# peterhpark/neuroclear

Hardware: AMD Instinct MI355X
Metric: voxels/sec (higher is better)
Workload: dtype f32

## Files before the change

include/nc_hip.h:

```cpp
#ifndef NC_HIP_H
#define NC_HIP_H

#include <stddef.h>
#include <stdint.h>

#ifdef __cplusplus
extern "C" {
#endif

#define NC_OK 0
#define NC_ERR_SHAPE (-1)
#define NC_ERR_WS (-2)
#define NC_ERR_HIP (-3)
#define NC_ERR_ARG (-4)

const char* nc_last_error(void);
int nc_version(void);
int nc_conv_fwd_path(int C, int K, int kd, int kh, int kw, int stride, int pad);
int nc_conv_wgrad_path(int C, int K, int kd, int kh, int kw, int stride, int pad);
void nc_prof_begin(double min_flop);
int nc_prof_end(int max, int* cls, double* flop, float* ms);
int nc_prof_end2(int max, int* cls, double* flop, float* ms, double* abytes);
void nc_set_force_direct(int on);
void nc_sconv_set_cfg(int cfg);
// ... 2 lines not shown
size_t nc_conv_ws_bytes(int N, int C, int D, int H, int W, int K, int kd, int kh, int kw, int stride, int pad);
int nc_conv_fwd(const float* x, const float* w, const float* bias, float* y, int N, int C, int D, int H, int W,
                int K, int kd, int kh, int kw, int stride, int pad, void* ws, size_t ws_bytes, void* stream);
int nc_conv_dgrad(const float* dy, const float* w, float* dx, int N, int C, int D, int H, int W, int K, int kd,
                  int kh, int kw, int stride, int pad, void* ws, size_t ws_bytes, void* stream);
int nc_conv_wgrad(const float* x, const float* dy, float* dw, float* dbias , int N, int C, int D, int H,
                  int W, int K, int kd, int kh, int kw, int stride, int pad, void* ws, size_t ws_bytes, void* stream);
int nc_conv_bwd(const float* x, const float* dy, const float* w, float* dx, float* dw, float* dbias, int N, int C, int D, int H, int W,
                int K, int kd, int kh, int kw, int stride, int pad, void* ws, size_t ws_bytes, void* stream);

#define NC_DT_F32 0
#define NC_DT_F16 1
#define NC_DT_BF16 2
int nc_conv_lp_supported(int what, int N, int C, int D, int H, int W, int K, int kd, int kh, int kw, int stride, int pad);
size_t nc_conv_lp_ws_bytes(int N, int C, int D, int H, int W, int K, int kd, int kh, int kw, int stride, int pad);
size_t nc_c8_bytes(int N, int C, long S);
int nc_to_c8(const float* x, void* xh, int N, int C, long S, int dtype, void* stream);
int nc_conv_fwd_lp(const float* x, const void* xh, const float* w, const float* bias, float* y, int N, int C, int D, int H,
                   int W, int K, int kd, int kh, int kw, int stride, int pad, int dtype, void* ws, size_t ws_bytes,
                   void* stream);
int nc_conv_dgrad_lp(const float* dy, const void* dyh, const float* w, float* dx, int N, int C, int D, int H, int W, int K,
                     int kd, int kh, int kw, int stride, int pad, int dtype, void* ws, size_t ws_bytes, void* stream);
int nc_conv_wgrad_lp(const float* x, const void* xh, const float* dy, const void* dyh, float* dw,
                     float* dbias , int N, int C, int D, int H, int W, int K, int kd, int kh, int kw,
                     int stride, int pad, int dtype, void* ws, size_t ws_bytes, void* stream);

size_t nc_convT_ws_bytes(int N, int C, int D, int H, int W, int K);
int nc_convT_k2s2_fwd(const float* x, const float* w, const float* bias, float* y, int N, int C, int D, int H, int W,
                      int K, void* stream);
int nc_convT_k2s2_dgrad(const float* dy, const float* w, float* dx, int N, int C, int D, int H, int W, int K,
                        void* ws, size_t ws_bytes, void* stream);
int nc_convT_k2s2_wgrad(const float* x, const float* dy, float* dw, float* dbias, int N, int C, int D, int H, int W,
                        int K, void* ws, size_t ws_bytes, void* stream);

size_t nc_instnorm_ws_bytes(int NC, long S);
int nc_instnorm_stats(const float* x, int NC, long S, float eps, float* mean, float* rstd, void* ws, size_t ws_bytes,
                      void* stream);
int nc_instnorm_fwd(const float* x, float eps, float slope, float* mean, float* rstd, float* y, int NC, long S, void* ws,
                    size_t ws_bytes, void* stream);
int nc_instnorm_act_fwd(const float* x, const float* mean, const float* rstd, float slope, float* y, int NC, long S,
                        void* stream);
int nc_instnorm_act_bwd(const float* dy, const float* x, const float* mean, const float* rstd, float slope, float* dx,
                        int NC, long S, void* ws, size_t ws_bytes, void* stream);
int nc_batchnorm_stats(const float* x, int N, int C, long S, float eps, float momentum, int training, float* mean, float* rstd,
                       float* running_mean, float* running_var, void* ws, size_t ws_bytes, void* stream);
int nc_batchnorm_act_fwd(const float* x, const float* mean, const float* rstd, const float* gamma, const float* beta, float slope, float* y,
                         int N, int C, long S, void* stream);
int nc_batchnorm_act_bwd(const float* dy, const float* x, const float* mean, const float* rstd, const float* gamma, const float* beta,
                         float slope, int training, float* dx, float* dgamma, float* dbeta, float* coef , int N, int C,
                         long S, void* ws, size_t ws_bytes, void* stream);
size_t nc_instnorm_bwd_dbias_ws_bytes(int NC, long S);
int nc_instnorm_act_bwd_dbias(const float* dy, const float* x, const float* mean, const float* rstd, float slope, float* dx,
                              float* dbias, int N, int C, long S, void* ws, size_t ws_bytes, void* stream);
int nc_instnorm_act_bwd_dbias_s3(const float* dy, const float* x, const float* mean, const float* rstd, float slope, void* dxs, float* dbias,
                                 int N, int C, long S, void* ws, size_t ws_bytes, void* stream);
int nc_instnorm_act_fwd_c8(const float* x, const float* mean, const float* rstd, float slope, float* y , void* yh,
                           int N, int C, long S, int dtype, void* stream);
int nc_instnorm_act_bwd_c8(const float* dy, const float* x, const float* mean, const float* rstd, float slope, float* dx,
                           void* dxh, float* dbias , int N, int C, long S, int dtype, void* ws, size_t ws_bytes,
                           void* stream);
int nc_leaky_relu_fwd(const float* x, float slope, float* y, long n, void* stream);
int nc_leaky_relu_bwd(const float* dy, const float* x, float slope, float* dx, long n, void* stream);

int nc_maxpool2_fwd(const float* x, float* y, int NC, int D, int H, int W, void* stream);
int nc_maxpool2_bwd(const float* dy, const float* x, float* dx, int NC, int D, int H, int W, void* stream);
int nc_maxpool2_bwd_add(const float* dy, const float* x, const float* skip, float* dx, int NC, int D, int H, int W,
                        void* stream);

int nc_sigmoid_fwd(const float* x, float* y, long n, void* stream);
int nc_sigmoid_bwd(const float* dy, const float* y, float* dx, long n, void* stream);

int nc_slice_fwd(const float* vol, float* out, int NC, int D, int H, int W, int axis, int index, void* stream);
int nc_slice_bwd(const float* dout, float* dvol, int NC, int D, int H, int W, int axis, int index, void* stream);
int nc_mip_fwd(const float* vol, float* out, int32_t* arg, int NC, int D, int H, int W, int axis, int start, int depth,
               void* stream);
int nc_mip_bwd(const float* dout, const int32_t* arg, float* dvol, int NC, int D, int H, int W, int axis,
               void* stream);

int nc_volume_slices(const float* src, float* dst, int N, int C, int D, int H, int W, int axis, int to_volume,
                     void* stream);

size_t nc_loss_ws_bytes(long n);
int nc_mse_const_fwd(const float* pred, long n, float target, float* out, void* ws, size_t ws_bytes, void* stream);
int nc_mse_const_bwd(const float* pred, long n, float target, const float* gscale, float* dpred, void* stream);
int nc_bce_logits_const_fwd(const float* pred, long n, float target, float* out, void* ws, size_t ws_bytes, void* stream);
int nc_bce_logits_const_bwd(const float* pred, long n, float target, const float* gscale, float* dpred, void* stream);
int nc_mean_fwd(const float* pred, long n, float* out, void* ws, size_t ws_bytes, void* stream);
int nc_mean_bwd(long n, const float* gscale, float* dpred, void* stream);
int nc_l1_fwd(const float* a, const float* b, long n, float* out, void* ws, size_t ws_bytes, void* stream);
int nc_l1_bwd(const float* a, const float* b, long n, const float* gscale, float* da, void* stream);

int nc_adam_step(float* p, const float* g, float* m, float* v, long n, float lr, float beta1, float beta2, float eps,
                 int step, void* stream);

int nc_dice_cut_cube(const void* vol, int is_u16, int L0, int L1, int L2, int roi, int overlap, int border, int index,
                     float* cube, void* stream);
int nc_rotate_crop(const void* vol, int is_u16, int D, int H, int W, int z0, int y0, int x0, int cz, int cy, int cx,
                   const double* inv_affine, float* out, void* stream);
int nc_assemble_scatter_add(const float* cube, float* acc, int P0, int P1, int P2, int roi, int overlap, int border,
                            int index, void* stream);
int nc_assemble_finalize(const float* acc, void* out, int out_is_u16, int P0, int P1, int P2, int L0, int L1, int L2,
                         int roi, int overlap, void* stream);
int nc_assemble_finalize_slab(const float* acc_slab, void* out, int out_is_u16, int P0, int P1, int P2, int L0, int L1, int L2, int roi,
                              int overlap, int z0, int nz, int za, void* stream);

int nc_assemble_merge(const float* acc, float* merged, int L0, int L1, int L2, int roi, int overlap, void* stream);
int nc_radix_hist(const float* x, long n, int pass, unsigned prefix, unsigned* hist4096, void* stream);
int nc_assemble_rescale_finalize(const float* merged, void* out, int out_is_u16, int L0, int L1, int L2, int roi,
                                 int overlap, float lo, float hi, float range, void* stream);

size_t nc_match_histograms_ws_bytes(long n);
int nc_match_histograms(const float* source, const float* tmpl, float* out, long n, void* ws, size_t ws_bytes,
                        void* stream);

int nc_spectral_norm_fwd(const float* w_orig, float* u, float* v, float* w_out, float* sigma, float* scratch_k, int K, int M,
                         int power_iteration, float eps, void* stream);
int nc_spectral_norm_bwd(const float* g, const float* w_sn, const float* u, const float* v, const float* sigma, float* dw_orig, int K,
                         int M, void* stream);

size_t nc_patchgan_param_floats(int n_layers, int ndf, int nd);
size_t nc_patchgan_saved_floats(int B, int D, int H, int W, int n_layers, int ndf, int nd);
size_t nc_patchgan_ws_bytes(int B, int D, int H, int W, int n_layers, int ndf, int nd);
int nc_patchgan_out_shape(int B, int D, int H, int W, int n_layers, int ndf, int nd, int* oD, int* oH, int* oW);
int nc_patchgan_fwd(const float* params, const float* x, float* y, float* saved, int B, int D, int H, int W,
                    int n_layers, int ndf, int nd, void* ws, size_t ws_bytes, void* stream);
int nc_patchgan_bwd(const float* params, const float* x, const float* saved, const float* dy, float* dx, float* dparams,
                    int B, int D, int H, int W, int n_layers, int ndf, int nd, void* ws, size_t ws_bytes, void* stream);
int nc_patchgan_fwd_part(const float* params, const float* x, float* y, float* saved, int Btot, int b0, int B, int D, int H,
                         int W, int n_layers, int ndf, int nd, void* ws, size_t ws_bytes, void* stream);
int nc_patchgan_bwd_part(const float* params, const float* x, const float* saved, const float* dy, float* dx, int Btot, int b0,
                         int B, int D, int H, int W, int n_layers, int ndf, int nd, void* ws, size_t ws_bytes, void* stream);
size_t nc_patchgan_gp_saved_floats(int B, int D, int H, int W, int n_layers, int ndf, int nd);
size_t nc_patchgan_gp_ws_bytes(int B, int D, int H, int W, int n_layers, int ndf, int nd);
int nc_patchgan_gp_fwd(const float* params, const float* x, float* g, float* pen, float* saved, int B, int D, int H, int W, int n_layers,
                       int ndf, int nd, float constant, float lambda_gp, void* ws, size_t ws_bytes, void* stream);
int nc_patchgan_gp_bwd(const float* params, const float* x, const float* saved, const float* g, const float* dpen, float* dparams, float* dx,
                       int B, int D, int H, int W, int n_layers, int ndf, int nd, float constant, float lambda_gp, void* ws, size_t ws_bytes,
                       void* stream);

size_t nc_unet_deconv_fwd_ws_bytes(int N, int S0, int S1, int S2);
int nc_unet_deconv_fwd(const float* params, const float* x, float* y, int N, int S0, int S1, int S2, void* ws,
                       size_t ws_bytes, void* stream);


size_t nc_unet_deconv_param_floats(void);
size_t nc_unet_deconv_saved_floats(int N, int S0, int S1, int S2);
size_t nc_unet_deconv_train_ws_bytes(int N, int S0, int S1, int S2);
int nc_unet_deconv_train_fwd(const float* params, const float* x, float* y, float* saved, int N, int S0, int S1, int S2,
                             void* ws, size_t ws_bytes, void* stream, unsigned* kept);
int nc_unet_deconv_bwd(const float* params, const float* x, const float* y, const float* saved, const float* dy, float* dx,
                       float* dparams, int N, int S0, int S1, int S2, void* ws, size_t ws_bytes, void* stream, unsigned kept);
void nc_set_unet_lean(int on);
int nc_get_unet_lean(void);
void nc_set_unet_wprep(int on);
int nc_get_unet_wprep(void);
int nc_unet_wprep_layout(int N, int S0, int S1, int S2, int block, int form, size_t* pack_off, size_t* pack_bytes, size_t* cell_off,
                         size_t* bound_off);
int nc_s3x_pack_h2_debug(const float* w, int C, int K, int form, const unsigned* cell_a, const unsigned* cell_b, void* wp, unsigned* wcell,
                         void* stream);
int nc_convT_h2_bound_debug(const float* w, const float* bias, int C, int K, float in_bound, unsigned* cell, void* stream);
size_t nc_deep_linear_param_floats(void);
size_t nc_deep_linear_saved_floats(int N, int S0, int S1, int S2);
size_t nc_deep_linear_ws_bytes(int N, int S0, int S1, int S2);
int nc_deep_linear_fwd(const float* params, const float* x, float* y, float* saved , int N, int S0, int S1,
                       int S2, void* ws, size_t ws_bytes, void* stream, unsigned* kept );
void nc_set_dl_collapse(int on);
int nc_get_dl_collapse(void);
int nc_deep_linear_bwd(const float* params, const float* x, const float* saved, const float* dy, float* dx, float* dparams,
                       int N, int S0, int S1, int S2, void* ws, size_t ws_bytes, void* stream, unsigned kept);

int nc_conv_fwd_c8(const void* xh, const float* w, const float* bias, void* yh, int out_ctot, int out_c0, int N, int C, int D, int H,
                   int W, int K, int kd, int kh, int kw, int stride, int pad, int dtype, void* ws, size_t ws_bytes, void* stream);
int nc_conv_dgrad_c8(const void* dyh, const float* w, void* dxh, int N, int C, int D, int H, int W, int K, int kd, int kh, int kw,
                     int stride, int pad, int dtype, void* ws, size_t ws_bytes, void* stream);
size_t nc_conv_c1_c8_ws_bytes(int N, int D, int H, int W, int ks);
int nc_conv_c1_fwd_c8(const float* x, const float* w, const float* bias, void* yh, int out_ctot, int out_c0, int N, int D, int H, int W,
                      int ks, int dtype, void* ws, size_t ws_bytes, void* stream);
int nc_conv_c1_dgrad_c8(const void* dyh, const float* w, float* dx, int N, int D, int H, int W, int ks, void* ws, size_t ws_bytes,
                        void* stream);
size_t nc_conv_c1_wgrad_c8_ws_bytes(int N, int D, int H, int W, int ks);
int nc_conv_c1_wgrad_c8(const float* x, const void* dyh, float* dw, int N, int D, int H, int W, int ks, void* ws, size_t ws_bytes,
                        void* stream);
size_t nc_c8_instnorm_ws_bytes(int N, int C, long S);
int nc_c8_instnorm_stats(const void* xh, int N, int C, long S, float eps, float* mean, float* rstd, int dtype, void* ws,
                         size_t ws_bytes, void* stream);
int nc_c8_instnorm_act_fwd(const void* xh, const float* mean, const float* rstd, float slope, void* yh, int out_ctot, int out_c0,
                           int N, int C, long S, int dtype, void* stream);
int nc_c8_instnorm_act_bwd(const void* gh, int g_ctot, int g_c0, const void* xh, const float* mean, const float* rstd, float slope,
                           void* dxh, float* dbias , int N, int C, long S, int dtype, void* ws, size_t ws_bytes,
                           void* stream);
int nc_c8_maxpool2_fwd(const void* xh, int x_ctot, int x_c0, void* yh, int N, int C, int D, int H, int W, int dtype, void* stream);
int nc_c8_maxpool2_bwd_add(const void* dph, const void* xh, int x_ctot, int x_c0, const void* skiph, int s_ctot, int s_c0, void* dxh,
                           int N, int C, int D, int H, int W, int dtype, void* stream);
int nc_from_c8(const void* xh, int x_ctot, int x_c0, float* y, int N, int C, long S, int dtype, void* stream);
size_t nc_convT_c8_ws_bytes(int N, int C, int D, int H, int W, int K);
int nc_convT_k2s2_fwd_c8(const void* xh, const float* w, const float* bias, void* yh, int out_ctot, int out_c0, int N, int C, int D,
                         int H, int W, int K, int dtype, void* ws, size_t ws_bytes, void* stream);
int nc_convT_k2s2_dgrad_c8(const void* dyh, int dy_ctot, int dy_c0, const float* w, void* dxh, int N, int C, int D, int H, int W, int K,
                           void* ws, size_t ws_bytes, void* stream);
int nc_convT_k2s2_wgrad_c8(const void* xh, const void* dyh, int dy_ctot, int dy_c0, float* dw, float* dbias , int N,
                           int C, int D, int H, int W, int K, void* ws, size_t ws_bytes, void* stream);

int nc_unet_deconv_lp_supported(int N, int S0, int S1, int S2, int dtype);
size_t nc_unet_deconv_lp_saved_bytes(int N, int S0, int S1, int S2);
size_t nc_unet_deconv_lp_ws_bytes(int N, int S0, int S1, int S2);
int nc_unet_deconv_lp_fwd(const float* params, const float* x, float* y, void* saved, int N, int S0, int S1, int S2, int dtype,
                          void* ws, size_t ws_bytes, void* stream);
int nc_unet_deconv_lp_bwd(const float* params, const float* x, const float* y, const void* saved, const float* dy, float* dx,
                          float* dparams, int N, int S0, int S1, int S2, int dtype, void* ws, size_t ws_bytes, void* stream);
int nc_deep_linear_lp_supported(int N, int S0, int S1, int S2, int dtype);
size_t nc_deep_linear_lp_saved_bytes(int N, int S0, int S1, int S2);
size_t nc_deep_linear_lp_ws_bytes(int N, int S0, int S1, int S2);
int nc_deep_linear_lp_fwd(const float* params, const float* x, float* y, void* saved, int N, int S0, int S1, int S2, int dtype,
                          void* ws, size_t ws_bytes, void* stream, unsigned* kept);
int nc_deep_linear_lp_bwd(const float* params, const float* x, const void* saved, const float* dy, float* dx, float* dparams,
                          int N, int S0, int S1, int S2, int dtype, void* ws, size_t ws_bytes, void* stream, unsigned kept);

void nc_set_conv_split(int on);
int nc_get_conv_split(void);
void nc_set_split_terms(int terms);
int nc_get_split_terms(void);
void nc_set_p2d_terms(int mode);
int nc_get_p2d_terms(void);
void nc_set_h2_guard(int on);
int nc_get_h2_guard(void);
int nc_h2_guard_stats(unsigned long long* out4, int reset);
void nc_set_epi_stats(int on);
int nc_get_epi_stats(void);
void nc_set_s3x_w64(int on);
int nc_get_s3x_w64(void);
int nc_unet_deconv_fwd_terms(int S0, int S1, int S2);
void nc_set_c8x_mode(int mode);
int nc_get_c8x_mode(void);
int nc_conv_lp_uses_c8x(int what , int fp32_out, int N, int C, int D, int H, int W, int K, int ks);
void nc_set_s3_fusion(int on);
int nc_conv_split_supported(int what, int N, int C, int D, int H, int W, int K, int kd, int kh, int kw, int stride, int pad);
size_t nc_conv_split_ws_bytes(int N, int C, int D, int H, int W, int K, int ks);
size_t nc_s3_bytes(int N, int C, long S);
int nc_to_s3(const float* x, void* xs, int N, int C, long S, void* stream);
int nc_conv_fwd_split(const float* x, const void* xs, const float* w, const float* bias, float* y, int N, int C, int D, int H, int W,
                      int K, int ks , void* ws, size_t ws_bytes, void* stream);
int nc_conv_dgrad_split(const float* dy, const void* dys, const float* w, float* dx, int N, int C, int D, int H, int W, int K, int ks,
                        void* ws, size_t ws_bytes, void* stream);
int nc_conv_wgrad_split(const float* x, const void* xs, const float* dy, const void* dys, float* dw, int N, int C, int D, int H, int W,
                        int K, int ks, void* ws, size_t ws_bytes, void* stream);

int nc_conv2d_split_active(int what, int N, int C, int H, int W, int K, int k, int stride, int pad);

int nc_convT_k2s2_split_supported(int N, int C, int D, int H, int W, int K);
int nc_convT_k2s2_split_active(int N, int C, int D, int H, int W, int K);
size_t nc_convT_k2s2_split_ws_bytes(int N, int C, int D, int H, int W, int K);
int nc_convT_k2s2_fwd_split(const float* x, const void* xs, const float* w, const float* bias, float* y, void* ys, int ys_ctot, int ys_c0,
                            int N, int C, int D, int H, int W, int K, void* ws, size_t ws_bytes, void* stream);

size_t nc_h2_bytes(int N, int C, long S);
size_t nc_h2_cells_offset(size_t elems);
int nc_to_h2_debug(const float* x, long xstride, void* xs, int N, int C, long S, int ctot, int c0, unsigned* cell, float bound, unsigned* guard,
                   void* stream);
int nc_act_split2h_debug(const float* x, const float* mean, const float* rstd, float slope, float* y, long ystride, void* ys, int N, int C, long S,
                         int ctot, int c0, float bound, unsigned* cell, unsigned* cell2, void* stream);
int nc_act_split2h_pool_debug(const float* x, const float* mean, const float* rstd, float slope, void* ys, void* pooled, int N, int C, int D, int H,
                              int W, int ctot, int c0, float bound, unsigned* cell, void* stream);
int nc_maxpool2_h2_debug(const void* in, void* out, int N, int C, int ctot, int D, int H, int W, void* stream);
int nc_h2_to_s3_if_debug(const void* xh, void* xs, int N, int C, long S, const unsigned* cells, const unsigned* guard, void* stream);
int nc_instnorm_act_bwd_dbias_h2_debug(const float* dy, const float* w1, const float* x, const float* mean, const float* rstd, float slope, void* dxs,
                                       float* dbias, int N, int C, long S, void* ws, size_t ws_bytes, unsigned* guard, void* stream);
size_t nc_convT_k2s2_split_h2_ws_bytes(int N, int C, int D, int H, int W, int K);
int nc_convT_k2s2_fwd_split_h2_debug(const float* x, const float* w, const float* bias, float* y, void* ys, int ys_ctot, int ys_c0, int N, int C,
                                     int D, int H, int W, int K, unsigned* out_cell, void* ws, size_t ws_bytes, void* stream);

size_t nc_lk_ws_bytes(int N, int D, int H, int W, int k);
int nc_lk_fwd(const float* x, const float* w, float* y, int N, int D, int H, int W, int k, void* ws, size_t ws_bytes, void* stream);
int nc_lk_dgrad(const float* dy, const float* w, float* dx, int N, int D, int H, int W, int k, void* ws, size_t ws_bytes, void* stream);
int nc_lk_wgrad(const float* x, const float* dy, float* dw, int N, int D, int H, int W, int k, void* ws, size_t ws_bytes, void* stream);

size_t nc_kgan_param_floats(int ndf, int nd);
size_t nc_kgan_saved_floats(int B, int D, int H, int W, int ndf, int nd);
size_t nc_kgan_ws_bytes(int B, int D, int H, int W, int ndf, int nd);
int nc_kgan_out_shape(int B, int D, int H, int W, int ndf, int nd, int* oD, int* oH, int* oW);
int nc_kgan_fwd(const float* params, const float* x, float* y, float* saved, int B, int D, int H, int W, int ndf, int nd, void* ws,
                size_t ws_bytes, void* stream);
int nc_kgan_bwd(const float* params, const float* x, const float* saved, const float* dy, float* dx, float* dparams, int B, int D, int H,
                int W, int ndf, int nd, void* ws, size_t ws_bytes, void* stream);

#ifdef __cplusplus
}
#endif
#endif
```

neuroclear_amd/_lib.py:

```python
import ctypes
import os
import re

_HERE = os.path.dirname(os.path.abspath(__file__))
LIB_PATH = os.environ.get('NC_HIP_LIB') or os.path.join(_HERE, 'csrc', 'libnc_hip.so')
HEADER_PATH = os.path.join(os.path.dirname(_HERE), 'include', 'nc_hip.h')

_lib = None


class NcError(RuntimeError):
    pass


def header_symbols():
    src = open(HEADER_PATH).read()
    src = re.sub(r'/\*.*?\*/', '', src, flags=re.S)
    return sorted(set(re.findall(r'\b(nc_[a-zA-Z0-9_]+)\s*\(', src)))


def lib():
    global _lib
    if _lib is None:
        if not os.path.exists(LIB_PATH):
            raise NcError('libnc_hip.so is not built (%s): run `python -c "import __graft_entry__ as g; g.build()"` '
                          'or `make -C neuroclear_amd/csrc`; there is no CPU fallback' % LIB_PATH)
        L = ctypes.CDLL(LIB_PATH)
        for name in header_symbols():
            fn = getattr(L, name)
            if name.endswith('_bytes') or name.endswith('_floats') or name == 'nc_h2_cells_offset':
                fn.restype = ctypes.c_size_t
            elif name == 'nc_last_error':
                fn.restype = ctypes.c_char_p
            elif name in ('nc_set_force_direct', 'nc_prof_begin', 'nc_sconv_set_cfg', 'nc_sconv_set_tune', 'nc_set_conv_split', 'nc_set_s3_fusion', 'nc_set_c8x_mode', 'nc_set_split_terms', 'nc_set_h2_guard', 'nc_set_epi_stats', 'nc_set_dl_collapse', 'nc_set_p2d_terms', 'nc_set_s3x_w64', 'nc_set_unet_lean', 'nc_set_unet_wprep'):
                fn.restype = None
            else:
                fn.restype = ctypes.c_int
        _lib = L
    return _lib


def check(code, what=''):
    if code != 0:
        raise NcError('%s failed (%d): %s' % (what, code, lib().nc_last_error().decode()))


P = ctypes.c_void_p
I = ctypes.c_int
L_ = ctypes.c_long
F = ctypes.c_float
Z = ctypes.c_size_t
```

neuroclear_amd/csrc/common.hpp:

```cpp
#pragma once
#include <hip/hip_runtime.h>

#include <cstdarg>
#include <cstdio>

#include "../../include/nc_hip.h"

namespace nc {

void set_error(const char* fmt, ...);

inline int check_launch(const char* what) {
  hipError_t e = hipGetLastError();
  if (e != hipSuccess) {
    set_error("%s: %s", what, hipGetErrorString(e));
    return NC_ERR_HIP;
  }
  return NC_OK;
}

inline long cdiv(long a, long b) { return (a + b - 1) / b; }

int raise_dyn_lds(const void* kernel, int bytes, const char* who);
template <typename K>
// ... 56 lines not shown
bool c1k3_fwd_supported(const ConvDims& d);
int conv_fwd_c1k3(const float* x, const float* w, const float* bias, float* y, const ConvDims& d, hipStream_t s, float* stats_part = nullptr);
size_t c1k3_stats_bytes(const ConvDims& d);
int c1k3_stats_finalize(const float* stats_part, const float* bias, const ConvDims& d, float eps, float* mean, float* rstd, hipStream_t s);
bool mfma_dgrad_supported(const ConvDims& d);
bool mfma_wgrad_supported(const ConvDims& d);
size_t mfma_ws_bytes(const ConvDims& d);
size_t mfma_fwd_ws_bytes(const ConvDims& d);
int conv_fwd_mfma(const float* x, const float* w, const float* b, float* y, const ConvDims& d, void* ws, size_t wsb,
                  hipStream_t s);
int conv_dgrad_mfma(const float* dy, const float* w, float* dx, const ConvDims& d, void* ws, size_t wsb,
                    hipStream_t s);
int conv_wgrad_mfma(const float* x, const float* dy, float* dw, const ConvDims& d, void* ws, size_t wsb,
                    hipStream_t s);

bool gemm_fwd_supported(const ConvDims& d);
bool gemm_dgrad_supported(const ConvDims& d);
bool gemm_wgrad_supported(const ConvDims& d);
size_t gemm_ws_bytes(const ConvDims& d);
int conv_fwd_gemm(const float* x, const float* w, const float* b, float* y, const ConvDims& d, void* ws, size_t wsb,
                  hipStream_t s);
int conv_dgrad_gemm(const float* dy, const float* w, float* dx, const ConvDims& d, void* ws, size_t wsb,
                    hipStream_t s);
int conv_wgrad_gemm(const float* x, const float* dy, float* dw, const ConvDims& d, void* ws, size_t wsb,
                    hipStream_t s);

bool sconv_fwd_supported(const ConvDims& d);
bool sconv_dgrad_supported(const ConvDims& d);
size_t sconv_ws_bytes(const ConvDims& d);
void p2d_set_terms(int m);
int p2d_get_terms();
bool p2d_fwd_supported(const ConvDims& d);
bool p2d_dgrad_supported(const ConvDims& d);
size_t p2d_ws_bytes(const ConvDims& d);
int conv_fwd_p2d(const float* x, const float* w, const float* bias, float* y, const ConvDims& d, void* ws, size_t wsb, hipStream_t s);
int conv_dgrad_p2d(const float* dy, const float* w, float* dx, const ConvDims& d, void* ws, size_t wsb, hipStream_t s);
bool p2d_wgrad_supported(const ConvDims& d);
size_t p2d_wgrad_ws_bytes(const ConvDims& d);
int conv_wgrad_p2d(const float* x, const float* dy, float* dw, const ConvDims& d, void* ws, size_t wsb, hipStream_t s);
int conv_fwd_sconv(const float* x, const float* w, const float* bias, float* y, const ConvDims& d, void* ws, size_t wsb, hipStream_t s);
int conv_dgrad_sconv(const float* dy, const float* w, float* dx, const ConvDims& d, void* ws, size_t wsb, hipStream_t s);
void sconv_set_cfg(int cfg);
void sconv_set_tune(int on);
bool sconv_wgrad_supported(const ConvDims& d);
size_t sconv_wgrad_ws_bytes(const ConvDims& d);
int conv_wgrad_sconv(const float* x, const float* dy, float* dw, const ConvDims& d, void* ws, size_t wsb, hipStream_t s);

bool pg1_supported(const ConvDims& d);
size_t pg1_ws_bytes(const ConvDims& d);
int conv_fwd_pg1(const float* x, const float* w, const float* bias, float* y, const ConvDims& d, float slope, hipStream_t s);
int conv_wgrad_pg1(const float* x, const float* g, const float* act, float slope, float* dw, float* db, const ConvDims& d,
                   void* ws, size_t wsb, hipStream_t s);
int conv_dgrad_pg1(const float* g, const float* act, float slope, const float* w, float* dx, const ConvDims& d, hipStream_t s);

bool wgrad_1x1_supported(const ConvDims& d);
size_t wgrad_1x1_ws_bytes(const ConvDims& d);
int conv_wgrad_1x1(const float* x, const float* dy, float* dw, const ConvDims& d, void* ws, size_t wsb, hipStream_t s);
bool flat_1x1_supported(const ConvDims& d);
int conv_fwd_1x1(const float* x, const float* w, const float* b, float* y, const ConvDims& d, void* ws, size_t wsb,
                 hipStream_t s);
int conv_dgrad_1x1(const float* dy, const float* w, float* dx, const ConvDims& d, void* ws, size_t wsb,
                   hipStream_t s);

size_t conv_fwd_to1_k3_ws_bytes(int N, int D, int H, int W);
int conv_fwd_to1_k3(const float* x, const float* w, float* y, int N, int C, int D, int H, int W, void* ws, size_t wsb, hipStream_t s);
bool to1_dgrad_supported(const ConvDims& d);
int conv_dgrad_to1(const float* dy, const float* w, float* dx, const ConvDims& d, hipStream_t s);
bool to1_mfma_supported(const ConvDims& d);
size_t to1_mfma_ws_bytes(const ConvDims& d);
int conv_dgrad_to1_mfma(const float* dy, const float* w, float* dx, const ConvDims& d, void* ws, size_t wsb,
                        hipStream_t s);
bool k1_fwd_supported(const ConvDims& d);
bool k1_wgrad_supported(const ConvDims& d);
int conv_fwd_k1(const float* x, const float* w, const float* b, float* y, const ConvDims& d, hipStream_t s);
int conv_wgrad_k1(const float* x, const float* dy, float* dw, const ConvDims& d, hipStream_t s);
bool c1_wgrad_supported(const ConvDims& d);
size_t c1_wgrad_ws_bytes(const ConvDims& d);
int conv_wgrad_c1(const float* x, const float* dy, float* dw, const ConvDims& d, void* ws, size_t wsb, hipStream_t s);

bool s3_fwd_supported(const ConvDims& d);
bool s3_dgrad_supported(const ConvDims& d);
size_t s3_ws_bytes(const ConvDims& d);
size_t s3_tensor_bytes(int N, int C, long S);
int split3_to(const float* x, void* xs, int N, int C, long S, hipStream_t s);
int split3_into(const float* x, long xstride, void* xs, int N, int C, long S, int ctot, int c0, hipStream_t s, const unsigned* guard = nullptr);
bool conv_layer_h2(const ConvDims& d);
struct ForceThreeTerm { ForceThreeTerm(); ~ForceThreeTerm(); };
struct NetworkScope { NetworkScope(); ~NetworkScope(); };
struct SwitchScope { SwitchScope(); ~SwitchScope(); };
struct ForceTwoTerm { ForceTwoTerm(); ~ForceTwoTerm(); int prev_terms, prev_depth; };
int frozen_terms();
int frozen_guard();
bool h2_guard_can_flip();
int operand_into(const ConvDims& d, const float* x, long xstride, void* xs, int N, int C, long S, int ctot, int c0, hipStream_t s);
int act_operand(const ConvDims& d, const float* x, const float* mean, const float* rstd, float slope, float* y, long ystride, void* ys, int N, int C,
                long S, int ctot, int c0, hipStream_t s);
int act_split3(const float* x, const float* mean, const float* rstd, float slope, float* y, long ystride, void* ys, int N, int C, long S,
               int ctot, int c0, hipStream_t s);
struct S3xPrepared { const void* wp; const unsigned* wcell; };
int conv_fwd_s3(const float* x, const void* xs, const float* w, const float* b, float* y, const ConvDims& d, void* ws, size_t wsb,
                hipStream_t s, void* xs_keep = nullptr, float* stats_part = nullptr, const S3xPrepared* prep = nullptr);
bool epi_stats_on();
void epi_stats_set(int on);
int epi_stats_mode();
void s3x_w64_set(int on);
int s3x_w64_get();
int conv_dgrad_s3(const float* dy, const void* dys, const float* w, float* dx, const ConvDims& d, void* ws, size_t wsb, hipStream_t s);
size_t s3_bwd_ws_bytes(const ConvDims& d);
int conv_bwd_s3(const float* x, const float* dy, const float* w, float* dx, float* dw, const ConvDims& d, void* ws, size_t wsb,
                hipStream_t s, int phase, const void* xs = nullptr, bool dy_guarded = false, const S3xPrepared* prep = nullptr);
int conv_fwd_keep(const float* x, const float* w, const float* bias, float* y, int N, int C, int D, int H, int W, int K, int ks,
                  void* ws, size_t ws_bytes, void* stream, void* xs_keep, bool* kept, const S3xPrepared* prep = nullptr);
int conv_bwd_keep(const float* x, const void* xs, const float* dy, const float* w, float* dx, float* dw, int N, int C, int D, int H,
                  int W, int K, int ks, void* ws, size_t ws_bytes, void* stream);
bool s3x_supported(int N, int Cin, int D, int H, int W, int Kout, int KS);
size_t s3x_packed_bytes(int Cin, int Kout, int KS, int NT = 3);
int s3x_ksteps(int Cin, int KS);
constexpr int kWPrepMaxSegs = 18, kWPrepMaxBounds = 2, kWPrepBoundCell0 = kWPrepMaxSegs, kWPrepCellBytes = 256;
struct WPrepSeg { const float* w; int Cin, Kout, flip; unsigned a_bits; int b_cell; unsigned* ext_cell; };
struct WPrepBound { const float* w; const float* bias; int C, K; float in_bound; int cell; };
size_t wprep_bytes(const WPrepSeg* segs, int n);
int wprep_run(const WPrepSeg* segs, int n, const WPrepBound* bounds, int nb, void* region, S3xPrepared* out, hipStream_t s);
int s3x_pack_h2(const float* w, int Cin, int Kout, int KS, long so, long si, int flip, int split_c, const unsigned* cell_a, const unsigned* cell_b,
                unsigned* wcell, void* wp_ws, hipStream_t s);
void s3x_set_terms(int t);
int s3x_get_terms();
int conv_s3x_h2(const void* xs, const unsigned* cell_a, const unsigned* cell_b, int split_c, const float* w, const float* bias, float* y, int N,
                int Cin, int D, int H, int W, int Kout, int KS, long so, long si, int flip, unsigned* wcell, void* wp_ws, hipStream_t s,
                const unsigned* guard = nullptr, float* stats_part = nullptr, const S3xPrepared* prep = nullptr);
size_t s3x_stats_bytes(int N, int D, int H, int W, int Kout, int KS);
int s3x_stats_finalize(const float* stats_part, const float* bias, int N, int D, int H, int W, int Kout, int KS, float eps, float* mean, float* rstd,
                       hipStream_t s);
bool c1k7_h2_supported(const ConvDims& d);
size_t c1k7_h2_ws_bytes(const ConvDims& d);
int conv_c1k7_h2(const float* x, const float* w, const float* bias, float* y, const ConvDims& d, void* ws, size_t wsb, hipStream_t s);
size_t c1k7_h2_dgrad_ws_bytes(const ConvDims& d);
bool dl_typed_supported(int N, int D, int H, int W);
size_t dl_typed_bytes(int N, int D, int H, int W);
const float* dl_typed_wp(const char* scratch, int N, int D, int H, int W);
float* dl_typed_dwsw(char* scratch, int N, int D, int H, int W);
int dl_typed_compose(const float* F, char* scratch, int N, int D, int H, int W, hipStream_t s);
int dl_typed_fwd_boundary(const float* act0, float* y, char* scratch, int N, int D, int H, int W, hipStream_t s);
int dl_typed_dgrad_boundary(const float* act0, const float* dy, float* g, char* scratch, int N, int D, int H, int W, hipStream_t s);
int dl_typed_p(const float* act0, const float* dy, float* Pq, char* scratch, int N, int D, int H, int W, hipStream_t s);
int conv_c1k7_h2_dgrad(const float* dy, const float* w, float* dx, const ConvDims& d, void* ws, size_t wsb, hipStream_t s);
inline size_t h2_cells_offset(size_t elems) { return (elems * 4 + 255) & ~(size_t)255; }
inline unsigned* h2_cells_of(const void* t, size_t elems) { return (unsigned*)((char*)const_cast<void*>(t) + h2_cells_offset(elems)); }
int instnorm_relu_tail_sigmoid(const float* x, const float* mean, const float* rstd, const float* w1, const float* b1, const float* w2,
                               const float* b2, float* y, int C, long S, hipStream_t s);
int instnorm_act_bwd_dbias_h2(const float* dy, const float* x, const float* mean, const float* rstd, float slope, void* dxs,
                              float* dbias, int N, int C, long S, void* ws, size_t ws_bytes, void* stream, unsigned* guard = nullptr);
int instnorm_act_bwd_dbias_h2_rank1(const float* dy1, const float* w1, const float* x, const float* mean, const float* rstd, float slope, void* dxs,
                                    float* dbias, int C, long S, void* ws, size_t ws_bytes, void* stream, unsigned* guard);
unsigned* conv_bwd_guard_words(void* ws, int N, int K, long S);
int maxpool2_h2(const void* in, void* out, int N, int C, int ctot, int D, int H, int W, hipStream_t s);
int h2_zero_cells(unsigned* cells, int n, hipStream_t s);
int h2_set_cell(unsigned* cell, float bound, hipStream_t s);
int h2_absmax(const float* x, long n, unsigned* cell, hipStream_t s, unsigned* cell2 = nullptr);
int split2h_into(const float* x, long xstride, void* xs, int N, int C, long S, int ctot, int c0, const unsigned* cell, hipStream_t s,
                 unsigned* guard = nullptr);
constexpr int kGuardLow = 0, kGuardAll = 1, kGuardFlag = 2;
constexpr unsigned kGuardDrop = 17u << 23;
constexpr unsigned long long kGuardShare = 64;
#if defined(__HIP_DEVICE_COMPILE__)
__device__ __forceinline__ bool guard_skip(const unsigned* guard, int want) {
  return guard && (int)(__builtin_nontemporal_load(guard + kGuardFlag) != 0) != want;
}
#else
__device__ bool guard_skip(const unsigned* guard, int want);
#endif
bool h2_guard_on();
int h2_guard_mode();
void h2_guard_set(int on);
int h2_guard_read(unsigned long long* out4, int reset);
int h2_guard_zero(unsigned* g, hipStream_t s, int nwords = 8);
int h2_guard_decide(unsigned* ga, unsigned* gb, unsigned* prior, unsigned* flag, bool can_flip, hipStream_t s, unsigned long long total_a = 0);
int h2_to_s3_if(const void* xh, void* xs, int N, int C, long S, const unsigned* cells, const unsigned* guard, hipStream_t s);
int act_split2h(const float* x, const float* mean, const float* rstd, float slope, float* y, long ystride, void* ys, int N, int C, long S, int ctot,
                int c0, float bound, unsigned* cell, unsigned* cell2, hipStream_t s);
int act_split2h_pool(const float* x, const float* mean, const float* rstd, float slope, void* ys, void* pooled, int N, int C, int D, int H, int W,
                     int ctot, int c0, float bound, unsigned* cell, hipStream_t s);
int conv_s3x(const void* xs, const float* w, const float* bias, float* y, int N, int Cin, int D, int H, int W, int Kout, int KS, long so,
             long si, int flip, void* wp_ws, hipStream_t s, const unsigned* guard = nullptr);
bool conv_keep_supported(int N, int C, int D, int H, int W, int K, int ks);
int conv_fwd_pre(const void* xs, const float* w, const float* bias, float* y, int N, int C, int D, int H, int W, int K, int ks, void* ws,
                 size_t ws_bytes, void* stream, float* stats_part = nullptr, const S3xPrepared* prep = nullptr);
bool conv_bwd_pre_supported(int N, int C, int D, int H, int W, int K, int ks, bool want_dx, size_t ws_bytes);
int conv_bwd_pre(const float* x, const void* xs, const float* w, float* dx, float* dw, int N, int C, int D, int H, int W, int K, int ks,
                 void* ws, size_t ws_bytes, void* stream, bool dy_guarded = false, const S3xPrepared* prep = nullptr);
bool instnorm_bwd_s3_supported(int N, int C, long S);
int instnorm_act_bwd_dbias_s3(const float* dy, const float* x, const float* mean, const float* rstd, float slope, void* dxs,
                              float* dbias, int N, int C, long S, void* ws, size_t ws_bytes, void* stream);
bool convT_fwd_s3_supported(int N, int C, int D, int H, int W, int K);
size_t c8x_packed_bytes(int Cin, int Kout, int KS);
void c8x_set_mode(int m);
int c8x_get_mode();
bool c8x_supported(int N, int Cin, int D, int H, int W, int Kout, int KS, bool fp32_out);
int conv_c8x(const void* xh, const float* w, const float* bias, float* y, void* yh, int ctot, int c0, int N, int Cin, int D, int H, int W,
             int Kout, int KS, long so, long si, int flip, int diffuse, int dt, void* wp_ws, hipStream_t s);
bool convT_s3x_supported(int N, int C, int D, int H, int W, int K);
size_t convT_s3x_ws_bytes(int C, int K);
int convT_fwd_s3x(const void* xs, const float* w, const float* bias, float* y, void* ys, int ctot, int c0, int N, int C, int D, int H, int W,
                  int K, void* ws, size_t wsb, hipStream_t s, const unsigned* h2cell = nullptr, const unsigned* xcell = nullptr);
int convT_h2_bound(const float* w, const float* bias, int C, int K, float in_bound, unsigned* cell, hipStream_t s);
int convT_fwd_split_h2(const float* x, const float* w, const float* bias, float* y, void* ys, int ys_ctot, int ys_c0, int N, int C, int D, int H,
                       int W, int K, const unsigned* out_cell, void* ws, size_t ws_bytes, hipStream_t s);
int convT_fwd_s3(const float* x, const float* w, const float* bias, float* y, void* ys, int ctot, int c0, int N, int C, int D, int H,
                 int W, int K, void* stream);
bool s3_wgrad_supported(const ConvDims& d);
bool c8x_wgrad_supported(const ConvDims& d);
size_t c8x_wgrad_part_bytes(const ConvDims& d);
int conv_wgrad_c8x(const void* xh, const void* dyh, float* dw, const ConvDims& d, int dtype, void* ws, size_t wsb, hipStream_t s);
size_t s3_wgrad_ws_bytes(const ConvDims& d);
int conv_wgrad_s3(const float* x, const void* xs, const float* dy, const void* dys, float* dw, const ConvDims& d, void* ws, size_t wsb,
                  hipStream_t s);
bool s3x_k32_supported(int N, int D, int H, int W);
bool conv_fwd_h2_k32_supported(const ConvDims& d);
int conv_fwd_h2_k32_keep(const float* x, const float* w, float* y, const ConvDims& d, void* ws, size_t wsb, hipStream_t s, void* xs_keep);
bool conv_fwd_h2_c32_supported(const ConvDims& d);
size_t conv_fwd_h2_c32_ws_bytes(const ConvDims& d);
int conv_fwd_h2_c32(const float* x, const float* w, float* y, const ConvDims& d, void* ws, size_t wsb, hipStream_t s);
bool wgrad_h2_supported(const ConvDims& d);
int conv_wgrad_h2(const float* x, const void* xs, const float* dy, const void* dys, float* dw, const ConvDims& d, void* ws, size_t wsb, hipStream_t s);
bool h_fwd_supported(const ConvDims& d);
bool h_dgrad_supported(const ConvDims& d);
bool h_wgrad_supported(const ConvDims& d);
size_t h_ws_bytes(const ConvDims& d);
int to_c8(const float* x, void* xh, int N, int C, long S, int dt, hipStream_t s);
int conv_fwd_h(const float* x, const void* xh, const float* w, const float* b, float* y, const ConvDims& d, int dt,
               void* ws, size_t wsb, hipStream_t s);
int conv_dgrad_h(const float* dy, const void* dyh, const float* w, float* dx, const ConvDims& d, int dt, void* ws,
                 size_t wsb, hipStream_t s);
int conv_wgrad_h(const float* x, const void* xh, const float* dy, const void* dyh, float* dw, const ConvDims& d, int dt,
                 void* ws, size_t wsb, hipStream_t s);
int conv_fwd_h_c8(const void* xh, const float* w, const float* b, void* yh, int ctot, int c0, const ConvDims& d, int dt,
                  void* ws, size_t wsb, hipStream_t s);
int conv_fwd_h_na1(const void* xh, const float* w, float* y, const ConvDims& d, int dt, void* ws, size_t wsb, hipStream_t s);
int conv_dgrad_h_c8(const void* dyh, const float* w, void* dxh, int ctot, int c0, const ConvDims& d, int dt, void* ws,
                    size_t wsb, hipStream_t s);
bool dl_collapse_on();
size_t dl_tail_bytes();
const float* dl_tail_E(const char* tail);
const float* dl_tail_Ef(const char* tail);
float* dl_tail_q(char* tail);
int dl_tail_compose(const float* w2, const float* w3, const float* w4, const float* w5, char* tail, hipStream_t s);
int dl_tail_grads(const float* w2, const float* w3, const float* w4, const float* w5, char* tail, float* dw2, float* dw3, float* dw4, float* dw5,
                  hipStream_t s);
float* dl_tail_P(char* tail);
const float* dl_w1_fold(char* tail, const float* w1, hipStream_t s);
int dl_w1_contract(const char* tail, float* dw1, hipStream_t s);
int dl_q_from_p(char* tail, const float* w1, hipStream_t s);
const float* dl_fold_fwd64(char* tail, const float* w1, hipStream_t s);
int dl_combine27(const float* Z, float* y, int N, int D, int H, int W, int zch, hipStream_t s);
bool c1_h_supported(int D, int H, int W, int KS);
size_t c1_h_ws_bytes(int N, int D, int H, int W, int KS);
int conv_c1_fwd_h(const float* x, const float* w, const float* bias, void* yh, int ctot, int c0, int N, int D, int H, int W, int KS,
                  int dt, void* ws, size_t wsb, hipStream_t s);
int conv_c1_dgrad_h(const void* dyh, const float* w, float* dx, int N, int D, int H, int W, int KS, void* ws, size_t wsb,
                    hipStream_t s);

void h_set_weight_diffusion(int on);

bool c1_wgrad_h_supported(int N, int D, int H, int W, int KS);
size_t c1_wgrad_h_ws_bytes(int N, int D, int H, int W, int KS);
int conv_c1_wgrad_h(const float* x, const void* dyh, float* dw, int N, int D, int H, int W, int KS, void* ws, size_t wsb,
                    hipStream_t s);

static constexpr size_t kPackSlackBytes = 128 * 1024;

extern int g_force_direct;

struct ProfScope {
  int idx;
  hipStream_t s;
  ProfScope(int op, int path, const ConvDims& d, int lp, hipStream_t stream);
  ~ProfScope();
};

}
```

neuroclear_amd/csrc/gen_nets.hip:

```cpp

#include <atomic>
#include <cstdlib>

#include "common.hpp"

using namespace nc;

#define NC_TRY(expr) do { int e_ = (expr); if (e_) return e_; } while (0)

namespace {

size_t up64(size_t n) { return (n + 63) & ~(size_t)63; }

size_t s3_floats(size_t elems) { return up64((elems * 6 + 3) / 4); }
size_t align256(size_t b) { return (b + 255) & ~(size_t)255; }

std::atomic<int> g_unet_lean{getenv("NC_UNET_LEAN") ? (atoi(getenv("NC_UNET_LEAN")) != 0) : 1};
constexpr int kLeanBit0 = 10;
constexpr int kLeanBlocks[5] = {1, 3, 5, 6, 8};
int lean_index(int consumer) {
  for (int j = 0; j < 5; ++j) if (kLeanBlocks[j] == consumer) return j;
  return -1;
}

struct UBlock { int C, K, lvl; };
const UBlock kUB[10] = {{1, 64, 0},    {64, 64, 0},    {64, 128, 1},  {128, 128, 1}, {128, 256, 2},
                        {256, 256, 2}, {256, 256, 2}, {256, 128, 1}, {128, 128, 1}, {128, 64, 0}};

std::atomic<int> g_unet_wprep{getenv("NC_UNET_WPREP") ? (atoi(getenv("NC_UNET_WPREP")) != 0) : 1};
constexpr unsigned kKeptWPrep = 1u << 15;
void wprep_segs(WPrepSeg (&sg)[18]) {
  for (int i = 1; i < 10; ++i) {
    sg[2 * (i - 1)] = WPrepSeg{nullptr, kUB[i].C, kUB[i].K, 0, 0u, -1, nullptr};
    sg[2 * (i - 1) + 1] = WPrepSeg{nullptr, kUB[i].K, kUB[i].C, 1, 0u, -1, nullptr};
  }
}
unsigned f32_bits(float f) { unsigned b; __builtin_memcpy(&b, &f, 4); return b; }


struct UPlan {
  int N, d[3][3];
  long S[3];
  size_t a1, cat1, p1, a2, cat2, p2, b1, b2, b3, e2a, e2b, e1, t1, raw[10], mean[10], rstd[10], saved;
  size_t xs3[10];
  size_t wprep;
  size_t G1, G2, G3, H1, H2, H3, Q1, Q2, s1, s2, T, grads;
  size_t conv_ws, in_ws, convT_ws;
};

bool u_plan(UPlan& p, int N, int S0, int S1, int S2) {
  if (N < 1 || S0 < 4 || S1 < 4 || S2 < 4 || (S0 & 3) || (S1 & 3) || (S2 & 3)) return false;
  p = UPlan{};
  p.N = N;
  for (int l = 0; l < 3; ++l) {
    p.d[l][0] = S0 >> l; p.d[l][1] = S1 >> l; p.d[l][2] = S2 >> l;
    p.S[l] = (long)p.d[l][0] * p.d[l][1] * p.d[l][2];
  }
  const size_t n = (size_t)N, S = (size_t)p.S[0], Sh = (size_t)p.S[1], Sq = (size_t)p.S[2];
  size_t off = 0;
  auto take = [&](size_t k) { size_t r = off; off += up64(k); return r; };
  p.a1 = take(n * 64 * S); p.cat1 = take(n * 128 * S); p.p1 = take(n * 64 * Sh); p.a2 = take(n * 128 * Sh);
  p.cat2 = take(n * 256 * Sh); p.p2 = take(n * 128 * Sq); p.b1 = take(n * 256 * Sq); p.b2 = take(n * 256 * Sq);
  p.b3 = take(n * 256 * Sq); p.e2a = take(n * 128 * Sh); p.e2b = take(n * 128 * Sh); p.e1 = take(n * 64 * S);
  p.t1 = take(n * S);
  for (int i = 0; i < 10; ++i) {
    p.raw[i] = take(n * kUB[i].K * (size_t)p.S[kUB[i].lvl]);
    p.mean[i] = take(n * kUB[i].K);
    p.rstd[i] = take(n * kUB[i].K);
  }
  for (int i = 1; i < 10; ++i) { p.xs3[i] = off; off += s3_floats(n * kUB[i].C * (size_t)p.S[kUB[i].lvl]); }
  {
    WPrepSeg sg[18];
    wprep_segs(sg);
    p.wprep = off;
    off += up64((wprep_bytes(sg, 18) + 3) / 4);
  }
  p.saved = off;
  off = 0;
  p.G1 = take(n * 64 * S); p.G2 = take(n * 64 * S); p.G3 = take(n * 128 * S);
  p.H1 = take(n * 128 * Sh); p.H2 = take(n * 128 * Sh); p.H3 = take(n * 256 * Sh);
  p.Q1 = take(n * 256 * Sq); p.Q2 = take(n * 256 * Sq); p.s1 = take(n * S); p.s2 = take(n * S);
  p.T = take(n * 64 * S);
  p.grads = off;
  auto upd = [&](int C, int K, int l, int k) {
    const size_t b = nc_conv_ws_bytes(N, C, p.d[l][0], p.d[l][1], p.d[l][2], K, k, k, k, 1, k / 2);
    if (b > p.conv_ws) p.conv_ws = b;
  };
  for (int i = 0; i < 10; ++i) upd(kUB[i].C, kUB[i].K, kUB[i].lvl, 3);
  upd(64, 1, 0, 1); upd(1, 1, 0, 1);
  p.in_ws = nc_instnorm_bwd_dbias_ws_bytes(N * 256, (long)S);
  for (int i = 1; i < 10; ++i) {
    const size_t b = s3x_stats_bytes(N, p.d[kUB[i].lvl][0], p.d[kUB[i].lvl][1], p.d[kUB[i].lvl][2], kUB[i].K, 3);
    if (b > p.in_ws) p.in_ws = b;
  }
  p.convT_ws = nc_convT_ws_bytes(N, 256, p.d[2][0], p.d[2][1], p.d[2][2], 128);
  const size_t c2 = nc_convT_ws_bytes(N, 128, p.d[1][0], p.d[1][1], p.d[1][2], 64);
  if (c2 > p.convT_ws) p.convT_ws = c2;
  return true;
}

struct UOff { size_t w[14], b[14], total; };
UOff u_offsets() {
  struct L { int id; size_t wn, bn; };
  const L order[14] = {{0, 64 * 1 * 27, 64},     {1, 64 * 64 * 27, 64},    {2, 128 * 64 * 27, 128},  {3, 128 * 128 * 27, 128},
                       {4, 256 * 128 * 27, 256}, {5, 256 * 256 * 27, 256}, {6, 256 * 256 * 27, 256}, {10, 256 * 128 * 8, 128},
                       {7, 128 * 256 * 27, 128}, {8, 128 * 128 * 27, 128}, {11, 128 * 64 * 8, 64},   {9, 64 * 128 * 27, 64},
                       {12, 64, 1},              {13, 1, 1}};
  UOff o{};
  size_t off = 0;
  for (const L& l : order) {
    o.w[l.id] = off; off += l.wn;
    o.b[l.id] = off; off += l.bn;
  }
  o.total = off;
  return o;
}

int gather_half(const float* src, float* dst, int N, int Ctot, int c0, int C, long S, hipStream_t s) {
  if (hipMemcpy2DAsync(dst, (size_t)C * S * 4, src + (size_t)c0 * S, (size_t)Ctot * S * 4, (size_t)C * S * 4, N,
                       hipMemcpyDeviceToDevice, s) != hipSuccess) {
    set_error("gather_half: hipMemcpy2DAsync failed");
    return NC_ERR_HIP;
  }
  return NC_OK;
}

size_t u_ws_bytes(const UPlan& p, bool bwd) {
  return align256(p.conv_ws) + align256(p.in_ws) + align256(p.convT_ws) + (bwd ? p.grads * sizeof(float) : 0) + 256;
}

}

extern "C" {

void nc_set_unet_wprep(int on) { g_unet_wprep.store(on != 0, std::memory_order_relaxed); }
int nc_get_unet_wprep(void) { return g_unet_wprep.load(std::memory_order_relaxed); }
void nc_set_unet_lean(int on) { g_unet_lean.store(on != 0, std::memory_order_relaxed); }
int nc_get_unet_lean(void) { return g_unet_lean.load(std::memory_order_relaxed); }

size_t nc_unet_deconv_param_floats(void) { return u_offsets().total; }

int nc_unet_wprep_layout(int N, int S0, int S1, int S2, int block, int form, size_t* pack_off, size_t* pack_bytes, size_t* cell_off,
                         size_t* bound_off) {
  UPlan p;
  if (!u_plan(p, N, S0, S1, S2) || block < 1 || block > 9 || form < 0 || form > 1) { set_error("unet_wprep_layout: bad argument"); return NC_ERR_ARG; }
  WPrepSeg sg[18];
  wprep_segs(sg);
  const int k = 2 * (block - 1) + form;
  size_t off = kWPrepCellBytes;
  for (int j = 0; j < k; ++j) off += s3x_packed_bytes(sg[j].Cin, sg[j].Kout, 3, 2);
  if (pack_off) *pack_off = p.wprep * 4 + off;
  if (pack_bytes) *pack_bytes = s3x_packed_bytes(sg[k].Cin, sg[k].Kout, 3, 2);
  if (cell_off) *cell_off = p.wprep * 4 + (size_t)k * 4;
  if (bound_off) *bound_off = block == 7 ? p.wprep * 4 + (size_t)kWPrepBoundCell0 * 4 : block == 9 ? p.wprep * 4 + (size_t)(kWPrepBoundCell0 + 1) * 4 : 0;
  return NC_OK;
}
int nc_s3x_pack_h2_debug(const float* w, int C, int K, int form, const unsigned* cell_a, const unsigned* cell_b, void* wp, unsigned* wcell,
                         void* stream) {
  if (!w || !cell_a || !cell_b || !wp || !wcell || C % 64 || K % 64) { set_error("s3x_pack_h2_debug: bad argument"); return NC_ERR_ARG; }
  if (form) return s3x_pack_h2(w, K, C, 3, 27, (long)C * 27, 1, K, cell_a, cell_a, wcell, wp, (hipStream_t)stream);
  return s3x_pack_h2(w, C, K, 3, (long)C * 27, 27, 0, C / 2, cell_a, cell_b, wcell, wp, (hipStream_t)stream);
}
int nc_convT_h2_bound_debug(const float* w, const float* bias, int C, int K, float in_bound, unsigned* cell, void* stream) {
  if (!w || !cell) { set_error("convT_h2_bound_debug: null pointer"); return NC_ERR_ARG; }
  NC_TRY(h2_zero_cells(cell, 1, (hipStream_t)stream));
  return convT_h2_bound(w, bias, C, K, in_bound, cell, (hipStream_t)stream);
}

size_t nc_unet_deconv_saved_floats(int N, int S0, int S1, int S2) {
  UPlan p;
  return u_plan(p, N, S0, S1, S2) ? p.saved : 0;
}

size_t nc_unet_deconv_train_ws_bytes(int N, int S0, int S1, int S2) {
  UPlan p;
  return u_plan(p, N, S0, S1, S2) ? u_ws_bytes(p, true) : 0;
}

int nc_unet_deconv_train_fwd(const float* params, const float* x, float* y, float* saved, int N, int S0, int S1, int S2,
                             void* ws, size_t ws_bytes, void* stream, unsigned* kept) {
  NetworkScope net_scope;
  if (!params || !x || !y || !saved) { set_error("unet_deconv_train_fwd: null pointer"); return NC_ERR_ARG; }
  UPlan p;
  if (!u_plan(p, N, S0, S1, S2)) {
    set_error("unet_deconv_train_fwd: every edge must be a positive multiple of 4 (got %d,%d,%d)", S0, S1, S2);
    return NC_ERR_SHAPE;
  }
  if (!ws || ws_bytes < u_ws_bytes(p, false)) { set_error("unet_deconv_train_fwd: workspace too small"); return NC_ERR_WS; }
  const UOff o = u_offsets();
  void* cws = ws;
  void* iws = (char*)ws + align256(p.conv_ws);
  float* V = saved;
  const float* P = params;
  if (kept) *kept = 0;
  hipStream_t hs = (hipStream_t)stream;
  static const bool fuse_on = !(getenv("NC_S3_TRAIN_FUSE") && atoi(getenv("NC_S3_TRAIN_FUSE")) == 0);
  const bool lean = g_unet_lean.load(std::memory_order_relaxed) != 0;
  bool use[10], pre[10], h2l[10];
  ConvDims cd[10];
  for (int i = 0; i < 10; ++i) {
    const UBlock& b = kUB[i];
    const int* d = p.d[b.lvl];
    use[i] = fuse_on && i >= 1 && conv_keep_supported(N, b.C, d[0], d[1], d[2], b.K, 3);
    pre[i] = false;
    h2l[i] = make_dims(cd[i], N, b.C, d[0], d[1], d[2], b.K, 3, 3, 3, 1, 1) && use[i] && conv_layer_h2(cd[i]);
  }
  const long S = p.S[0], Sh = p.S[1], Sq = p.S[2];
  const int *d0 = p.d[0], *d1 = p.d[1], *d2 = p.d[2];
  const bool ct2 = nc_convT_k2s2_split_active(1, 256, d2[0], d2[1], d2[2], 128) &&
                   p.conv_ws >= nc_convT_k2s2_split_ws_bytes(1, 256, d2[0], d2[1], d2[2], 128);
  static const bool ct_h2 = !(getenv("NC_CONVT_H2") && atoi(getenv("NC_CONVT_H2")) == 0);
  const bool ct2h = ct2 && h2l[7] && ct_h2;
  const bool ct1 = nc_convT_k2s2_split_active(1, 128, d1[0], d1[1], d1[2], 64) &&
                   p.conv_ws >= nc_convT_k2s2_split_ws_bytes(1, 128, d1[0], d1[1], d1[2], 64);
  const bool ct1h = ct1 && h2l[9] && ct_h2;
  unsigned* cell7 = h2_cells_of(V + p.xs3[7], (size_t)N * 256 * Sh) + 1;
  unsigned* cell9 = h2_cells_of(V + p.xs3[9], (size_t)N * 128 * S) + 1;
  unsigned kept_mask = 0;
  S3xPrepared prep[18] = {};
  bool bound7 = false, bound9 = false;
  if (g_unet_wprep.load(std::memory_order_relaxed) != 0) {
    WPrepSeg sg[18];
    wprep_segs(sg);
    WPrepBound wb[2];
    int nb = 0, any = 0;
    for (int i = 1; i < 10; ++i) {
      if (!h2l[i]) continue;
      WPrepSeg& f = sg[2 * (i - 1)];
      f.a_bits = f32_bits(sqrtf((float)p.S[kUB[i].lvl]));
      f.w = P + o.w[i];
      if (i == 7 || i == 9) {
        if (i == 7 ? ct2h : ct1h) {
          f.b_cell = kWPrepBoundCell0 + nb;
          f.ext_cell = i == 7 ? cell7 : cell9;
          wb[nb++] = i == 7 ? WPrepBound{P + o.w[10], P + o.b[10], 256, 128, sqrtf((float)Sq), 0}
                            : WPrepBound{P + o.w[11], P + o.b[11], 128, 64, sqrtf((float)Sh), 0};
          (i == 7 ? bound7 : bound9) = true;
        } else {
          f.w = nullptr;
        }
      }
      sg[2 * (i - 1) + 1].w = P + o.w[i];
      any = 1;
    }
    if (any) {
      NC_TRY(wprep_run(sg, 18, wb, nb, V + p.wprep, prep, hs));
      kept_mask |= kKeptWPrep;
    }
  }
  auto prep_of = [&](int seg) -> const S3xPrepared* { return prep[seg].wp ? &prep[seg] : nullptr; };
  auto block = [&](int i, const float* in, float* out, size_t out_stride, int to, int to_ctot) -> int {
    const UBlock& b = kUB[i];
    const int* d = p.d[b.lvl];
    const long S = p.S[b.lvl];
    const bool epi = pre[i] && h2l[i] && epi_stats_mode() == 2 && s3x_stats_bytes(N, d[0], d[1], d[2], b.K, 3) && s3x_stats_bytes(N, d[0], d[1], d[2], b.K, 3) <= p.in_ws;
    if (pre[i]) {
      NC_TRY(conv_fwd_pre(V + p.xs3[i], P + o.w[i], P + o.b[i], V + p.raw[i], N, b.C, d[0], d[1], d[2], b.K, 3, cws, p.conv_ws, stream,
                          epi ? (float*)iws : nullptr, i >= 1 ? prep_of(2 * (i - 1)) : nullptr));
      kept_mask |= 1u << i;
      if (h2l[i]) kept_mask |= 1u << (16 + i);
    } else {
      bool kept1 = false;
      NC_TRY(conv_fwd_keep(in, P + o.w[i], P + o.b[i], V + p.raw[i], N, b.C, d[0], d[1], d[2], b.K, 3, cws, p.conv_ws, stream,
                           i >= 1 ? (void*)(V + p.xs3[i]) : nullptr, &kept1, i >= 1 ? prep_of(2 * (i - 1)) : nullptr));
      if (kept1) kept_mask |= 1u << i;
      if (kept1 && i >= 1 && conv_layer_h2(cd[i])) kept_mask |= 1u << (16 + i);
    }
    if (epi) NC_TRY(s3x_stats_finalize((const float*)iws, P + o.b[i], N, d[0], d[1], d[2], b.K, 3, 1e-5f, V + p.mean[i], V + p.rstd[i], hs));
    else NC_TRY(nc_instnorm_stats(V + p.raw[i], N * b.K, S, 1e-5f, V + p.mean[i], V + p.rstd[i], iws, p.in_ws, stream));
    if (to >= 0 && use[to]) {
      const int lj = lean && h2l[to] && to_ctot == b.K ? lean_index(to) : -1;
      if (lj >= 0) { out = nullptr; kept_mask |= 1u << (kLeanBit0 + lj); }
      NC_TRY(act_operand(cd[to], V + p.raw[i], V + p.mean[i], V + p.rstd[i], 0.f, out, (long)out_stride, V + p.xs3[to], N, b.K, S, to_ctot, 0, hs));
      if (to_ctot == b.K) pre[to] = true;
      return NC_OK;
    }
    if (out_stride == (size_t)b.K * S || N == 1)
      return nc_instnorm_act_fwd(V + p.raw[i], V + p.mean[i], V + p.rstd[i], 0.f, out, N * b.K, S, stream);
    for (int n = 0; n < N; ++n)
      NC_TRY(nc_instnorm_act_fwd(V + p.raw[i] + (size_t)n * b.K * S, V + p.mean[i] + n * b.K, V + p.rstd[i] + n * b.K, 0.f,
                                 out + n * out_stride, b.K, S, stream));
    return NC_OK;
  };
  NC_TRY(block(0, x, V + p.a1, (size_t)64 * S, 1, 64));
  NC_TRY(block(1, V + p.a1, V + p.cat1, (size_t)128 * S, 9, 128));
  for (int n = 0; n < N; ++n)
    NC_TRY(nc_maxpool2_fwd(V + p.cat1 + (size_t)n * 128 * S, V + p.p1 + (size_t)n * 64 * Sh, 64, d0[0], d0[1], d0[2], stream));
  NC_TRY(block(2, V + p.p1, V + p.a2, (size_t)128 * Sh, 3, 128));
  NC_TRY(block(3, V + p.a2, V + p.cat2, (size_t)256 * Sh, 7, 256));
  for (int n = 0; n < N; ++n)
    NC_TRY(nc_maxpool2_fwd(V + p.cat2 + (size_t)n * 256 * Sh, V + p.p2 + (size_t)n * 128 * Sq, 128, d1[0], d1[1], d1[2], stream));
  NC_TRY(block(4, V + p.p2, V + p.b1, (size_t)256 * Sq, 5, 256));
  NC_TRY(block(5, V + p.b1, V + p.b2, (size_t)256 * Sq, 6, 256));
  NC_TRY(block(6, V + p.b2, V + p.b3, (size_t)256 * Sq, -1, 0));
  if (ct2h && !bound7) {
    NC_TRY(h2_zero_cells(cell7, 1, hs));
    NC_TRY(convT_h2_bound(P + o.w[10], P + o.b[10], 256, 128, sqrtf((float)Sq), cell7, hs));
  }
  for (int n = 0; n < N; ++n) {
    if (ct2h)
      NC_TRY(convT_fwd_split_h2(V + p.b3 + (size_t)n * 256 * Sq, P + o.w[10], P + o.b[10], V + p.cat2 + ((size_t)n * 256 + 128) * Sh,
                                (char*)(V + p.xs3[7]) + (size_t)n * 256 * Sh * 4, 256, 128, 1, 256, d2[0], d2[1], d2[2], 128, cell7, cws, p.conv_ws, hs));
    else if (ct2)
      NC_TRY(nc_convT_k2s2_fwd_split(V + p.b3 + (size_t)n * 256 * Sq, nullptr, P + o.w[10], P + o.b[10], V + p.cat2 + ((size_t)n * 256 + 128) * Sh,
                                     use[7] && !h2l[7] ? (char*)(V + p.xs3[7]) + (size_t)n * 256 * Sh * 6 : nullptr, 256, 128, 1, 256, d2[0], d2[1], d2[2], 128, cws,
                                     p.conv_ws, stream));
    else
      NC_TRY(nc_convT_k2s2_fwd(V + p.b3 + (size_t)n * 256 * Sq, P + o.w[10], P + o.b[10], V + p.cat2 + ((size_t)n * 256 + 128) * Sh,
                               1, 256, d2[0], d2[1], d2[2], 128, stream));
  }
  if (use[7]) {
    if (!ct2 || (h2l[7] && !ct2h)) NC_TRY(operand_into(cd[7], V + p.cat2 + (size_t)128 * Sh, (long)256 * Sh, V + p.xs3[7], N, 128, Sh, 256, 128, hs));
    pre[7] = true;
  }
  NC_TRY(block(7, V + p.cat2, V + p.e2a, (size_t)128 * Sh, 8, 128));
  NC_TRY(block(8, V + p.e2a, V + p.e2b, (size_t)128 * Sh, -1, 0));
  const bool ct_s3 = use[9] && !h2l[9] && (ct1 || convT_fwd_s3_supported(1, 128, d1[0], d1[1], d1[2], 64));
  if (ct1h && !bound9) {
    NC_TRY(h2_zero_cells(cell9, 1, hs));
    NC_TRY(convT_h2_bound(P + o.w[11], P + o.b[11], 128, 64, sqrtf((float)Sh), cell9, hs));
  }
  for (int n = 0; n < N; ++n) {
    if (ct1h)
      NC_TRY(convT_fwd_split_h2(V + p.e2b + (size_t)n * 128 * Sh, P + o.w[11], P + o.b[11], V + p.cat1 + ((size_t)n * 128 + 64) * S,
                                (char*)(V + p.xs3[9]) + (size_t)n * 128 * S * 4, 128, 64, 1, 128, d1[0], d1[1], d1[2], 64, cell9, cws, p.conv_ws, hs));
    else if (ct1)
      NC_TRY(nc_convT_k2s2_fwd_split(V + p.e2b + (size_t)n * 128 * Sh, nullptr, P + o.w[11], P + o.b[11], V + p.cat1 + ((size_t)n * 128 + 64) * S,
                                     use[9] && !h2l[9] ? (char*)(V + p.xs3[9]) + (size_t)n * 128 * S * 6 : nullptr, 128, 64, 1, 128, d1[0], d1[1], d1[2], 64, cws,
                                     p.conv_ws, stream));
    else if (ct_s3)
      NC_TRY(convT_fwd_s3(V + p.e2b + (size_t)n * 128 * Sh, P + o.w[11], P + o.b[11], V + p.cat1 + ((size_t)n * 128 + 64) * S,
                          (char*)(V + p.xs3[9]) + (size_t)n * 128 * S * 6, 128, 64, 1, 128, d1[0], d1[1], d1[2], 64, stream));
    else
      NC_TRY(nc_convT_k2s2_fwd(V + p.e2b + (size_t)n * 128 * Sh, P + o.w[11], P + o.b[11], V + p.cat1 + ((size_t)n * 128 + 64) * S,
                               1, 128, d1[0], d1[1], d1[2], 64, stream));
  }
  if (use[9]) {
    if (!ct_s3 && !ct1h) NC_TRY(operand_into(cd[9], V + p.cat1 + (size_t)64 * S, (long)128 * S, V + p.xs3[9], N, 64, S, 128, 64, hs));
    pre[9] = true;
  }
  NC_TRY(block(9, V + p.cat1, V + p.e1, (size_t)64 * S, -1, 0));
  NC_TRY(nc_conv_fwd(V + p.e1, P + o.w[12], P + o.b[12], V + p.t1, N, 64, d0[0], d0[1], d0[2], 1, 1, 1, 1, 1, 0, cws, p.conv_ws, stream));
  NC_TRY(nc_conv_fwd(V + p.t1, P + o.w[13], P + o.b[13], y, N, 1, d0[0], d0[1], d0[2], 1, 1, 1, 1, 1, 0, cws, p.conv_ws, stream));
  if (kept) *kept = kept_mask;
  return nc_sigmoid_fwd(y, y, (long)N * S, stream);
}

int nc_unet_deconv_bwd(const float* params, const float* x, const float* y, const float* saved, const float* dy, float* dx,
                       float* dparams, int N, int S0, int S1, int S2, void* ws, size_t ws_bytes, void* stream, unsigned kept) {
  NetworkScope net_scope;
  if (!params || !x || !y || !saved || !dy || !dparams) { set_error("unet_deconv_bwd: null pointer"); return NC_ERR_ARG; }
  UPlan p;
  if (!u_plan(p, N, S0, S1, S2)) { set_error("unet_deconv_bwd: bad shape"); return NC_ERR_SHAPE; }
  if (!ws || ws_bytes < u_ws_bytes(p, true)) { set_error("unet_deconv_bwd: workspace too small"); return NC_ERR_WS; }
  const UOff o = u_offsets();
  hipStream_t hs = (hipStream_t)stream;
  void* cws = ws;
  void* iws = (char*)ws + align256(p.conv_ws);
  void* tws = (char*)iws + align256(p.in_ws);
  float* G = (float*)((char*)tws + align256(p.convT_ws));
  const float* V = saved;
  const float* P = params;
  float* DP = dparams;
  const long S = p.S[0], Sh = p.S[1], Sq = p.S[2];
  const int *d0 = p.d[0], *d1 = p.d[1], *d2 = p.d[2];
  const unsigned kept_mask = kept;
  static const bool fuse_bwd = !(getenv("NC_S3_TRAIN_FUSE") && atoi(getenv("NC_S3_TRAIN_FUSE")) == 0) &&
                               true;
  const bool wprep_now = g_unet_wprep.load(std::memory_order_relaxed) != 0;
  S3xPrepared prepd[10] = {};
  {
    WPrepSeg sg[18];
    wprep_segs(sg);
    const char* region = (const char*)(V + p.wprep);
    size_t off = kWPrepCellBytes;
    for (int k = 0; k < 18; ++k) {
      if (k & 1) prepd[k / 2 + 1] = S3xPrepared{region + off, (const unsigned*)region + k};
      off += s3x_packed_bytes(sg[k].Cin, sg[k].Kout, 3, 2);
    }
  }
  auto block_bwd = [&](int i, const float* g, const float* in, float* draw, float* gin, bool r1 = false) -> int {
    const UBlock& b = kUB[i];
    const int* d = p.d[b.lvl];
    const long Sl = p.S[b.lvl];
    ConvDims cdk;
    const bool now_h2 = make_dims(cdk, N, b.C, d[0], d[1], d[2], b.K, 3, 3, 3, 1, 1) && conv_layer_h2(cdk);
    const void* xs = ((kept_mask >> i) & 1) && (((kept_mask >> (16 + i)) & 1) != 0) == now_h2 ? (const void*)(V + p.xs3[i]) : nullptr;
    const S3xPrepared* pd = i >= 1 && gin && now_h2 && (kept_mask & kKeptWPrep) && ((kept_mask >> (16 + i)) & 1) && wprep_now ? &prepd[i] : nullptr;
    const int lj = lean_index(i);
    if (lj >= 0 && ((kept_mask >> (kLeanBit0 + lj)) & 1) &&
        !(xs && !h2_guard_can_flip() && conv_bwd_pre_supported(N, b.C, d[0], d[1], d[2], b.K, 3, gin != nullptr, p.conv_ws))) {
      NC_TRY(nc_instnorm_act_fwd(V + p.raw[i - 1], V + p.mean[i - 1], V + p.rstd[i - 1], 0.f, G + p.T, N * b.C, Sl, stream));
      in = G + p.T;
    }
    if (r1) {
      NC_TRY(instnorm_act_bwd_dbias_h2_rank1(g, P + o.w[12], V + p.raw[i], V + p.mean[i], V + p.rstd[i], 0.f, cws, DP + o.b[i], b.K, Sl, iws, p.in_ws,
                                             stream, conv_bwd_guard_words(cws, N, b.K, Sl)));
      return conv_bwd_pre(in, xs, P + o.w[i], gin, DP + o.w[i], N, b.C, d[0], d[1], d[2], b.K, 3, cws, p.conv_ws, stream, h2_guard_can_flip(), pd);
    }
    if (fuse_bwd && i >= 1 && conv_bwd_pre_supported(N, b.C, d[0], d[1], d[2], b.K, 3, gin != nullptr, p.conv_ws) &&
        instnorm_bwd_s3_supported(N, b.K, Sl)) {
      if (now_h2)
        NC_TRY(instnorm_act_bwd_dbias_h2(g, V + p.raw[i], V + p.mean[i], V + p.rstd[i], 0.f, cws, DP + o.b[i], N, b.K, Sl, iws, p.in_ws, stream,
                                         conv_bwd_guard_words(cws, N, b.K, Sl)));
      else
        NC_TRY(instnorm_act_bwd_dbias_s3(g, V + p.raw[i], V + p.mean[i], V + p.rstd[i], 0.f, cws, DP + o.b[i], N, b.K, Sl, iws, p.in_ws, stream));
      return conv_bwd_pre(in, xs, P + o.w[i], gin, DP + o.w[i], N, b.C, d[0], d[1], d[2], b.K, 3, cws, p.conv_ws, stream, now_h2 && h2_guard_can_flip(), pd);
    }
    NC_TRY(nc_instnorm_act_bwd_dbias(g, V + p.raw[i], V + p.mean[i], V + p.rstd[i], 0.f, draw, DP + o.b[i], N, b.K, Sl, iws,
                                     p.in_ws, stream));
    return conv_bwd_keep(in, xs, draw, P + o.w[i], gin, DP + o.w[i], N, b.C, d[0], d[1], d[2], b.K, 3, cws, p.conv_ws, stream);
  };
  auto upper_half = [&](const float* dcat, int Ctot, long Sl, const float** out) -> int {
    const int C = Ctot / 2;
    if (N == 1) { *out = dcat + (size_t)C * Sl; return NC_OK; }
    NC_TRY(gather_half(dcat, G + p.T, N, Ctot, C, C, Sl, hs));
    *out = G + p.T;
    return NC_OK;
  };
  NC_TRY(nc_sigmoid_bwd(dy, y, G + p.s1, (long)N * S, stream));
  NC_TRY(nc_conv_wgrad(V + p.t1, G + p.s1, DP + o.w[13], DP + o.b[13], N, 1, d0[0], d0[1], d0[2], 1, 1, 1, 1, 1, 0, cws, p.conv_ws, stream));
  NC_TRY(nc_conv_dgrad(G + p.s1, P + o.w[13], G + p.s2, N, 1, d0[0], d0[1], d0[2], 1, 1, 1, 1, 1, 0, cws, p.conv_ws, stream));
  ConvDims cd9;
  const bool r1 = g_unet_lean.load(std::memory_order_relaxed) != 0 && N == 1 && fuse_bwd &&
                  make_dims(cd9, N, 128, d0[0], d0[1], d0[2], 64, 3, 3, 3, 1, 1) && conv_layer_h2(cd9) &&
                  conv_bwd_pre_supported(N, 128, d0[0], d0[1], d0[2], 64, 3, true, p.conv_ws) && instnorm_bwd_s3_supported(N, 64, S);
  NC_TRY(nc_conv_wgrad(V + p.e1, G + p.s2, DP + o.w[12], DP + o.b[12], N, 64, d0[0], d0[1], d0[2], 1, 1, 1, 1, 1, 0, cws, p.conv_ws, stream));
  if (!r1) {
    NC_TRY(nc_conv_dgrad(G + p.s2, P + o.w[12], G + p.G1, N, 64, d0[0], d0[1], d0[2], 1, 1, 1, 1, 1, 0, cws, p.conv_ws, stream));
  }
  NC_TRY(block_bwd(9, r1 ? G + p.s2 : G + p.G1, V + p.cat1, G + p.G2, G + p.G3, r1));
  const float* g;
  NC_TRY(upper_half(G + p.G3, 128, S, &g));
  NC_TRY(nc_convT_k2s2_dgrad(g, P + o.w[11], G + p.H1, N, 128, d1[0], d1[1], d1[2], 64, tws, p.convT_ws, stream));
  NC_TRY(nc_convT_k2s2_wgrad(V + p.e2b, g, DP + o.w[11], DP + o.b[11], N, 128, d1[0], d1[1], d1[2], 64, tws, p.convT_ws, stream));
  NC_TRY(block_bwd(8, G + p.H1, V + p.e2a, G + p.H2, G + p.H1));
  NC_TRY(block_bwd(7, G + p.H1, V + p.cat2, G + p.H2, G + p.H3));
  NC_TRY(upper_half(G + p.H3, 256, Sh, &g));
  NC_TRY(nc_convT_k2s2_dgrad(g, P + o.w[10], G + p.Q1, N, 256, d2[0], d2[1], d2[2], 128, tws, p.convT_ws, stream));
  NC_TRY(nc_convT_k2s2_wgrad(V + p.b3, g, DP + o.w[10], DP + o.b[10], N, 256, d2[0], d2[1], d2[2], 128, tws, p.convT_ws, stream));
  NC_TRY(block_bwd(6, G + p.Q1, V + p.b2, G + p.Q2, G + p.Q1));
  NC_TRY(block_bwd(5, G + p.Q1, V + p.b1, G + p.Q2, G + p.Q1));
  NC_TRY(block_bwd(4, G + p.Q1, V + p.p2, G + p.Q2, G + p.Q1));
  for (int n = 0; n < N; ++n)
    NC_TRY(nc_maxpool2_bwd_add(G + p.Q1 + (size_t)n * 128 * Sq, V + p.cat2 + (size_t)n * 256 * Sh, G + p.H3 + (size_t)n * 256 * Sh,
                               G + p.H1 + (size_t)n * 128 * Sh, 128, d1[0], d1[1], d1[2], stream));
  NC_TRY(block_bwd(3, G + p.H1, V + p.a2, G + p.H2, G + p.H1));
  NC_TRY(block_bwd(2, G + p.H1, V + p.p1, G + p.H2, G + p.H1));
  for (int n = 0; n < N; ++n)
    NC_TRY(nc_maxpool2_bwd_add(G + p.H1 + (size_t)n * 64 * Sh, V + p.cat1 + (size_t)n * 128 * S, G + p.G3 + (size_t)n * 128 * S,
                               G + p.G1 + (size_t)n * 64 * S, 64, d0[0], d0[1], d0[2], stream));
  NC_TRY(block_bwd(1, G + p.G1, V + p.a1, G + p.G2, G + p.G1));
  return block_bwd(0, G + p.G1, x, G + p.G2, dx);
}

}

namespace {

struct LLayer { int C, K, k; };
const LLayer kLL[6] = {{1, 64, 7}, {64, 64, 5}, {64, 64, 3}, {64, 32, 1}, {32, 16, 1}, {16, 1, 1}};

struct LPlan {
  int N, d[3];
  long S;
  size_t w[6], params;
  size_t act[5], saved;
  size_t xs3[6];
  size_t g[2], grads;
  size_t conv_ws;
};

struct LTail {
  static constexpr size_t a = 0, e = 32 * 8, r = e + 64 * 8, E = r + 64 * 8, Ef = E + 1728 * 4, q = Ef + 1728 * 4, P = q + 1728 * 4 + 256,
                          Wf = P + (size_t)64 * 32 * 125 * 4 + 256, bytes = Wf + (size_t)64 * 32 * 125 * 4 + 256;
};

__global__ void __launch_bounds__(256) k_dl_shift27(const float* __restrict__ dy, float* __restrict__ dsh, int D, int H, int W) {
  const long S = (long)D * H * W;
  const int a = blockIdx.y, n = blockIdx.z;
  float* out = dsh + ((long)n * 32 + a) * S;
  const float* in = dy + (long)n * S;
  const int az = a / 9 - 1, ay = (a / 3) % 3 - 1, ax = a % 3 - 1;
  for (long v = (long)blockIdx.x * 256 + threadIdx.x; v < S; v += (long)gridDim.x * 256) {
    float r = 0.f;
    if (a < 27) {
      const int x = (int)(v % W), y = (int)((v / W) % H), z = (int)(v / ((long)W * H));
      const int sx = x - ax, sy = y - ay, sz = z - az;
      if ((unsigned)sx < (unsigned)W && (unsigned)sy < (unsigned)H && (unsigned)sz < (unsigned)D) r = in[((long)sz * H + sy) * W + sx];
    }
    out[v] = r;
  }
}
__global__ void __launch_bounds__(128) k_dl_w1_fold(const float* __restrict__ E, const float* __restrict__ w1, float* __restrict__ wf) {
  const int c = blockIdx.x, a = blockIdx.y, sidx = threadIdx.x;
  if (sidx >= 125) return;
  double v = 0.0;
  if (a < 27)
    for (int k = 0; k < 64; ++k) v += (double)w1[((long)k * 64 + c) * 125 + 124 - sidx] * (double)E[k * 27 + a];
  wf[((long)c * 32 + a) * 125 + sidx] = (float)v;
}
__global__ void __launch_bounds__(128) k_dl_fold_fwd(const float* __restrict__ E, const float* __restrict__ w1, float* __restrict__ F) {
  const int t = blockIdx.x, c = blockIdx.y, sidx = threadIdx.x;
  if (sidx >= 125) return;
  double v = 0.0;
  if (t < 27)
    for (int cp = 0; cp < 64; ++cp) v += (double)E[cp * 27 + t] * (double)w1[((long)cp * 64 + c) * 125 + sidx];
  F[((long)t * 64 + c) * 125 + sidx] = (float)v;
}
__global__ void __launch_bounds__(256) k_dl_combine27(const float* __restrict__ Z, float* __restrict__ y, int D, int H, int W, int zch) {
  const long S = (long)D * H * W;
  const int n = blockIdx.y;
  const float* z = Z + (long)n * zch * S;
  for (long v = (long)blockIdx.x * 256 + threadIdx.x; v < S; v += (long)gridDim.x * 256) {
    const int x = (int)(v % W), yy = (int)((v / W) % H), zz = (int)(v / ((long)W * H));
    float acc = 0.f;
#pragma unroll
    for (int t = 0; t < 27; ++t) {
      const int dz = t / 9 - 1, dy = (t / 3) % 3 - 1, dx = t % 3 - 1;
      if ((unsigned)(x + dx) < (unsigned)W && (unsigned)(yy + dy) < (unsigned)H && (unsigned)(zz + dz) < (unsigned)D)
        acc += z[(long)t * S + v + ((long)dz * H + dy) * W + dx];
    }
    y[(long)n * S + v] = acc;
  }
}

__global__ void __launch_bounds__(256) k_dl_q_from_p(const float* __restrict__ w1, const float* __restrict__ Pq, float* __restrict__ qf) {
  __shared__ double red[256];
  const int cp = blockIdx.x, t = blockIdx.y, th = threadIdx.x;
  double v = 0.0;
  for (int i = th; i < 64 * 125; i += 256) {
    const int c = i / 125, sidx = i - c * 125;
    v += (double)w1[((long)cp * 64 + c) * 125 + sidx] * (double)Pq[((long)c * 32 + t) * 125 + 124 - sidx];
  }
  red[th] = v;
  __syncthreads();
  for (int o = 128; o > 0; o >>= 1) {
    if (th < o) red[th] += red[th + o];
    __syncthreads();
  }
  if (th == 0) qf[cp * 27 + 26 - t] = (float)red[0];
}
__global__ void __launch_bounds__(128) k_dl_w1_contract(const float* __restrict__ E, const float* __restrict__ Pq, float* __restrict__ dw1) {
  const int k = blockIdx.x, c = blockIdx.y, t = threadIdx.x;
  if (t >= 125) return;
  double v = 0.0;
#pragma unroll
  for (int a = 0; a < 27; ++a) v += (double)E[k * 27 + a] * (double)Pq[((long)c * 32 + a) * 125 + 124 - t];
  dw1[((long)k * 64 + c) * 125 + t] = (float)v;
}
constexpr unsigned kKeptCollapsed = 1u << 31;
constexpr unsigned kKeptNoAct1 = 1u << 30;
constexpr unsigned kKeptTyped = 1u << 29;

__global__ void __launch_bounds__(256) k_dl_compose(const float* __restrict__ w2, const float* __restrict__ w3, const float* __restrict__ w4,
                                                    const float* __restrict__ w5, char* __restrict__ tail) {
  __shared__ double sa[32], se[64];
  const int t = threadIdx.x;
  if (t < 32) {
    double v = 0.0;
#pragma unroll
    for (int i = 0; i < 16; ++i) v += (double)w5[i] * (double)w4[i * 32 + t];
    sa[t] = v;
    if (blockIdx.x == 0) ((double*)(tail + LTail::a))[t] = v;
  }
  __syncthreads();
  if (t < 64) {
    double v = 0.0;
#pragma unroll
    for (int b = 0; b < 32; ++b) v += sa[b] * (double)w3[b * 64 + t];
    se[t] = v;
    if (blockIdx.x == 0) ((double*)(tail + LTail::e))[t] = v;
  }
  __syncthreads();
  if (t < 216) {
    const int i = blockIdx.x * 216 + t;
    double v = 0.0;
#pragma unroll 16
    for (int k = 0; k < 64; ++k) v += se[k] * (double)w2[(long)k * 1728 + i];
    const int c = i / 27, tap = i - c * 27;
    ((float*)(tail + LTail::E))[i] = (float)v;
    ((float*)(tail + LTail::Ef))[c * 27 + 26 - tap] = (float)v;
  }
}

__global__ void __launch_bounds__(256) k_dl_tail_w2(const float* __restrict__ w2, char* __restrict__ tail, float* __restrict__ dw2) {
  __shared__ double red[256];
  const int k = blockIdx.x, t = threadIdx.x;
  const float* qf = (const float*)(tail + LTail::q);
  const double ek = ((const double*)(tail + LTail::e))[k];
  double part = 0.0;
  for (int i = t; i < 1728; i += 256) {
    const int c = i / 27, tap = i - c * 27;
    const double q = (double)qf[c * 27 + 26 - tap];
    dw2[(long)k * 1728 + i] = (float)(ek * q);
    part += (double)w2[(long)k * 1728 + i] * q;
  }
  red[t] = part;
  __syncthreads();
  for (int o = 128; o > 0; o >>= 1) {
    if (t < o) red[t] += red[t + o];
    __syncthreads();
  }
  if (t == 0) ((double*)(tail + LTail::r))[k] = red[0];
}
// ... 304 lines not shown
```

neuroclear_amd/csrc/h2.hip:

```cpp
#include <atomic>
#include <cstdlib>
#include <mutex>

#include "common.hpp"
#include "s3_common.hpp"

namespace nc {
namespace {

__global__ void __launch_bounds__(256) k_absmax(const float* __restrict__ x, long n, unsigned* __restrict__ cell, unsigned* __restrict__ cell2) {
  unsigned m = 0;
  const int head = (int)((4 - (((unsigned long long)x >> 2) & 3)) & 3) < n ? (int)((4 - (((unsigned long long)x >> 2) & 3)) & 3) : (int)n;
  if (blockIdx.x == 0 && (int)threadIdx.x < head) {
    const unsigned b = __float_as_uint(x[threadIdx.x]) & 0x7fffffffu;
    if (b < 0x7f800000u && b > m) m = b;
  }
  x += head;
  n -= head;
  const long n4 = n >> 2;
  const float4* x4 = reinterpret_cast<const float4*>(x);
  auto take = [&](const float4& v) __attribute__((always_inline)) {
    const unsigned b[4] = {__float_as_uint(v.x) & 0x7fffffffu, __float_as_uint(v.y) & 0x7fffffffu, __float_as_uint(v.z) & 0x7fffffffu,
                           __float_as_uint(v.w) & 0x7fffffffu};
#pragma unroll
// ... 2 lines not shown
  };
  const long stride = (long)gridDim.x * 256;
  long i = (long)blockIdx.x * 256 + threadIdx.x;
  for (; i + 3 * stride < n4; i += 4 * stride) {
    const float4 v0 = x4[i], v1 = x4[i + stride], v2 = x4[i + 2 * stride], v3 = x4[i + 3 * stride];
    take(v0); take(v1); take(v2); take(v3);
  }
  for (; i < n4; i += stride) take(x4[i]);
  if (blockIdx.x == 0 && threadIdx.x < (n & 3)) {
    const unsigned b = __float_as_uint(x[(n4 << 2) + threadIdx.x]) & 0x7fffffffu;
    if (b < 0x7f800000u && b > m) m = b;
  }
#pragma unroll
  for (int o = 32; o > 0; o >>= 1) {
    const unsigned q = (unsigned)__shfl_xor((int)m, o);
    m = q > m ? q : m;
  }
  __shared__ unsigned wm[4];
  if ((threadIdx.x & 63) == 0) wm[threadIdx.x >> 6] = m;
  __syncthreads();
  if (threadIdx.x == 0) {
    unsigned b = wm[0];
    for (int k = 1; k < 4; ++k) b = wm[k] > b ? wm[k] : b;
    if (b) {
      atomicMax(cell, b);
      if (cell2) atomicMax(cell2, b);
    }
  }
}

__global__ void k_set_cells(unsigned* cells, int n, unsigned bits) {
  if ((int)threadIdx.x < n) cells[threadIdx.x] = bits;
}

__global__ void __launch_bounds__(256) k_split2h(const float* __restrict__ x, uint4* __restrict__ out, long S, int cblocks, int oblocks, int ob0,
                                                 long xstride, const unsigned* __restrict__ cell, unsigned* __restrict__ guard) {
  const unsigned cb_bits = *cell;
  const float sc = h2_scale(cb_bits);
  const int n = blockIdx.y / cblocks, cb = blockIdx.y % cblocks;
  const float* xb = x + (long)n * xstride + (long)cb * 8 * S;
  const long ob = (long)n * oblocks + ob0 + cb;
  unsigned n_all = 0, n_low = 0;
  for (long v0 = (long)blockIdx.x * 256; v0 < S; v0 += (long)gridDim.x * 256) {
    const long v = v0 + threadIdx.x;
    unsigned m = 0;
    if (v < S) {
      unsigned short e[8][3];
#pragma unroll
      for (int j = 0; j < 8; ++j) {
        const float f = xb[j * S + v];
        const unsigned b = __float_as_uint(f) & 0x7fffffffu;
        if (b < 0x7f800000u && b > m) m = b;
        h2_split(f * sc, e[j]);
      }
#pragma unroll
      for (int t = 0; t < 2; ++t) out[(ob * 2 + t) * S + v] = s3_unit(e, t);
    }
    if (guard) {
      const unsigned thr = cb_bits > kGuardDrop ? cb_bits - kGuardDrop : 0u;
      const bool any_hi = __builtin_amdgcn_ballot_w64(m >= thr && m != 0) != 0;
      const bool any_nz = __builtin_amdgcn_ballot_w64(m != 0) != 0;
      if (any_nz) {
        ++n_all;
        if (!any_hi) ++n_low;
      }
    }
  }
  if (!guard) return;
  __shared__ unsigned cnt[2];
  if (threadIdx.x < 2) cnt[threadIdx.x] = 0;
  __syncthreads();
  if ((threadIdx.x & 63) == 0) {
    if (n_all) atomicAdd(&cnt[kGuardAll], n_all);
    if (n_low) atomicAdd(&cnt[kGuardLow], n_low);
  }
  __syncthreads();
  if (threadIdx.x < 2 && cnt[threadIdx.x]) atomicAdd(guard + threadIdx.x, cnt[threadIdx.x]);
}

__global__ void k_h2_guard_decide(unsigned* ga, unsigned* gb, unsigned* prior, unsigned* flag, int can_flip, unsigned long long* stats,
                                  unsigned long long total_a) {
  if (threadIdx.x || blockIdx.x) return;
  unsigned f = 0;
  unsigned long long worst = 0;
  int n = 0;
  for (unsigned* g : {ga, gb}) {
    if (!g) continue;
    ++n;
    const unsigned long long lo = g[kGuardLow], all = (g == ga && total_a) ? total_a - g[kGuardAll] : g[kGuardAll];
    if (all && lo * kGuardShare > all) f = 1;
    const unsigned long long ppm = all ? lo * 1000000ull / all : 0;
    worst = ppm > worst ? ppm : worst;
  }
  unsigned F = f && can_flip ? 1u : 0u;
  if (prior && prior[kGuardFlag]) F = 1u;
  *flag = F;
  if (prior) prior[kGuardFlag] = F;
  if (stats && n) {
    __hip_atomic_fetch_add(stats + 0, (unsigned long long)n, __ATOMIC_RELAXED, __HIP_MEMORY_SCOPE_SYSTEM);
    if (f) __hip_atomic_fetch_add(stats + (can_flip ? 1 : 2), 1ull, __ATOMIC_RELAXED, __HIP_MEMORY_SCOPE_SYSTEM);
    __hip_atomic_fetch_max(stats + 3, worst, __ATOMIC_RELAXED, __HIP_MEMORY_SCOPE_SYSTEM);
  }
}

__global__ void __launch_bounds__(256) k_h2_to_s3_if(const uint4* __restrict__ in, uint4* __restrict__ out, long S, int cblocks,
                                                      const unsigned* __restrict__ cells, const unsigned* __restrict__ guard) {
  if (guard_skip(guard, 1)) return;
  const long v = (long)blockIdx.x * 256 + threadIdx.x;
  if (v >= S) return;
  const int cb = blockIdx.y % cblocks;
  const float inv = h2_inv_scale(cells[cb >= cblocks / 2 ? 1 : 0]);
  const long b = blockIdx.y;
  const uint4 a = in[(b * 2 + 0) * S + v], r = in[(b * 2 + 1) * S + v];
  const unsigned aw[4] = {a.x, a.y, a.z, a.w}, rw[4] = {r.x, r.y, r.z, r.w};
  unsigned short e[8][3];
#pragma unroll
  for (int j = 0; j < 8; ++j) {
    const unsigned short h0 = (unsigned short)(aw[j >> 1] >> ((j & 1) * 16)), h1 = (unsigned short)(rw[j >> 1] >> ((j & 1) * 16));
    const float val = ((float)__builtin_bit_cast(_Float16, h0) + (float)__builtin_bit_cast(_Float16, h1)) * inv;
    s3_split(val, e[j]);
  }
#pragma unroll
  for (int t = 0; t < 3; ++t) out[(b * 3 + t) * S + v] = s3_unit(e, t);
}

__global__ void __launch_bounds__(256) k_act_split2h(const float* __restrict__ x, const float* __restrict__ mean, const float* __restrict__ rstd,
                                                     float slope, float* __restrict__ y, long ystride, uint4* __restrict__ out, long S, int cblocks,
                                                     int oblocks, int ob0, unsigned bound_bits, unsigned* __restrict__ cell, unsigned* __restrict__ cell2) {
  if (blockIdx.x == 0 && blockIdx.y == 0 && threadIdx.x == 0) {
    if (cell) *cell = bound_bits;
    if (cell2) *cell2 = bound_bits;
  }
  const long v = (long)blockIdx.x * 256 + threadIdx.x;
  if (v >= S) return;
  const float sc = h2_scale(bound_bits);
  const int n = blockIdx.y / cblocks, cb = blockIdx.y % cblocks;
  const long c0 = (long)blockIdx.y * 8;
  const float* xs = x + c0 * S + v;
  float* ys = y ? y + (long)n * ystride + (long)cb * 8 * S + v : nullptr;
  unsigned short e[8][3];
#pragma unroll
  for (int j = 0; j < 8; ++j) {
    float t = (xs[j * S] - mean[c0 + j]) * rstd[c0 + j];
    t = t > 0.f ? t : t * slope;
    if (ys) ys[j * S] = t;
    asm("" : "+v"(t));
    h2_split(t * sc, e[j]);
  }
  const long ob = (long)n * oblocks + ob0 + cb;
#pragma unroll
  for (int t = 0; t < 2; ++t) out[(ob * 2 + t) * S + v] = s3_unit(e, t);
}

__global__ void __launch_bounds__(256) k_act_split2h_pool(const float* __restrict__ x, const float* __restrict__ mean, const float* __restrict__ rstd,
                                                          float slope, uint4* __restrict__ out, uint4* __restrict__ pooled, int D, int H, int W,
                                                          int cblocks, int oblocks, int ob0, unsigned bound_bits, unsigned* __restrict__ cell) {
  if (blockIdx.x == 0 && blockIdx.y == 0 && threadIdx.x == 0 && cell) *cell = bound_bits;
  const int Do = D / 2, Ho = H / 2, Wo = W / 2;
  const long So = (long)Do * Ho * Wo, S = (long)D * H * W;
  const long v = (long)blockIdx.x * 256 + threadIdx.x;
  if (v >= So) return;
  const int xo = (int)(v % Wo), yo = (int)((v / Wo) % Ho), zo = (int)(v / ((long)Wo * Ho));
  const float sc = h2_scale(bound_bits);
  const int n = blockIdx.y / cblocks, cb = blockIdx.y % cblocks;
  const long c0 = (long)blockIdx.y * 8;
  const long ob = (long)n * oblocks + ob0 + cb;
  float m[8], r[8];
#pragma unroll
  for (int j = 0; j < 8; ++j) { m[j] = mean[c0 + j]; r[j] = rstd[c0 + j]; }
  float best[8];
  unsigned short w0[8], w1[8];
#pragma unroll
  for (int kp = 0; kp < 4; ++kp) {
    const long u = ((long)(2 * zo + (kp >> 1)) * H + (2 * yo + (kp & 1))) * W + 2 * xo;
    unsigned short e[2][8][3];
#pragma unroll
    for (int j = 0; j < 8; ++j) {
      const float2 xv = *reinterpret_cast<const float2*>(x + (c0 + j) * S + u);
      float t0 = (xv.x - m[j]) * r[j], t1 = (xv.y - m[j]) * r[j];
      t0 = t0 > 0.f ? t0 : t0 * slope;
      t1 = t1 > 0.f ? t1 : t1 * slope;
      asm("" : "+v"(t0), "+v"(t1));
      h2_split(t0 * sc, e[0][j]);
      h2_split(t1 * sc, e[1][j]);
    }
#pragma unroll
    for (int h = 0; h < 2; ++h) {
#pragma unroll
      for (int t = 0; t < 2; ++t) out[(ob * 2 + t) * S + u + h] = s3_unit(e[h], t);
      const int k = (kp >> 1) * 4 + (kp & 1) * 2 + h;
#pragma unroll
      for (int j = 0; j < 8; ++j) {
        const float val = (float)__builtin_bit_cast(_Float16, e[h][j][0]) + (float)__builtin_bit_cast(_Float16, e[h][j][1]);
        if (val > best[j] || k == 0) { best[j] = val; w0[j] = e[h][j][0]; w1[j] = e[h][j][1]; }
      }
    }
  }
  uint4 o0, o1;
  o0.x = w0[0] | ((unsigned)w0[1] << 16); o0.y = w0[2] | ((unsigned)w0[3] << 16); o0.z = w0[4] | ((unsigned)w0[5] << 16); o0.w = w0[6] | ((unsigned)w0[7] << 16);
  o1.x = w1[0] | ((unsigned)w1[1] << 16); o1.y = w1[2] | ((unsigned)w1[3] << 16); o1.z = w1[4] | ((unsigned)w1[5] << 16); o1.w = w1[6] | ((unsigned)w1[7] << 16);
  uint4* o = pooled + ((long)n * cblocks + cb) * 2 * So;
  o[v] = o0;
  o[So + v] = o1;
}

__global__ void __launch_bounds__(256) k_maxpool2_h2(const uint4* __restrict__ in, uint4* __restrict__ out, int cblocks, int iblocks, int D, int H,
                                                     int W) {
  const int Do = D / 2, Ho = H / 2, Wo = W / 2;
  const long So = (long)Do * Ho * Wo, S = (long)D * H * W;
  const long v = (long)blockIdx.x * 256 + threadIdx.x;
  if (v >= So) return;
  const int n = blockIdx.y / cblocks, cb = blockIdx.y % cblocks;
  const int xo = (int)(v % Wo), yo = (int)((v / Wo) % Ho), zo = (int)(v / ((long)Wo * Ho));
  const uint4* i0 = in + ((long)n * iblocks + cb) * 2 * S;
  float best[8];
  unsigned short t0[8], t1[8];
#pragma unroll
  for (int j = 0; j < 8; ++j) { best[j] = -3.0e38f; t0[j] = 0; t1[j] = 0; }
#pragma unroll
  for (int k = 0; k < 8; ++k) {
    const long u = ((long)(2 * zo + (k >> 2)) * H + (2 * yo + ((k >> 1) & 1))) * W + 2 * xo + (k & 1);
    const uint4 a = i0[u], b = i0[S + u];
    const unsigned aw[4] = {a.x, a.y, a.z, a.w}, bw[4] = {b.x, b.y, b.z, b.w};
#pragma unroll
    for (int j = 0; j < 8; ++j) {
      const unsigned short h0 = (unsigned short)(aw[j >> 1] >> ((j & 1) * 16)), h1 = (unsigned short)(bw[j >> 1] >> ((j & 1) * 16));
      const float val = (float)__builtin_bit_cast(_Float16, h0) + (float)__builtin_bit_cast(_Float16, h1);
      if (val > best[j] || k == 0) { best[j] = val; t0[j] = h0; t1[j] = h1; }
    }
  }
  uint4 o0, o1;
  o0.x = t0[0] | ((unsigned)t0[1] << 16); o0.y = t0[2] | ((unsigned)t0[3] << 16); o0.z = t0[4] | ((unsigned)t0[5] << 16); o0.w = t0[6] | ((unsigned)t0[7] << 16);
  o1.x = t1[0] | ((unsigned)t1[1] << 16); o1.y = t1[2] | ((unsigned)t1[3] << 16); o1.z = t1[4] | ((unsigned)t1[5] << 16); o1.w = t1[6] | ((unsigned)t1[7] << 16);
  uint4* o = out + ((long)n * cblocks + cb) * 2 * So;
  o[v] = o0;
  o[So + v] = o1;
}

}

int maxpool2_h2(const void* in, void* out, int N, int C, int ctot, int D, int H, int W, hipStream_t s) {
  if (C % 8 || ctot % 8 || (D | H | W) & 1) { set_error("maxpool2_h2: channels % 8, even extents"); return NC_ERR_SHAPE; }
  const long So = (long)(D / 2) * (H / 2) * (W / 2);
  hipLaunchKernelGGL(k_maxpool2_h2, dim3((unsigned)cdiv(So, 256), (unsigned)(N * C / 8)), dim3(256), 0, s, (const uint4*)in, (uint4*)out, C / 8, ctot / 8, D, H,
                     W);
  return check_launch("maxpool2_h2");
}

int h2_zero_cells(unsigned* cells, int n, hipStream_t s) {
  hipLaunchKernelGGL(k_set_cells, dim3(1), dim3(64), 0, s, cells, n, 0u);
  return check_launch("h2_zero_cells");
}
int h2_set_cell(unsigned* cell, float bound, hipStream_t s) {
  unsigned bits;
  static_assert(sizeof(bits) == sizeof(bound), "");
  __builtin_memcpy(&bits, &bound, 4);
  hipLaunchKernelGGL(k_set_cells, dim3(1), dim3(64), 0, s, cell, 1, bits);
  return check_launch("h2_set_cell");
}
int h2_absmax(const float* x, long n, unsigned* cell, hipStream_t s, unsigned* cell2) {
  if ((unsigned long long)x & 3) { set_error("h2_absmax: the tensor must be 4-byte aligned"); return NC_ERR_ARG; }
  long blocks = cdiv(n, 256 * 4 * 8);
  if (blocks > 1024) blocks = 1024;
  if (blocks < 1) blocks = 1;
  hipLaunchKernelGGL(k_absmax, dim3((unsigned)blocks), dim3(256), 0, s, x, n, cell, cell2);
  return check_launch("h2_absmax");
}
int split2h_into(const float* x, long xstride, void* xs, int N, int C, long S, int ctot, int c0, const unsigned* cell, hipStream_t s, unsigned* guard) {
  if (C % 8 || ctot % 8 || c0 % 8) { set_error("split2h: channels must be multiples of 8"); return NC_ERR_SHAPE; }
  long bx = cdiv(S, 256);
  const long ny = (long)N * C / 8;
  if (guard && h2_guard_on() && bx * ny > 4096) bx = cdiv(4096, ny) < bx ? cdiv(4096, ny) : bx;
  hipLaunchKernelGGL(k_split2h, dim3((unsigned)bx, (unsigned)ny), dim3(256), 0, s, x, (uint4*)xs, S, C / 8, ctot / 8, c0 / 8, xstride,
                     cell, h2_guard_on() ? guard : nullptr);
  return check_launch("split2h");
}

static std::atomic<int> g_guard{getenv("NC_H2_GUARD") ? atoi(getenv("NC_H2_GUARD")) : 1};
int h2_guard_mode() { const int f = frozen_guard(); return f >= 0 ? f : g_guard.load(); }
bool h2_guard_on() { return h2_guard_mode() != 0; }
namespace { unsigned long long* guard_stats_dev(); }
void h2_guard_set(int on) { g_guard = on == 2 ? 2 : on ? 1 : 0; if (on) (void)guard_stats_dev(); }
namespace {
std::mutex g_stats_mu;
unsigned long long* g_stats_host = nullptr;
unsigned long long* g_stats_dev = nullptr;
unsigned long long* guard_stats_dev() {
  std::lock_guard<std::mutex> lk(g_stats_mu);
  if (!g_stats_host) {
    void* h = nullptr;
    if (hipHostMalloc(&h, 64, hipHostMallocMapped | hipHostMallocPortable) != hipSuccess) { (void)hipGetLastError(); return nullptr; }
    __builtin_memset(h, 0, 64);
    void* d = nullptr;
    if (hipHostGetDevicePointer(&d, h, 0) != hipSuccess) { (void)hipGetLastError(); (void)hipHostFree(h); return nullptr; }
    g_stats_host = (unsigned long long*)h;
    g_stats_dev = (unsigned long long*)d;
  }
  return g_stats_dev;
}
}
int h2_guard_read(unsigned long long* out4, int reset) {
  std::lock_guard<std::mutex> lk(g_stats_mu);
  for (int i = 0; i < 4; ++i) {
    if (!g_stats_host) out4[i] = 0;
    else out4[i] = reset ? __atomic_exchange_n(g_stats_host + i, 0ull, __ATOMIC_RELAXED) : __atomic_load_n(g_stats_host + i, __ATOMIC_RELAXED);
  }
  return NC_OK;
}
int h2_guard_zero(unsigned* g, hipStream_t s, int nwords) {
  hipLaunchKernelGGL(k_set_cells, dim3(1), dim3(64), 0, s, g, nwords, 0u);
  return check_launch("h2_guard_zero");
}
int h2_guard_decide(unsigned* ga, unsigned* gb, unsigned* prior, unsigned* flag, bool can_flip, hipStream_t s, unsigned long long total_a) {
  if (!h2_guard_on() && !prior) return NC_OK;
  hipLaunchKernelGGL(k_h2_guard_decide, dim3(1), dim3(64), 0, s, ga, gb, prior, flag, can_flip ? 1 : 0, guard_stats_dev(), total_a);
  return check_launch("h2_guard_decide");
}
int h2_to_s3_if(const void* xh, void* xs, int N, int C, long S, const unsigned* cells, const unsigned* guard, hipStream_t s) {
  if (C % 8) { set_error("h2_to_s3: channels must be a multiple of 8"); return NC_ERR_SHAPE; }
  hipLaunchKernelGGL(k_h2_to_s3_if, dim3((unsigned)cdiv(S, 256), (unsigned)(N * C / 8)), dim3(256), 0, s, (const uint4*)xh, (uint4*)xs, S, C / 8, cells, guard);
  return check_launch("h2_to_s3_if");
}
int act_split2h(const float* x, const float* mean, const float* rstd, float slope, float* y, long ystride, void* ys, int N, int C, long S, int ctot,
                int c0, float bound, unsigned* cell, unsigned* cell2, hipStream_t s) {
  if (C % 8 || ctot % 8 || c0 % 8) { set_error("act_split2h: channels must be multiples of 8"); return NC_ERR_SHAPE; }
  unsigned bits;
  __builtin_memcpy(&bits, &bound, 4);
  hipLaunchKernelGGL(k_act_split2h, dim3((unsigned)cdiv(S, 256), (unsigned)(N * C / 8)), dim3(256), 0, s, x, mean, rstd, slope, y, ystride,
                     (uint4*)ys, S, C / 8, ctot / 8, c0 / 8, bits, cell, cell2);
  return check_launch("act_split2h");
}

int act_split2h_pool(const float* x, const float* mean, const float* rstd, float slope, void* ys, void* pooled, int N, int C, int D, int H, int W,
                     int ctot, int c0, float bound, unsigned* cell, hipStream_t s) {
  if (C % 8 || ctot % 8 || c0 % 8 || ((D | H | W) & 1)) { set_error("act_split2h_pool: channels % 8, even extents"); return NC_ERR_SHAPE; }
  if ((((uintptr_t)x) & 7) != 0) { set_error("act_split2h_pool: input not 8-byte aligned"); return NC_ERR_ARG; }
  unsigned bits;
  __builtin_memcpy(&bits, &bound, 4);
  const long So = (long)(D / 2) * (H / 2) * (W / 2);
  hipLaunchKernelGGL(k_act_split2h_pool, dim3((unsigned)cdiv(So, 256), (unsigned)(N * C / 8)), dim3(256), 0, s, x, mean, rstd, slope, (uint4*)ys,
                     (uint4*)pooled, D, H, W, C / 8, ctot / 8, c0 / 8, bits, cell);
  return check_launch("act_split2h_pool");
}

}
```

neuroclear_amd/csrc/h2_debug.hip:

```cpp
#include <cmath>

#include "common.hpp"

using namespace nc;

extern "C" {

size_t nc_h2_bytes(int N, int C, long S) {
  if (N < 1 || C < 1 || S < 1) return 0;
  return h2_cells_offset((size_t)N * C * S) + 256;
}
size_t nc_h2_cells_offset(size_t elems) { return h2_cells_offset(elems); }

static bool h2_part_ok(int N, int C, long S, int ctot, int c0) {
  return N >= 1 && C >= 8 && S >= 1 && C % 8 == 0 && ctot % 8 == 0 && c0 % 8 == 0 && c0 >= 0 && c0 + C <= ctot && (long)N * C / 8 <= 65535;
}

int nc_to_h2_debug(const float* x, long xstride, void* xs, int N, int C, long S, int ctot, int c0, unsigned* cell, float bound, unsigned* guard,
                   void* stream) {
  if (!x || !xs || !cell) { set_error("to_h2_debug: null pointer"); return NC_ERR_ARG; }
  if (!h2_part_ok(N, C, S, ctot, c0) || xstride < (long)C * S) { set_error("to_h2_debug: bad shape"); return NC_ERR_SHAPE; }
  hipStream_t s = (hipStream_t)stream;
  if (bound > 0.f) {
    if (int e = h2_set_cell(cell, bound, s)) return e;
  } else {
    if (int e = h2_zero_cells(cell, 1, s)) return e;
    for (int n = 0; n < N; ++n)
      if (int e = h2_absmax(x + (long)n * xstride, (long)C * S, cell, s)) return e;
  }
  if (guard)
    if (int e = h2_guard_zero(guard, s)) return e;
  return split2h_into(x, xstride, xs, N, C, S, ctot, c0, cell, s, guard);
}

int nc_act_split2h_debug(const float* x, const float* mean, const float* rstd, float slope, float* y, long ystride, void* ys, int N, int C, long S,
                         int ctot, int c0, float bound, unsigned* cell, unsigned* cell2, void* stream) {
  if (!x || !mean || !rstd || !ys) { set_error("act_split2h_debug: null pointer"); return NC_ERR_ARG; }
  if (!h2_part_ok(N, C, S, ctot, c0) || (y && ystride < (long)C * S) || !(bound > 0.f)) { set_error("act_split2h_debug: bad shape"); return NC_ERR_SHAPE; }
  return act_split2h(x, mean, rstd, slope, y, ystride, ys, N, C, S, ctot, c0, bound, cell, cell2, (hipStream_t)stream);
}

int nc_act_split2h_pool_debug(const float* x, const float* mean, const float* rstd, float slope, void* ys, void* pooled, int N, int C, int D, int H,
                              int W, int ctot, int c0, float bound, unsigned* cell, void* stream) {
  if (!x || !mean || !rstd || !ys || !pooled) { set_error("act_split2h_pool_debug: null pointer"); return NC_ERR_ARG; }
  if (D < 2 || H < 2 || W < 2 || !h2_part_ok(N, C, (long)D * H * W, ctot, c0) || !(bound > 0.f)) { set_error("act_split2h_pool_debug: bad shape"); return NC_ERR_SHAPE; }
  return act_split2h_pool(x, mean, rstd, slope, ys, pooled, N, C, D, H, W, ctot, c0, bound, cell, (hipStream_t)stream);
}

int nc_maxpool2_h2_debug(const void* in, void* out, int N, int C, int ctot, int D, int H, int W, void* stream) {
  if (!in || !out) { set_error("maxpool2_h2_debug: null pointer"); return NC_ERR_ARG; }
  if (D < 2 || H < 2 || W < 2 || !h2_part_ok(N, C, (long)D * H * W, ctot, 0)) { set_error("maxpool2_h2_debug: bad shape"); return NC_ERR_SHAPE; }
  return maxpool2_h2(in, out, N, C, ctot, D, H, W, (hipStream_t)stream);
}

int nc_h2_to_s3_if_debug(const void* xh, void* xs, int N, int C, long S, const unsigned* cells, const unsigned* guard, void* stream) {
  if (!xh || !xs || !cells) { set_error("h2_to_s3_if_debug: null pointer"); return NC_ERR_ARG; }
  if (!h2_part_ok(N, C, S, C, 0)) { set_error("h2_to_s3_if_debug: bad shape"); return NC_ERR_SHAPE; }
  return h2_to_s3_if(xh, xs, N, C, S, cells, guard, (hipStream_t)stream);
}

int nc_instnorm_act_bwd_dbias_h2_debug(const float* dy, const float* w1, const float* x, const float* mean, const float* rstd, float slope, void* dxs,
                                       float* dbias, int N, int C, long S, void* ws, size_t ws_bytes, unsigned* guard, void* stream) {
  if (w1) {
    if (N != 1) { set_error("instnorm_act_bwd_dbias_h2_debug: the rank-one form takes one sample"); return NC_ERR_ARG; }
    return instnorm_act_bwd_dbias_h2_rank1(dy, w1, x, mean, rstd, slope, dxs, dbias, C, S, ws, ws_bytes, stream, guard);
  }
  return instnorm_act_bwd_dbias_h2(dy, x, mean, rstd, slope, dxs, dbias, N, C, S, ws, ws_bytes, stream, guard);
}

static size_t al256(size_t b) { return (b + 255) & ~(size_t)255; }
size_t nc_convT_k2s2_split_h2_ws_bytes(int N, int C, int D, int H, int W, int K) {
  if (!convT_s3x_supported(N, C, D, H, W, K)) return 0;
  return al256(convT_s3x_ws_bytes(C, K)) + h2_cells_offset((size_t)N * C * D * H * W) + 256;
}
int nc_convT_k2s2_fwd_split_h2_debug(const float* x, const float* w, const float* bias, float* y, void* ys, int ys_ctot, int ys_c0, int N, int C,
                                     int D, int H, int W, int K, unsigned* out_cell, void* ws, size_t ws_bytes, void* stream) {
  if (!x || !w || !ys || !out_cell || !ws) { set_error("convT_k2s2_fwd_split_h2_debug: null pointer"); return NC_ERR_ARG; }
  if (!convT_s3x_supported(N, C, D, H, W, K) || ys_ctot % 8 || ys_c0 % 8 || ys_c0 < 0 || ys_c0 + K > ys_ctot) {
    set_error("convT_k2s2_fwd_split_h2_debug: shape not covered");
    return NC_ERR_SHAPE;
  }
  hipStream_t s = (hipStream_t)stream;
  if (int e = h2_zero_cells(out_cell, 1, s)) return e;
  if (int e = convT_h2_bound(w, bias, C, K, sqrtf((float)((long)D * H * W)), out_cell, s)) return e;
  return convT_fwd_split_h2(x, w, bias, y, ys, ys_ctot, ys_c0, N, C, D, H, W, K, out_cell, ws, ws_bytes, s);
}

}
```

neuroclear_amd/csrc/norm_act.hip:

```cpp
#include <cstdlib>

#include "common.hpp"
#include "s3_common.hpp"

namespace nc {

static constexpr int kMaxSplits = 64;

static int pick_splits(int NC, long S) {
  long want = cdiv(2048, NC);
  long cap = cdiv(S, 8192);
  long s = want < cap ? want : cap;
  if (s < 1) s = 1;
  if (s > kMaxSplits) s = kMaxSplits;
  return (int)s;
}

__device__ __forceinline__ void block_reduce2(double& a, double& b, double* out2) {
  __shared__ double red[2][4];
  for (int o = 32; o > 0; o >>= 1) {
    a += __shfl_down(a, o);
    b += __shfl_down(b, o);
  }
  const int lane = threadIdx.x & 63, wv = threadIdx.x >> 6;
// ... 216 lines not shown
  const float* pg = dy + inst * S;
  float* o = dx + inst * S;
  double s1 = 0.0, s2 = 0.0;
#pragma unroll 4
  for (int i = sub; i < S; i += G) {
    const float xh = (px[i] - m) * r;
    const float g = xh > 0.f ? pg[i] : pg[i] * slope;
    s1 += (double)g;
    s2 = fma((double)g, (double)xh, s2);
  }
  s1 = group_sum<G>(s1);
  s2 = group_sum<G>(s2);
  const float m1 = (float)(s1 / (double)S), m2 = (float)(s2 / (double)S);
  double rs = 0.0;
#pragma unroll 4
  for (int i = sub; i < S; i += G) {
    const float v = in_bwd_value(px[i], pg[i], m, r, m1, m2, slope);
    o[i] = v;
    rs += (double)v;
  }
  if (rowsum) {
    rs = group_sum<G>(rs);
    if (sub == 0) rowsum[inst] = rs;
  }
}

static inline bool rows_path(long S) {
  static const bool on = true;
  return on && S <= kRowsMaxS;
}

template <int MODE>
static void launch_fwd_rows(const float* x, long NC, long S, float eps, float slope, float* mean, float* rstd, float* y,
                            hipStream_t s) {
  if (S <= 256)
    hipLaunchKernelGGL((k_in_fwd_rows<16, MODE>), dim3((unsigned)cdiv(NC, 16)), dim3(256), 0, s, x, NC, (int)S, eps, slope, mean,
                       rstd, y);
  else
    hipLaunchKernelGGL((k_in_fwd_rows<64, MODE>), dim3((unsigned)cdiv(NC, 4)), dim3(256), 0, s, x, NC, (int)S, eps, slope, mean,
                       rstd, y);
}

static void launch_bwd_rows(const float* dy, const float* x, const float* mean, const float* rstd, float slope, long NC, long S,
                            float* dx, double* rowsum, hipStream_t s) {
  if (S <= 256)
    hipLaunchKernelGGL((k_in_bwd_rows<16>), dim3((unsigned)cdiv(NC, 16)), dim3(256), 0, s, dy, x, mean, rstd, slope, NC, (int)S, dx,
                       rowsum);
  else
    hipLaunchKernelGGL((k_in_bwd_rows<64>), dim3((unsigned)cdiv(NC, 4)), dim3(256), 0, s, dy, x, mean, rstd, slope, NC, (int)S, dx,
                       rowsum);
}

template <int DT>
__device__ __forceinline__ unsigned short cvt16n(float f) {
  if constexpr (DT == NC_DT_F16) {
    const _Float16 v = (_Float16)f;
    return __builtin_bit_cast(unsigned short, v);
  } else {
    const __bf16 v = (__bf16)f;
    return __builtin_bit_cast(unsigned short, v);
  }
}
__device__ __forceinline__ uint4 pack8(const unsigned short (&e)[8]) {
  uint4 o;
  o.x = e[0] | ((unsigned)e[1] << 16); o.y = e[2] | ((unsigned)e[3] << 16);
  o.z = e[4] | ((unsigned)e[5] << 16); o.w = e[6] | ((unsigned)e[7] << 16);
  return o;
}

template <int DT>
__global__ __launch_bounds__(256) void k_in_act_fwd_c8(const float* __restrict__ x, const float* __restrict__ mean,
                                                       const float* __restrict__ rstd, float slope, float* __restrict__ y,
                                                       uint4* __restrict__ yh, long S) {
  const long ncb = blockIdx.y;
  float m[8], r[8];
#pragma unroll
  for (int j = 0; j < 8; ++j) { m[j] = mean[ncb * 8 + j]; r[j] = rstd[ncb * 8 + j]; }
  const float* px = x + ncb * 8 * S;
  float* py = y ? y + ncb * 8 * S : nullptr;
  for (long v = (long)blockIdx.x * 256 + threadIdx.x; v < S; v += (long)gridDim.x * 256) {
    unsigned short e[8];
#pragma unroll
    for (int j = 0; j < 8; ++j) {
      float t = (px[j * S + v] - m[j]) * r[j];
      t = t > 0.f ? t : t * slope;
      if (py) py[j * S + v] = t;
      e[j] = cvt16n<DT>(t);
    }
    yh[ncb * S + v] = pack8(e);
  }
}

template <int DT>
__global__ __launch_bounds__(256) void k_in_bwd_apply_c8(const float* __restrict__ dy, const float* __restrict__ x,
                                                         const float* __restrict__ mean, const float* __restrict__ rstd,
                                                         float slope, long S, int splits, const double* __restrict__ part,
                                                         float* __restrict__ dx, uint4* __restrict__ dxh,
                                                         double* __restrict__ rowpart) {
  __shared__ float sm[2][8];
  __shared__ double red[8][4];
  const long ncb = blockIdx.y;
  if (threadIdx.x < 8) {
    const long inst = ncb * 8 + threadIdx.x;
    double s1 = 0.0, s2 = 0.0;
    for (int k = 0; k < splits; ++k) {
      s1 += part[(inst * splits + k) * 2];
      s2 += part[(inst * splits + k) * 2 + 1];
    }
    sm[0][threadIdx.x] = (float)(s1 / (double)S);
    sm[1][threadIdx.x] = (float)(s2 / (double)S);
  }
  __syncthreads();
  float m[8], r[8], m1[8], m2[8];
#pragma unroll
  for (int j = 0; j < 8; ++j) { m[j] = mean[ncb * 8 + j]; r[j] = rstd[ncb * 8 + j]; m1[j] = sm[0][j]; m2[j] = sm[1][j]; }
  const float* px = x + ncb * 8 * S;
  const float* pg = dy + ncb * 8 * S;
  float* o = dx + ncb * 8 * S;
  double rs[8];
#pragma unroll
  for (int j = 0; j < 8; ++j) rs[j] = 0.0;
  for (long v = (long)blockIdx.x * 256 + threadIdx.x; v < S; v += (long)gridDim.x * 256) {
    unsigned short e[8];
#pragma unroll
    for (int j = 0; j < 8; ++j) {
      const float t = in_bwd_value(px[j * S + v], pg[j * S + v], m[j], r[j], m1[j], m2[j], slope);
      o[j * S + v] = t;
      rs[j] += (double)t;
      e[j] = cvt16n<DT>(t);
    }
    dxh[ncb * S + v] = pack8(e);
  }
  if (rowpart) {
    const int lane = threadIdx.x & 63, wv = threadIdx.x >> 6;
#pragma unroll
    for (int j = 0; j < 8; ++j) {
      double a = rs[j];
      for (int of = 32; of > 0; of >>= 1) a += __shfl_down(a, of);
      if (lane == 0) red[j][wv] = a;
    }
    __syncthreads();
    if (threadIdx.x < 8)
      rowpart[(ncb * 8 + threadIdx.x) * gridDim.x + blockIdx.x] =
          (red[threadIdx.x][0] + red[threadIdx.x][1]) + (red[threadIdx.x][2] + red[threadIdx.x][3]);
  }
}

__device__ __forceinline__ float r1_product(float w, float s) {
  float g = __builtin_fmaf(w, s, 0.f);
  asm("" : "+v"(g));
  return g;
}

template <bool R1 = false>
__global__ __launch_bounds__(256) void k_in_bwd_apply_s3(const float* __restrict__ dy, const float* __restrict__ x,
                                                         const float* __restrict__ mean, const float* __restrict__ rstd,
                                                         float slope, long S, int splits, const double* __restrict__ part,
                                                         uint4* __restrict__ dxs, int cblocks, double* __restrict__ rowpart,
                                                         const unsigned* __restrict__ guard = nullptr, const float* __restrict__ w1 = nullptr) {
  __shared__ float sm[2][8];
  __shared__ double red[8][4];
  if (guard_skip(guard, 1)) return;
  const long ncb = blockIdx.y;
  if (threadIdx.x < 8) {
    const long inst = ncb * 8 + threadIdx.x;
    double s1 = 0.0, s2 = 0.0;
    for (int k = 0; k < splits; ++k) {
      s1 += part[(inst * splits + k) * 2];
      s2 += part[(inst * splits + k) * 2 + 1];
    }
    sm[0][threadIdx.x] = (float)(s1 / (double)S);
    sm[1][threadIdx.x] = (float)(s2 / (double)S);
  }
  __syncthreads();
  float m[8], r[8], m1[8], m2[8];
#pragma unroll
  for (int j = 0; j < 8; ++j) { m[j] = mean[ncb * 8 + j]; r[j] = rstd[ncb * 8 + j]; m1[j] = sm[0][j]; m2[j] = sm[1][j]; }
  const float* px = x + ncb * 8 * S;
  const float* pg = R1 ? dy : dy + ncb * 8 * S;
  float wj[8];
#pragma unroll
  for (int j = 0; j < 8; ++j) wj[j] = R1 ? w1[ncb * 8 + j] : 0.f;
  double rs[8];
#pragma unroll
  for (int j = 0; j < 8; ++j) rs[j] = 0.0;
  for (long v = (long)blockIdx.x * 256 + threadIdx.x; v < S; v += (long)gridDim.x * 256) {
    unsigned short e[8][3];
    const float sv = R1 ? pg[v] : 0.f;
#pragma unroll
    for (int j = 0; j < 8; ++j) {
      const float t = in_bwd_value(px[j * S + v], R1 ? r1_product(wj[j], sv) : pg[j * S + v], m[j], r[j], m1[j], m2[j], slope);
      rs[j] += (double)t;
      s3_split(t, e[j]);
    }
#pragma unroll
    for (int t = 0; t < 3; ++t) dxs[(ncb * 3 + t) * S + v] = s3_unit(e, t);
  }
  if (rowpart) {
    const int lane = threadIdx.x & 63, wv = threadIdx.x >> 6;
#pragma unroll
    for (int j = 0; j < 8; ++j) {
      double a = rs[j];
      for (int of = 32; of > 0; of >>= 1) a += __shfl_down(a, of);
      if (lane == 0) red[j][wv] = a;
    }
    __syncthreads();
    if (threadIdx.x < 8)
      rowpart[(ncb * 8 + threadIdx.x) * gridDim.x + blockIdx.x] =
          (red[threadIdx.x][0] + red[threadIdx.x][1]) + (red[threadIdx.x][2] + red[threadIdx.x][3]);
  }
}

template <bool R1 = false>
__global__ __launch_bounds__(256) void k_in_bwd_sums_h2(const float* __restrict__ dy, const float* __restrict__ x, const float* __restrict__ mean,
                                                        const float* __restrict__ rstd, float slope, long S, int splits,
                                                        double* __restrict__ part, unsigned* __restrict__ gmax, unsigned* __restrict__ xmax,
                                                        const float* __restrict__ w1 = nullptr) {
  const int inst = blockIdx.y, sp = blockIdx.x;
  long b, e;
  chunk_range(S, splits, sp, b, e);
  const float m = mean[inst], r = rstd[inst];
  const float* px = x + (long)inst * S;
  const float* pg = R1 ? dy : dy + (long)inst * S;
  const float w = R1 ? w1[inst] : 0.f;
  double s1 = 0.0, s2 = 0.0;
  unsigned gm = 0, xm = 0;
  for (long i = b + threadIdx.x; i < e; i += 256) {
    const float xh = (px[i] - m) * r;
    const float gy = R1 ? r1_product(w, pg[i]) : pg[i];
    const float g = xh > 0.f ? gy : gy * slope;
    s1 += (double)g;
    s2 = fma((double)g, (double)xh, s2);
    const unsigned gb = __float_as_uint(g) & 0x7fffffffu, xb = __float_as_uint(xh) & 0x7fffffffu;
    if (gb < 0x7f800000u && gb > gm) gm = gb;
    if (xb < 0x7f800000u && xb > xm) xm = xb;
  }
#pragma unroll
  for (int o = 32; o > 0; o >>= 1) {
    const unsigned q1 = (unsigned)__shfl_xor((int)gm, o), q2 = (unsigned)__shfl_xor((int)xm, o);
    gm = q1 > gm ? q1 : gm; xm = q2 > xm ? q2 : xm;
  }
  if ((threadIdx.x & 63) == 0) {
    if (gm) atomicMax(gmax + inst, gm);
    if (xm) atomicMax(xmax + inst, xm);
  }
  block_reduce2(s1, s2, part + ((long)inst * splits + sp) * 2);
}

__global__ __launch_bounds__(256) void k_in_bwd_bound(const float* __restrict__ rstd, const unsigned* __restrict__ gmax,
                                                      const unsigned* __restrict__ xmax, int NC, unsigned* __restrict__ cell,
                                                      unsigned* __restrict__ cell2, unsigned* __restrict__ guard) {
  if (guard && threadIdx.x < 8) guard[threadIdx.x] = 0u;
  unsigned m = 0;
  for (int i = threadIdx.x; i < NC; i += 256) {
    const float bnd = rstd[i] * __uint_as_float(gmax[i]) * (2.f + __uint_as_float(xmax[i]));
    const unsigned b = __float_as_uint(bnd) & 0x7fffffffu;
    if (b < 0x7f800000u && b > m) m = b;
  }
#pragma unroll
  for (int o = 32; o > 0; o >>= 1) {
    const unsigned q = (unsigned)__shfl_xor((int)m, o);
    m = q > m ? q : m;
  }
  if ((threadIdx.x & 63) == 0 && m) {
    atomicMax(cell, m);
    atomicMax(cell2, m);
  }
}

__global__ void k_zero_u32(unsigned* p, int n) {
  for (int i = blockIdx.x * blockDim.x + threadIdx.x; i < n; i += gridDim.x * blockDim.x) p[i] = 0u;
}

template <bool R1 = false>
__global__ __launch_bounds__(256) void k_in_bwd_apply_h2(const float* __restrict__ dy, const float* __restrict__ x,
                                                         const float* __restrict__ mean, const float* __restrict__ rstd,
                                                         float slope, long S, int splits, const double* __restrict__ part,
                                                         uint4* __restrict__ dxs, int cblocks, double* __restrict__ rowpart,
                                                         const unsigned* __restrict__ cell, unsigned* __restrict__ guard,
                                                         const float* __restrict__ w1 = nullptr) {
  __shared__ float sm[2][8];
  __shared__ double red[8][4];
  const long ncb = blockIdx.y;
  if (threadIdx.x < 8) {
    const long inst = ncb * 8 + threadIdx.x;
    double s1 = 0.0, s2 = 0.0;
    for (int k = 0; k < splits; ++k) {
      s1 += part[(inst * splits + k) * 2];
      s2 += part[(inst * splits + k) * 2 + 1];
    }
    sm[0][threadIdx.x] = (float)(s1 / (double)S);
    sm[1][threadIdx.x] = (float)(s2 / (double)S);
  }
  __syncthreads();
  const unsigned cbits = *cell;
  const float sc = h2_scale(cbits);
  unsigned n_zero = 0, n_low = 0;
  float m[8], r[8], m1[8], m2[8];
#pragma unroll
  for (int j = 0; j < 8; ++j) { m[j] = mean[ncb * 8 + j]; r[j] = rstd[ncb * 8 + j]; m1[j] = sm[0][j]; m2[j] = sm[1][j]; }
  const float* px = x + ncb * 8 * S;
  const float* pg = R1 ? dy : dy + ncb * 8 * S;
  float wj[8];
#pragma unroll
  for (int j = 0; j < 8; ++j) wj[j] = R1 ? w1[ncb * 8 + j] : 0.f;
  double rs[8];
#pragma unroll
  for (int j = 0; j < 8; ++j) rs[j] = 0.0;
  for (long v = (long)blockIdx.x * 256 + threadIdx.x; v < S; v += (long)gridDim.x * 256) {
    unsigned short e[8][3];
    unsigned mx = 0;
    const float sv = R1 ? pg[v] : 0.f;
#pragma unroll
    for (int j = 0; j < 8; ++j) {
      float t = in_bwd_value(px[j * S + v], R1 ? r1_product(wj[j], sv) : pg[j * S + v], m[j], r[j], m1[j], m2[j], slope);
      rs[j] += (double)t;
      asm("" : "+v"(t));
      const unsigned b = __float_as_uint(t) & 0x7fffffffu;
      if (b < 0x7f800000u && b > mx) mx = b;
      h2_split(t * sc, e[j]);
    }
#pragma unroll
    for (int t = 0; t < 2; ++t) dxs[(ncb * 2 + t) * S + v] = s3_unit(e, t);
    if (guard) {
      const unsigned thr = cbits > kGuardDrop ? cbits - kGuardDrop : 0u;
      const bool any_hi = __builtin_amdgcn_ballot_w64(mx >= thr && mx != 0) != 0;
      const bool any_nz = __builtin_amdgcn_ballot_w64(mx != 0) != 0;
      if (!any_nz) ++n_zero;
      else if (!any_hi) ++n_low;
    }
  }
  if (guard && (threadIdx.x & 63) == 0) {
    if (n_low) atomicAdd(guard + kGuardLow, n_low);
    if (n_zero) atomicAdd(guard + kGuardAll, n_zero);
  }
  if (rowpart) {
    const int lane = threadIdx.x & 63, wv = threadIdx.x >> 6;
#pragma unroll
    for (int j = 0; j < 8; ++j) {
      double a = rs[j];
      for (int of = 32; of > 0; of >>= 1) a += __shfl_down(a, of);
      if (lane == 0) red[j][wv] = a;
    }
    __syncthreads();
    if (threadIdx.x < 8)
      rowpart[(ncb * 8 + threadIdx.x) * gridDim.x + blockIdx.x] =
          (red[threadIdx.x][0] + red[threadIdx.x][1]) + (red[threadIdx.x][2] + red[threadIdx.x][3]);
  }
}


__global__ void k_lrelu_fwd(const float* __restrict__ x, float slope, float* __restrict__ y, long n) {
  for (long i = (long)blockIdx.x * blockDim.x + threadIdx.x; i < n; i += (long)gridDim.x * blockDim.x) {
    const float v = x[i];
    y[i] = v > 0.f ? v : v * slope;
  }
}
__global__ void k_lrelu_bwd(const float* __restrict__ dy, const float* __restrict__ x, float slope,
                            float* __restrict__ dx, long n) {
  for (long i = (long)blockIdx.x * blockDim.x + threadIdx.x; i < n; i += (long)gridDim.x * blockDim.x)
    dx[i] = x[i] > 0.f ? dy[i] : dy[i] * slope;
}
__global__ void __launch_bounds__(256) k_in_act_tail(const float* __restrict__ x, const float* __restrict__ mean, const float* __restrict__ rstd,
                                                     const float* __restrict__ w1, const float* __restrict__ b1, const float* __restrict__ w2,
                                                     const float* __restrict__ b2, float* __restrict__ y, long S, int C) {
  __shared__ float sm[3][256];
  for (int c = threadIdx.x; c < C; c += 256) { sm[0][c] = mean[c]; sm[1][c] = rstd[c]; sm[2][c] = w1[c]; }
  __syncthreads();
  const long v = (long)blockIdx.x * 256 + threadIdx.x;
  if (v >= S) return;
  float acc = 0.f;
  for (int c = 0; c < C; ++c) {
    float t = (x[(long)c * S + v] - sm[0][c]) * sm[1][c];
    t = t > 0.f ? t : 0.f;
    acc = fmaf(sm[2][c], t, acc);
  }
  const float t1 = acc + b1[0];
  const float t2 = fmaf(w2[0], t1, b2[0]);
  y[v] = 1.f / (1.f + expf(-t2));
}

__global__ void k_sigmoid_fwd(const float* __restrict__ x, float* __restrict__ y, long n) {
  for (long i = (long)blockIdx.x * blockDim.x + threadIdx.x; i < n; i += (long)gridDim.x * blockDim.x)
    y[i] = 1.f / (1.f + expf(-x[i]));
}
__global__ void k_sigmoid_bwd(const float* __restrict__ dy, const float* __restrict__ y, float* __restrict__ dx,
                              long n) {
  for (long i = (long)blockIdx.x * blockDim.x + threadIdx.x; i < n; i += (long)gridDim.x * blockDim.x) {
    const float s = y[i];
    dx[i] = dy[i] * s * (1.f - s);
  }
}

__global__ void k_maxpool2_fwd(const float* __restrict__ x, float* __restrict__ y, int NC, int D, int H, int W, int Do,
                               int Ho, int Wo, int wd) {
  const long total = (long)NC * Do * Ho * Wo;
  for (long i = (long)blockIdx.x * blockDim.x + threadIdx.x; i < total; i += (long)gridDim.x * blockDim.x) {
    const int ow = (int)(i % Wo), oh = (int)((i / Wo) % Ho), od = (int)((i / ((long)Wo * Ho)) % Do);
    const long nc = i / ((long)Wo * Ho * Do);
    const float* p = x + nc * D * H * W;
    float best = -INFINITY;
    for (int a = 0; a < wd; ++a)
      for (int b = 0; b < 2; ++b)
        for (int c = 0; c < 2; ++c) {
          const float v = p[((long)(od * wd + a) * H + (oh * 2 + b)) * W + ow * 2 + c];
          if (v > best || v != v) best = v;
        }
    y[i] = best;
  }
}

template <bool SKIP>
__global__ void k_maxpool2_bwd(const float* __restrict__ dy, const float* __restrict__ x, const float* __restrict__ skip,
                               float* __restrict__ dx, int NC, int D, int H, int W, int Do, int Ho, int Wo, int wd) {
  const long total = (long)NC * Do * Ho * Wo;
  for (long i = (long)blockIdx.x * blockDim.x + threadIdx.x; i < total; i += (long)gridDim.x * blockDim.x) {
    const int ow = (int)(i % Wo), oh = (int)((i / Wo) % Ho), od = (int)((i / ((long)Wo * Ho)) % Do);
    const long nc = i / ((long)Wo * Ho * Do);
    const float* p = x + nc * D * H * W;
    float* q = dx + nc * D * H * W;
    float best = -INFINITY;
    int arg = 0;
    for (int a = 0; a < wd; ++a)
      for (int b = 0; b < 2; ++b)
        for (int c = 0; c < 2; ++c) {
          const float v = p[((long)(od * wd + a) * H + (oh * 2 + b)) * W + ow * 2 + c];
          if (v > best || v != v) {
            best = v;
            arg = (a * 2 + b) * 2 + c;
          }
        }
    const float g = dy[i];
    for (int a = 0; a < wd; ++a)
      for (int b = 0; b < 2; ++b)
        for (int c = 0; c < 2; ++c) {
          const long o = ((long)(od * wd + a) * H + (oh * 2 + b)) * W + ow * 2 + c;
          const float v = ((a * 2 + b) * 2 + c) == arg ? g : 0.f;
          q[o] = SKIP ? skip[nc * D * H * W + o] + v : v;
        }
  }
}

static unsigned flat_grid(long n, int per_block = 256) {
  long b = cdiv(n, per_block);
  if (b > 16384) b = 16384;
  if (b < 1) b = 1;
  return (unsigned)b;
}

}

using namespace nc;

__global__ void k_bn_finalize(const double* __restrict__ part, int N, int C, int splits, long S, float eps, float momentum,
                              float* __restrict__ mean, float* __restrict__ rstd, float* __restrict__ running_mean,
                              float* __restrict__ running_var) {
  const int c = blockIdx.x * blockDim.x + threadIdx.x;
  if (c >= C) return;
  double s = 0.0, q = 0.0;
  for (int n = 0; n < N; ++n)
    for (int k = 0; k < splits; ++k) {
      s += part[(((long)n * C + c) * splits + k) * 2];
      q += part[(((long)n * C + c) * splits + k) * 2 + 1];
    }
  const double M = (double)N * (double)S;
  const double m = s / M;
  double var = q / M - m * m;
  if (var < 0.0) var = 0.0;
// ... 113 lines not shown
  hipLaunchKernelGGL(k_in_stats, dim3(splits, NC), dim3(256), 0, s, x, S, splits, (double*)ws);
  hipLaunchKernelGGL(k_in_finalize, dim3((unsigned)cdiv(NC, 128)), dim3(128), 0, s, (const double*)ws, NC, splits, S, eps,
                     mean, rstd);
  return check_launch("instnorm_stats");
}

int nc_instnorm_act_fwd(const float* x, const float* mean, const float* rstd, float slope, float* y, int NC, long S,
                        void* stream) {
  if (!x || !mean || !rstd || !y) { set_error("instnorm_act_fwd: null pointer"); return NC_ERR_ARG; }
  if (NC >= 1 && S >= 1 && rows_path(S)) {
    launch_fwd_rows<1>(x, NC, S, 0.f, slope, const_cast<float*>(mean), const_cast<float*>(rstd), y, (hipStream_t)stream);
    return check_launch("instnorm_act_fwd");
  }
  if (NC > 65535) {
    for (int c0 = 0; c0 < NC; c0 += 65535) {
      const int n = NC - c0 < 65535 ? NC - c0 : 65535;
      if (int e = nc_instnorm_act_fwd(x + (long)c0 * S, mean + c0, rstd + c0, slope, y + (long)c0 * S, n, S, stream)) return e;
    }
    return NC_OK;
  }
  if (NC < 1 || S < 1) { set_error("instnorm_act_fwd: bad shape"); return NC_ERR_SHAPE; }
  long bx = cdiv(S, 1024 * 4);
  if (bx > 1024) bx = 1024;
  hipLaunchKernelGGL(k_in_act_fwd, dim3((unsigned)bx, NC), dim3(256), 0, (hipStream_t)stream, x, mean, rstd, slope, y, S);
  return check_launch("instnorm_act_fwd");
}

int nc_instnorm_fwd(const float* x, float eps, float slope, float* mean, float* rstd, float* y, int NC, long S, void* ws,
                    size_t ws_bytes, void* stream) {
  if (!x || !mean || !rstd || !y) { set_error("instnorm_fwd: null pointer"); return NC_ERR_ARG; }
  if (NC < 1 || S < 1) { set_error("instnorm_fwd: bad shape NC=%d S=%ld", NC, S); return NC_ERR_SHAPE; }
  if (rows_path(S)) {
    launch_fwd_rows<2>(x, NC, S, eps, slope, mean, rstd, y, (hipStream_t)stream);
    return check_launch("instnorm_fwd");
  }
  if (int e = nc_instnorm_stats(x, NC, S, eps, mean, rstd, ws, ws_bytes, stream)) return e;
  return nc_instnorm_act_fwd(x, mean, rstd, slope, y, NC, S, stream);
}

int nc_instnorm_act_bwd(const float* dy, const float* x, const float* mean, const float* rstd, float slope, float* dx,
                        int NC, long S, void* ws, size_t ws_bytes, void* stream) {
  if (!dy || !x || !mean || !rstd || !dx) { set_error("instnorm_act_bwd: null pointer"); return NC_ERR_ARG; }
  if (NC >= 1 && S >= 1 && rows_path(S)) {
    launch_bwd_rows(dy, x, mean, rstd, slope, NC, S, dx, nullptr, (hipStream_t)stream);
    return check_launch("instnorm_act_bwd");
  }
  if (NC > 65535) {
    for (int c0 = 0; c0 < NC; c0 += 65535) {
      const int n = NC - c0 < 65535 ? NC - c0 : 65535;
      if (int e = nc_instnorm_act_bwd(dy + (long)c0 * S, x + (long)c0 * S, mean + c0, rstd + c0, slope, dx + (long)c0 * S, n, S, ws,
                                      ws_bytes, stream)) return e;
    }
    return NC_OK;
  }
  if (NC < 1 || S < 1) { set_error("instnorm_act_bwd: bad shape"); return NC_ERR_SHAPE; }
  if (!ws || ws_bytes < nc_instnorm_ws_bytes(NC, S)) { set_error("instnorm_act_bwd: workspace too small"); return NC_ERR_WS; }
  hipStream_t s = (hipStream_t)stream;
  const int splits = pick_splits(NC, S);
  hipLaunchKernelGGL(k_in_bwd_sums, dim3(splits, NC), dim3(256), 0, s, dy, x, mean, rstd, slope, S, splits, (double*)ws);
  long bx = cdiv(S, 1024);
  if (bx > 1024) bx = 1024;
  hipLaunchKernelGGL(k_in_bwd_apply, dim3((unsigned)bx, NC), dim3(256), 0, s, dy, x, mean, rstd, slope, S, splits,
                     (const double*)ws, dx, (double*)nullptr);
  return check_launch("instnorm_act_bwd");
}

size_t nc_instnorm_bwd_dbias_ws_bytes(int NC, long S) {
  long bx = cdiv(S, 1024);
  if (bx > 1024) bx = 1024;
  return nc_instnorm_ws_bytes(NC, S) + (size_t)NC * bx * sizeof(double);
}

int nc_instnorm_act_bwd_dbias(const float* dy, const float* x, const float* mean, const float* rstd, float slope, float* dx,
                              float* dbias, int N, int C, long S, void* ws, size_t ws_bytes, void* stream) {
  if (!dy || !x || !mean || !rstd || !dx || !dbias) { set_error("instnorm_act_bwd_dbias: null pointer"); return NC_ERR_ARG; }
  const long NCl = (long)N * C;
  if (N < 1 || C < 1 || S < 1 || NCl > 0x7fffffffL) { set_error("instnorm_act_bwd_dbias: bad shape"); return NC_ERR_SHAPE; }
  hipStream_t s = (hipStream_t)stream;
  if (rows_path(S)) {
    if (!ws || ws_bytes < (size_t)NCl * sizeof(double)) { set_error("instnorm_act_bwd_dbias: workspace too small"); return NC_ERR_WS; }
    launch_bwd_rows(dy, x, mean, rstd, slope, NCl, S, dx, (double*)ws, s);
    hipLaunchKernelGGL(k_in_dbias_final, dim3(C), dim3(256), 0, s, (const double*)ws, N, C, 1, dbias);
    return check_launch("instnorm_act_bwd_dbias");
  }
  if (NCl > 65535) { set_error("instnorm_act_bwd_dbias: more than 65535 long instances"); return NC_ERR_SHAPE; }
  const int NC = (int)NCl;
  if (!ws || ws_bytes < nc_instnorm_bwd_dbias_ws_bytes(NC, S)) { set_error("instnorm_act_bwd_dbias: workspace too small"); return NC_ERR_WS; }
  const int splits = pick_splits(NC, S);
  double* rowpart = (double*)((char*)ws + nc_instnorm_ws_bytes(NC, S));
  hipLaunchKernelGGL(k_in_bwd_sums, dim3(splits, NC), dim3(256), 0, s, dy, x, mean, rstd, slope, S, splits, (double*)ws);
  long bx = cdiv(S, 1024);
  if (bx > 1024) bx = 1024;
  hipLaunchKernelGGL(k_in_bwd_apply, dim3((unsigned)bx, NC), dim3(256), 0, s, dy, x, mean, rstd, slope, S, splits,
                     (const double*)ws, dx, rowpart);
  hipLaunchKernelGGL(k_in_dbias_final, dim3(C), dim3(256), 0, s, (const double*)rowpart, N, C, (int)bx, dbias);
  return check_launch("instnorm_act_bwd_dbias");
}

int nc_instnorm_act_fwd_c8(const float* x, const float* mean, const float* rstd, float slope, float* y, void* yh, int N, int C,
                           long S, int dtype, void* stream) {
  if (!x || !mean || !rstd || !yh) { set_error("instnorm_act_fwd_c8: null pointer"); return NC_ERR_ARG; }
  if (N < 1 || C < 8 || C % 8 || S < 1 || (long)N * C / 8 > 65535) { set_error("instnorm_act_fwd_c8: bad shape"); return NC_ERR_SHAPE; }
  if (dtype != NC_DT_F16 && dtype != NC_DT_BF16) { set_error("instnorm_act_fwd_c8: dtype must be NC_DT_F16 or NC_DT_BF16"); return NC_ERR_ARG; }
  long bx = cdiv(S, 256);
  if (bx > 2048) bx = 2048;
  dim3 grid((unsigned)bx, (unsigned)(N * C / 8));
  if (dtype == NC_DT_F16)
    hipLaunchKernelGGL(k_in_act_fwd_c8<NC_DT_F16>, grid, dim3(256), 0, (hipStream_t)stream, x, mean, rstd, slope, y, (uint4*)yh, S);
  else
    hipLaunchKernelGGL(k_in_act_fwd_c8<NC_DT_BF16>, grid, dim3(256), 0, (hipStream_t)stream, x, mean, rstd, slope, y, (uint4*)yh, S);
  return check_launch("instnorm_act_fwd_c8");
}

int nc_instnorm_act_bwd_c8(const float* dy, const float* x, const float* mean, const float* rstd, float slope, float* dx,
                           void* dxh, float* dbias, int N, int C, long S, int dtype, void* ws, size_t ws_bytes, void* stream) {
  if (!dy || !x || !mean || !rstd || !dx || !dxh) { set_error("instnorm_act_bwd_c8: null pointer"); return NC_ERR_ARG; }
  const long NCl = (long)N * C;
  if (N < 1 || C < 8 || C % 8 || S < 1 || NCl > 65535) { set_error("instnorm_act_bwd_c8: bad shape"); return NC_ERR_SHAPE; }
  if (dtype != NC_DT_F16 && dtype != NC_DT_BF16) { set_error("instnorm_act_bwd_c8: dtype must be NC_DT_F16 or NC_DT_BF16"); return NC_ERR_ARG; }
  const int NC = (int)NCl;
  if (!ws || ws_bytes < nc_instnorm_bwd_dbias_ws_bytes(NC, S)) { set_error("instnorm_act_bwd_c8: workspace too small"); return NC_ERR_WS; }
  hipStream_t s = (hipStream_t)stream;
  const int splits = pick_splits(NC, S);
  hipLaunchKernelGGL(k_in_bwd_sums, dim3(splits, NC), dim3(256), 0, s, dy, x, mean, rstd, slope, S, splits, (double*)ws);
  long bx = cdiv(S, 1024);
  if (bx > 1024) bx = 1024;
  double* rowpart = dbias ? (double*)((char*)ws + nc_instnorm_ws_bytes(NC, S)) : nullptr;
  dim3 grid((unsigned)bx, (unsigned)(NC / 8));
  if (dtype == NC_DT_F16)
    hipLaunchKernelGGL(k_in_bwd_apply_c8<NC_DT_F16>, grid, dim3(256), 0, s, dy, x, mean, rstd, slope, S, splits,
                       (const double*)ws, dx, (uint4*)dxh, rowpart);
  else
    hipLaunchKernelGGL(k_in_bwd_apply_c8<NC_DT_BF16>, grid, dim3(256), 0, s, dy, x, mean, rstd, slope, S, splits,
                       (const double*)ws, dx, (uint4*)dxh, rowpart);
  if (dbias) hipLaunchKernelGGL(k_in_dbias_final, dim3(C), dim3(256), 0, s, (const double*)rowpart, N, C, (int)bx, dbias);
  return check_launch("instnorm_act_bwd_c8");
}

}
namespace nc {
bool instnorm_bwd_s3_supported(int N, int C, long S) { return N >= 1 && C >= 8 && C % 8 == 0 && S >= 1 && !rows_path(S) && (long)N * C <= 65535; }
int instnorm_act_bwd_dbias_s3(const float* dy, const float* x, const float* mean, const float* rstd, float slope, void* dxs,
                              float* dbias, int N, int C, long S, void* ws, size_t ws_bytes, void* stream) {
  if (!dy || !x || !mean || !rstd || !dxs || !dbias) { set_error("instnorm_act_bwd_dbias_s3: null pointer"); return NC_ERR_ARG; }
  if (!instnorm_bwd_s3_supported(N, C, S)) { set_error("instnorm_act_bwd_dbias_s3: bad shape"); return NC_ERR_SHAPE; }
  const int NC = N * C;
  if (!ws || ws_bytes < nc_instnorm_bwd_dbias_ws_bytes(NC, S)) { set_error("instnorm_act_bwd_dbias_s3: workspace too small"); return NC_ERR_WS; }
  hipStream_t s = (hipStream_t)stream;
  const int splits = pick_splits(NC, S);
  hipLaunchKernelGGL(k_in_bwd_sums, dim3(splits, NC), dim3(256), 0, s, dy, x, mean, rstd, slope, S, splits, (double*)ws);
  long bx = cdiv(S, 1024);
  if (bx > 1024) bx = 1024;
  double* rowpart = (double*)((char*)ws + nc_instnorm_ws_bytes(NC, S));
  hipLaunchKernelGGL(k_in_bwd_apply_s3<false>, dim3((unsigned)bx, (unsigned)(NC / 8)), dim3(256), 0, s, dy, x, mean, rstd, slope, S, splits,
                     (const double*)ws, (uint4*)dxs, C / 8, rowpart, (const unsigned*)nullptr, (const float*)nullptr);
  hipLaunchKernelGGL(k_in_dbias_final, dim3(C), dim3(256), 0, s, (const double*)rowpart, N, C, (int)bx, dbias);
  return check_launch("instnorm_act_bwd_dbias_s3");
}
static int in_bwd_dbias_h2(const float* dy, const float* w1, const float* x, const float* mean, const float* rstd, float slope, void* dxs,
                           float* dbias, int N, int C, long S, void* ws, size_t ws_bytes, void* stream, unsigned* guard) {
  if (!dy || !x || !mean || !rstd || !dxs || !dbias) { set_error("instnorm_act_bwd_dbias_h2: null pointer"); return NC_ERR_ARG; }
  if (!instnorm_bwd_s3_supported(N, C, S)) { set_error("instnorm_act_bwd_dbias_h2: bad shape"); return NC_ERR_SHAPE; }
  const int NC = N * C;
  if (w1 && N != 1) { set_error("instnorm_act_bwd_dbias_h2: the rank-one form takes one sample"); return NC_ERR_ARG; }
  if (!ws || ws_bytes < nc_instnorm_bwd_dbias_ws_bytes(NC, S)) { set_error("instnorm_act_bwd_dbias_h2: workspace too small"); return NC_ERR_WS; }
  if ((size_t)NC * S * 2 < 512 + (size_t)NC * 8) { set_error("instnorm_act_bwd_dbias_h2: tensor too small"); return NC_ERR_SHAPE; }
  hipStream_t s = (hipStream_t)stream;
  unsigned* cells = (unsigned*)((char*)dxs + h2_cells_offset((size_t)NC * S));
  unsigned* gmax = cells + 64;
  unsigned* xmax = gmax + NC;
  hipLaunchKernelGGL(k_zero_u32, dim3((unsigned)cdiv(64 + 2 * NC, 256)), dim3(256), 0, s, cells, 64 + 2 * NC);
  const int splits = pick_splits(NC, S);
  if (w1)
    hipLaunchKernelGGL(k_in_bwd_sums_h2<true>, dim3(splits, NC), dim3(256), 0, s, dy, x, mean, rstd, slope, S, splits, (double*)ws, gmax, xmax, w1);
  else
    hipLaunchKernelGGL(k_in_bwd_sums_h2<false>, dim3(splits, NC), dim3(256), 0, s, dy, x, mean, rstd, slope, S, splits, (double*)ws, gmax, xmax,
                       (const float*)nullptr);
  hipLaunchKernelGGL(k_in_bwd_bound, dim3(1), dim3(256), 0, s, rstd, gmax, xmax, NC, cells, cells + 1, guard);
  long bx = cdiv(S, 1024);
  if (bx > 1024) bx = 1024;
  double* rowpart = (double*)((char*)ws + nc_instnorm_ws_bytes(NC, S));
  unsigned* g = guard && h2_guard_on() ? guard : nullptr;
  if (w1)
    hipLaunchKernelGGL(k_in_bwd_apply_h2<true>, dim3((unsigned)bx, (unsigned)(NC / 8)), dim3(256), 0, s, dy, x, mean, rstd, slope, S, splits,
                       (const double*)ws, (uint4*)dxs, C / 8, rowpart, (const unsigned*)cells, g, w1);
  else
    hipLaunchKernelGGL(k_in_bwd_apply_h2<false>, dim3((unsigned)bx, (unsigned)(NC / 8)), dim3(256), 0, s, dy, x, mean, rstd, slope, S, splits,
                       (const double*)ws, (uint4*)dxs, C / 8, rowpart, (const unsigned*)cells, g, (const float*)nullptr);
  hipLaunchKernelGGL(k_in_dbias_final, dim3(C), dim3(256), 0, s, (const double*)rowpart, N, C, (int)bx, dbias);
  if (g) {
    const unsigned long long total = (unsigned long long)(NC / 8) * (unsigned long long)cdiv(S, 64);
    const bool flip = h2_guard_can_flip();
    if (int e = h2_guard_decide(g, nullptr, nullptr, g + kGuardFlag, flip, s, total)) return e;
    if (!flip) return check_launch("instnorm_act_bwd_dbias_h2");
    long bx3 = bx < 128 ? bx : 128;
    if (w1)
      hipLaunchKernelGGL(k_in_bwd_apply_s3<true>, dim3((unsigned)bx3, (unsigned)(NC / 8)), dim3(256), 0, s, dy, x, mean, rstd, slope, S, splits,
                         (const double*)ws, (uint4*)dxs, C / 8, (double*)nullptr, (const unsigned*)g, w1);
    else
      hipLaunchKernelGGL(k_in_bwd_apply_s3<false>, dim3((unsigned)bx3, (unsigned)(NC / 8)), dim3(256), 0, s, dy, x, mean, rstd, slope, S, splits,
                         (const double*)ws, (uint4*)dxs, C / 8, (double*)nullptr, (const unsigned*)g, (const float*)nullptr);
  }
  return check_launch("instnorm_act_bwd_dbias_h2");
}
int instnorm_act_bwd_dbias_h2(const float* dy, const float* x, const float* mean, const float* rstd, float slope, void* dxs,
                              float* dbias, int N, int C, long S, void* ws, size_t ws_bytes, void* stream, unsigned* guard) {
  return in_bwd_dbias_h2(dy, nullptr, x, mean, rstd, slope, dxs, dbias, N, C, S, ws, ws_bytes, stream, guard);
}
int instnorm_act_bwd_dbias_h2_rank1(const float* dy1, const float* w1, const float* x, const float* mean, const float* rstd, float slope, void* dxs,
                                    float* dbias, int C, long S, void* ws, size_t ws_bytes, void* stream, unsigned* guard) {
  if (!w1) { set_error("instnorm_act_bwd_dbias_h2_rank1: null pointer"); return NC_ERR_ARG; }
  return in_bwd_dbias_h2(dy1, w1, x, mean, rstd, slope, dxs, dbias, 1, C, S, ws, ws_bytes, stream, guard);
}
int instnorm_relu_tail_sigmoid(const float* x, const float* mean, const float* rstd, const float* w1, const float* b1, const float* w2,
                               const float* b2, float* y, int C, long S, hipStream_t s) {
  if (C > 256) { set_error("instnorm_relu_tail_sigmoid: at most 256 channels"); return NC_ERR_SHAPE; }
  hipLaunchKernelGGL(k_in_act_tail, dim3((unsigned)cdiv(S, 256)), dim3(256), 0, s, x, mean, rstd, w1, b1, w2, b2, y, S, C);
  return check_launch("instnorm_relu_tail_sigmoid");
}
}
extern "C" {

int nc_instnorm_act_bwd_dbias_s3(const float* dy, const float* x, const float* mean, const float* rstd, float slope, void* dxs, float* dbias,
                                 int N, int C, long S, void* ws, size_t ws_bytes, void* stream) {
  return instnorm_act_bwd_dbias_s3(dy, x, mean, rstd, slope, dxs, dbias, N, C, S, ws, ws_bytes, stream);
}

int nc_leaky_relu_fwd(const float* x, float slope, float* y, long n, void* stream) {
  if (!x || !y) { set_error("leaky_relu_fwd: null pointer"); return NC_ERR_ARG; }
  hipLaunchKernelGGL(k_lrelu_fwd, dim3(flat_grid(n)), dim3(256), 0, (hipStream_t)stream, x, slope, y, n);
  return check_launch("leaky_relu_fwd");
}
int nc_leaky_relu_bwd(const float* dy, const float* x, float slope, float* dx, long n, void* stream) {
  if (!dy || !x || !dx) { set_error("leaky_relu_bwd: null pointer"); return NC_ERR_ARG; }
  hipLaunchKernelGGL(k_lrelu_bwd, dim3(flat_grid(n)), dim3(256), 0, (hipStream_t)stream, dy, x, slope, dx, n);
  return check_launch("leaky_relu_bwd");
}
int nc_sigmoid_fwd(const float* x, float* y, long n, void* stream) {
  if (!x || !y) { set_error("sigmoid_fwd: null pointer"); return NC_ERR_ARG; }
  hipLaunchKernelGGL(k_sigmoid_fwd, dim3(flat_grid(n)), dim3(256), 0, (hipStream_t)stream, x, y, n);
  return check_launch("sigmoid_fwd");
}
int nc_sigmoid_bwd(const float* dy, const float* y, float* dx, long n, void* stream) {
  if (!dy || !y || !dx) { set_error("sigmoid_bwd: null pointer"); return NC_ERR_ARG; }
  hipLaunchKernelGGL(k_sigmoid_bwd, dim3(flat_grid(n)), dim3(256), 0, (hipStream_t)stream, dy, y, dx, n);
  return check_launch("sigmoid_bwd");
}

int nc_maxpool2_fwd(const float* x, float* y, int NC, int D, int H, int W, void* stream) {
  if (!x || !y) { set_error("maxpool2_fwd: null pointer"); return NC_ERR_ARG; }
  const int wd = D > 1 ? 2 : 1;
  const int Do = D / wd, Ho = H / 2, Wo = W / 2;
  if (NC < 1 || Do < 1 || Ho < 1 || Wo < 1) { set_error("maxpool2_fwd: bad shape"); return NC_ERR_SHAPE; }
  const long total = (long)NC * Do * Ho * Wo;
  hipLaunchKernelGGL(k_maxpool2_fwd, dim3(flat_grid(total)), dim3(256), 0, (hipStream_t)stream, x, y, NC, D, H, W, Do, Ho, Wo, wd);
  return check_launch("maxpool2_fwd");
}

int nc_maxpool2_bwd(const float* dy, const float* x, float* dx, int NC, int D, int H, int W, void* stream) {
  if (!dy || !x || !dx) { set_error("maxpool2_bwd: null pointer"); return NC_ERR_ARG; }
  const int wd = D > 1 ? 2 : 1;
  const int Do = D / wd, Ho = H / 2, Wo = W / 2;
  if (NC < 1 || Do < 1 || Ho < 1 || Wo < 1) { set_error("maxpool2_bwd: bad shape"); return NC_ERR_SHAPE; }
  hipStream_t s = (hipStream_t)stream;
  if ((D % wd) || (H & 1) || (W & 1)) {
    if (hipMemsetAsync(dx, 0, (size_t)NC * D * H * W * sizeof(float), s) != hipSuccess) {
      set_error("maxpool2_bwd: memset failed");
      return NC_ERR_HIP;
    }
  }
  const long total = (long)NC * Do * Ho * Wo;
  hipLaunchKernelGGL(k_maxpool2_bwd<false>, dim3(flat_grid(total)), dim3(256), 0, s, dy, x, nullptr, dx, NC, D, H, W, Do, Ho, Wo, wd);
  return check_launch("maxpool2_bwd");
}

int nc_maxpool2_bwd_add(const float* dy, const float* x, const float* skip, float* dx, int NC, int D, int H, int W,
                        void* stream) {
  if (!dy || !x || !skip || !dx) { set_error("maxpool2_bwd_add: null pointer"); return NC_ERR_ARG; }
  const int wd = D > 1 ? 2 : 1;
  const int Do = D / wd, Ho = H / 2, Wo = W / 2;
  if (NC < 1 || Do < 1 || Ho < 1 || Wo < 1 || (D % wd) || (H & 1) || (W & 1)) {
    set_error("maxpool2_bwd_add: even sizes expected (the skip tensor and the pooled tensor are the same tensor)");
    return NC_ERR_SHAPE;
  }
  const long total = (long)NC * Do * Ho * Wo;
  hipLaunchKernelGGL(k_maxpool2_bwd<true>, dim3(flat_grid(total)), dim3(256), 0, (hipStream_t)stream, dy, x, skip, dx, NC, D, H, W,
                     Do, Ho, Wo, wd);
  return check_launch("maxpool2_bwd_add");
}


int nc_batchnorm_stats(const float* x, int N, int C, long S, float eps, float momentum, int training, float* mean, float* rstd,
                       float* running_mean, float* running_var, void* ws, size_t ws_bytes, void* stream) {
  if (!x || !mean || !rstd) { set_error("batchnorm_stats: null pointer"); return NC_ERR_ARG; }
  if (N < 1 || C < 1 || S < 1 || C > 65535 || (long)N * C > 0x7fffffffL) { set_error("batchnorm_stats: bad shape N=%d C=%d S=%ld", N, C, S); return NC_ERR_SHAPE; }
  hipStream_t s = (hipStream_t)stream;
  if (!training) {
    if (!running_mean || !running_var) { set_error("batchnorm_stats: evaluation mode needs the running statistics"); return NC_ERR_ARG; }
    hipLaunchKernelGGL(k_bn_running, dim3((unsigned)cdiv(C, 128)), dim3(128), 0, s, running_mean, running_var, C, eps, mean, rstd);
    return check_launch("batchnorm_stats");
  }
  if (!ws || ws_bytes < nc_instnorm_ws_bytes(N * C, S)) { set_error("batchnorm_stats: workspace too small"); return NC_ERR_WS; }
  const int splits = pick_splits(N * C, S);
  for (long i0 = 0, step = (long)(65535 / C) * C; i0 < (long)N * C; i0 += step) {
    const int ni = (long)N * C - i0 < step ? (int)((long)N * C - i0) : (int)step;
    hipLaunchKernelGGL(k_in_stats, dim3(splits, ni), dim3(256), 0, s, x + i0 * S, S, splits, (double*)ws + i0 * splits * 2);
  }
  hipLaunchKernelGGL(k_bn_finalize, dim3((unsigned)cdiv(C, 128)), dim3(128), 0, s, (const double*)ws, N, C, splits, S, eps, momentum, mean, rstd,
                     running_mean, running_var);
  return check_launch("batchnorm_stats");
}
int nc_batchnorm_act_fwd(const float* x, const float* mean, const float* rstd, const float* gamma, const float* beta, float slope, float* y,
                         int N, int C, long S, void* stream) {
  if (!x || !mean || !rstd || !gamma || !beta || !y) { set_error("batchnorm_act_fwd: null pointer"); return NC_ERR_ARG; }
  if (N < 1 || C < 1 || S < 1 || C > 65535 || (long)N * C > 0x7fffffffL) { set_error("batchnorm_act_fwd: bad shape"); return NC_ERR_SHAPE; }
  long bx = cdiv(S, 1024 * 4);
  if (bx > 1024) bx = 1024;
  for (long i0 = 0, step = (long)(65535 / C) * C; i0 < (long)N * C; i0 += step) {
    const int ni = (long)N * C - i0 < step ? (int)((long)N * C - i0) : (int)step;
    hipLaunchKernelGGL(k_bn_act_fwd, dim3((unsigned)bx, ni), dim3(256), 0, (hipStream_t)stream, x + i0 * S, mean, rstd, gamma, beta, slope, y + i0 * S, C, S);
  }
  return check_launch("batchnorm_act_fwd");
}
int nc_batchnorm_act_bwd(const float* dy, const float* x, const float* mean, const float* rstd, const float* gamma, const float* beta,
                         float slope, int training, float* dx, float* dgamma, float* dbeta, float* coef, int N, int C, long S, void* ws,
                         size_t ws_bytes, void* stream) {
  if (!dy || !x || !mean || !rstd || !gamma || !beta || !dx || !dgamma || !dbeta || !coef) { set_error("batchnorm_act_bwd: null pointer"); return NC_ERR_ARG; }
  if (N < 1 || C < 1 || S < 1 || C > 65535 || (long)N * C > 0x7fffffffL) { set_error("batchnorm_act_bwd: bad shape"); return NC_ERR_SHAPE; }
  if (!ws || ws_bytes < nc_instnorm_ws_bytes(N * C, S)) { set_error("batchnorm_act_bwd: workspace too small"); return NC_ERR_WS; }
  hipStream_t s = (hipStream_t)stream;
  const int splits = pick_splits(N * C, S);
  const long NCl = (long)N * C, step = (long)(65535 / C) * C;
  for (long i0 = 0; i0 < NCl; i0 += step) {
    const int ni = NCl - i0 < step ? (int)(NCl - i0) : (int)step;
    hipLaunchKernelGGL(k_bn_bwd_sums, dim3(splits, ni), dim3(256), 0, s, dy + i0 * S, x + i0 * S, mean, rstd, gamma, beta, slope, C, S, splits,
                       (double*)ws + i0 * splits * 2);
  }
  hipLaunchKernelGGL(k_bn_bwd_finalize, dim3((unsigned)cdiv(C, 128)), dim3(128), 0, s, (const double*)ws, N, C, splits, S, dgamma, dbeta, coef);
  long bx = cdiv(S, 1024 * 4);
  if (bx > 1024) bx = 1024;
  for (long i0 = 0; i0 < NCl; i0 += step) {
    const int ni = NCl - i0 < step ? (int)(NCl - i0) : (int)step;
    hipLaunchKernelGGL(k_bn_bwd_apply, dim3((unsigned)bx, ni), dim3(256), 0, s, dy + i0 * S, x + i0 * S, mean, rstd, gamma, beta, slope, coef, training,
                       dx + i0 * S, C, S);
  }
  return check_launch("batchnorm_act_bwd");
}
}
```

Measured before the change: 55.59 million.

## Fuse maxpool into UNet encoder activation and skip fp32 concat writes

Adds a default-on pool mode for the UNet encoder. The activation split kernel now computes the 2x pooling directly, writing pooled fp32 output and per-window argmax indices in place of the separate maxpool pass. The convT decoder stages no longer write their fp32 skip-concat halves. In backward, the norm kernels take the pooled gradient through the stored indices, and the fp32 concat buffers are rebuilt only when needed. This cuts forward memory traffic and kernel launches, but adds backward-side recompute in some configurations and more complicated kernel templates.

```diff
diff --git a/include/nc_hip.h b/include/nc_hip.h
--- a/include/nc_hip.h
+++ b/include/nc_hip.h
@@ -178,6 +178,9 @@
                        float* dparams, int N, int S0, int S1, int S2, void* ws, size_t ws_bytes, void* stream, unsigned kept);
 void nc_set_unet_lean(int on);
 int nc_get_unet_lean(void);
+void nc_set_unet_pool(int on);
+int nc_get_unet_pool(void);
+int nc_unet_deconv_saved_offset(int N, int S0, int S1, int S2, int which, size_t* offset, size_t* bytes);
 void nc_set_unet_wprep(int on);
 int nc_get_unet_wprep(void);
 int nc_unet_wprep_layout(int N, int S0, int S1, int S2, int block, int form, size_t* pack_off, size_t* pack_bytes, size_t* cell_off,
@@ -291,6 +294,11 @@
 int nc_h2_to_s3_if_debug(const void* xh, void* xs, int N, int C, long S, const unsigned* cells, const unsigned* guard, void* stream);
 int nc_instnorm_act_bwd_dbias_h2_debug(const float* dy, const float* w1, const float* x, const float* mean, const float* rstd, float slope, void* dxs,
                                        float* dbias, int N, int C, long S, void* ws, size_t ws_bytes, unsigned* guard, void* stream);
+int nc_act_split2h_pool_arg_debug(const float* x, const float* mean, const float* rstd, float slope, void* ys, void* pooled, int N, int C, int D,
+                                  int H, int W, int ctot, int c0, float bound, unsigned* cell, unsigned char* widx, float* pooled_f32, void* stream);
+int nc_instnorm_act_bwd_dbias_h2_pool_debug(const float* skip, long skip_stride, const float* dyp, const unsigned char* widx, int D, int H, int W,
+                                            const float* x, const float* mean, const float* rstd, float slope, void* dxs, float* dbias, int N, int C,
+                                            void* ws, size_t ws_bytes, unsigned* guard, void* stream);
 size_t nc_convT_k2s2_split_h2_ws_bytes(int N, int C, int D, int H, int W, int K);
 int nc_convT_k2s2_fwd_split_h2_debug(const float* x, const float* w, const float* bias, float* y, void* ys, int ys_ctot, int ys_c0, int N, int C,
                                      int D, int H, int W, int K, unsigned* out_cell, void* ws, size_t ws_bytes, void* stream);
diff --git a/neuroclear_amd/_lib.py b/neuroclear_amd/_lib.py
--- a/neuroclear_amd/_lib.py
+++ b/neuroclear_amd/_lib.py
@@ -32,7 +32,7 @@
                 fn.restype = ctypes.c_size_t
             elif name == 'nc_last_error':
                 fn.restype = ctypes.c_char_p
-            elif name in ('nc_set_force_direct', 'nc_prof_begin', 'nc_sconv_set_cfg', 'nc_sconv_set_tune', 'nc_set_conv_split', 'nc_set_s3_fusion', 'nc_set_c8x_mode', 'nc_set_split_terms', 'nc_set_h2_guard', 'nc_set_epi_stats', 'nc_set_dl_collapse', 'nc_set_p2d_terms', 'nc_set_s3x_w64', 'nc_set_unet_lean', 'nc_set_unet_wprep'):
+            elif name in ('nc_set_force_direct', 'nc_prof_begin', 'nc_sconv_set_cfg', 'nc_sconv_set_tune', 'nc_set_conv_split', 'nc_set_s3_fusion', 'nc_set_c8x_mode', 'nc_set_split_terms', 'nc_set_h2_guard', 'nc_set_epi_stats', 'nc_set_dl_collapse', 'nc_set_p2d_terms', 'nc_set_s3x_w64', 'nc_set_unet_lean', 'nc_set_unet_wprep', 'nc_set_unet_pool'):
                 fn.restype = None
             else:
                 fn.restype = ctypes.c_int
diff --git a/neuroclear_amd/csrc/common.hpp b/neuroclear_amd/csrc/common.hpp
--- a/neuroclear_amd/csrc/common.hpp
+++ b/neuroclear_amd/csrc/common.hpp
@@ -232,6 +232,9 @@
                               float* dbias, int N, int C, long S, void* ws, size_t ws_bytes, void* stream, unsigned* guard = nullptr);
 int instnorm_act_bwd_dbias_h2_rank1(const float* dy1, const float* w1, const float* x, const float* mean, const float* rstd, float slope, void* dxs,
                                     float* dbias, int C, long S, void* ws, size_t ws_bytes, void* stream, unsigned* guard);
+int instnorm_act_bwd_dbias_h2_pool(const float* skip, long skip_stride, const float* dyp, const unsigned char* idx, int D, int H, int W, const float* x,
+                                   const float* mean, const float* rstd, float slope, void* dxs, float* dbias, int N, int C, void* ws, size_t ws_bytes,
+                                   void* stream, unsigned* guard);
 unsigned* conv_bwd_guard_words(void* ws, int N, int K, long S);
 int maxpool2_h2(const void* in, void* out, int N, int C, int ctot, int D, int H, int W, hipStream_t s);
 int h2_zero_cells(unsigned* cells, int n, hipStream_t s);
@@ -259,7 +262,7 @@
 int act_split2h(const float* x, const float* mean, const float* rstd, float slope, float* y, long ystride, void* ys, int N, int C, long S, int ctot,
                 int c0, float bound, unsigned* cell, unsigned* cell2, hipStream_t s);
 int act_split2h_pool(const float* x, const float* mean, const float* rstd, float slope, void* ys, void* pooled, int N, int C, int D, int H, int W,
-                     int ctot, int c0, float bound, unsigned* cell, hipStream_t s);
+                     int ctot, int c0, float bound, unsigned* cell, hipStream_t s, unsigned char* widx = nullptr, float* pooled_f32 = nullptr);
 int conv_s3x(const void* xs, const float* w, const float* bias, float* y, int N, int Cin, int D, int H, int W, int Kout, int KS, long so,
              long si, int flip, void* wp_ws, hipStream_t s, const unsigned* guard = nullptr);
 bool conv_keep_supported(int N, int C, int D, int H, int W, int K, int ks);
diff --git a/neuroclear_amd/csrc/gen_nets.hip b/neuroclear_amd/csrc/gen_nets.hip
--- a/neuroclear_amd/csrc/gen_nets.hip
+++ b/neuroclear_amd/csrc/gen_nets.hip
@@ -22,6 +22,9 @@
   for (int j = 0; j < 5; ++j) if (kLeanBlocks[j] == consumer) return j;
   return -1;
 }
+
+std::atomic<int> g_unet_pool{getenv("NC_UNET_POOL") ? atoi(getenv("NC_UNET_POOL")) : 1};
+constexpr unsigned kKeptPool0 = 1u << 26, kKeptPool1 = 1u << 27, kKeptNoCat1 = 1u << 28, kKeptNoCat2 = 1u << 29;
 
 struct UBlock { int C, K, lvl; };
 const UBlock kUB[10] = {{1, 64, 0},    {64, 64, 0},    {64, 128, 1},  {128, 128, 1}, {128, 256, 2},
@@ -135,6 +138,22 @@
 
 void nc_set_unet_wprep(int on) { g_unet_wprep.store(on != 0, std::memory_order_relaxed); }
 int nc_get_unet_wprep(void) { return g_unet_wprep.load(std::memory_order_relaxed); }
+void nc_set_unet_pool(int on) { g_unet_pool.store(on == 2 ? 2 : on != 0, std::memory_order_relaxed); }
+int nc_get_unet_pool(void) { return g_unet_pool.load(std::memory_order_relaxed); }
+int nc_unet_deconv_saved_offset(int N, int S0, int S1, int S2, int which, size_t* offset, size_t* bytes) {
+  UPlan p;
+  if (!u_plan(p, N, S0, S1, S2) || which < 1 || which > 13) { set_error("unet_deconv_saved_offset: bad argument"); return NC_ERR_ARG; }
+  const size_t n = (size_t)N, S = (size_t)p.S[0], Sh = (size_t)p.S[1], Sq = (size_t)p.S[2];
+  size_t off, b;
+  if (which <= 9) { off = p.xs3[which]; b = s3_floats(n * kUB[which].C * (size_t)p.S[kUB[which].lvl]); }
+  else if (which == 10) { off = p.cat1; b = n * 128 * S; }
+  else if (which == 11) { off = p.cat2; b = n * 256 * Sh; }
+  else if (which == 12) { off = p.p1; b = n * 64 * Sh; }
+  else { off = p.p2; b = n * 128 * Sq; }
+  if (offset) *offset = off * 4;
+  if (bytes) *bytes = b * 4;
+  return NC_OK;
+}
 void nc_set_unet_lean(int on) { g_unet_lean.store(on != 0, std::memory_order_relaxed); }
 int nc_get_unet_lean(void) { return g_unet_lean.load(std::memory_order_relaxed); }
 
@@ -217,6 +236,11 @@
   unsigned* cell7 = h2_cells_of(V + p.xs3[7], (size_t)N * 256 * Sh) + 1;
   unsigned* cell9 = h2_cells_of(V + p.xs3[9], (size_t)N * 128 * S) + 1;
   unsigned kept_mask = 0;
+  const int pool_mode = g_unet_pool.load(std::memory_order_relaxed);
+  const bool pool0 = pool_mode == 1 && h2l[1] && h2l[2] && ct1h, pool1 = pool_mode == 1 && h2l[3] && h2l[4] && ct2h;
+  const bool nocat1 = pool_mode != 0 && ct1h, nocat2 = pool_mode != 0 && ct2h;
+  if (nocat1) kept_mask |= kKeptNoCat1;
+  if (nocat2) kept_mask |= kKeptNoCat2;
   S3xPrepared prep[18] = {};
   bool bound7 = false, bound9 = false;
   if (g_unet_wprep.load(std::memory_order_relaxed) != 0) {
@@ -268,6 +292,13 @@
     }
     if (epi) NC_TRY(s3x_stats_finalize((const float*)iws, P + o.b[i], N, d[0], d[1], d[2], b.K, 3, 1e-5f, V + p.mean[i], V + p.rstd[i], hs));
     else NC_TRY(nc_instnorm_stats(V + p.raw[i], N * b.K, S, 1e-5f, V + p.mean[i], V + p.rstd[i], iws, p.in_ws, stream));
+    if (to >= 0 && use[to] && ((i == 1 && pool0) || (i == 3 && pool1))) {
+      NC_TRY(act_split2h_pool(V + p.raw[i], V + p.mean[i], V + p.rstd[i], 0.f, V + p.xs3[to], nullptr, N, b.K, d[0], d[1], d[2], to_ctot, 0,
+                              sqrtf((float)S), h2_cells_of(V + p.xs3[to], (size_t)N * to_ctot * S), hs, (unsigned char*)(V + (i == 1 ? p.cat1 : p.cat2)),
+                              V + (i == 1 ? p.p1 : p.p2)));
+      kept_mask |= i == 1 ? kKeptPool0 : kKeptPool1;
+      return NC_OK;
+    }
     if (to >= 0 && use[to]) {
       const int lj = lean && h2l[to] && to_ctot == b.K ? lean_index(to) : -1;
       if (lj >= 0) { out = nullptr; kept_mask |= 1u << (kLeanBit0 + lj); }
@@ -284,11 +315,11 @@
   };
   NC_TRY(block(0, x, V + p.a1, (size_t)64 * S, 1, 64));
   NC_TRY(block(1, V + p.a1, V + p.cat1, (size_t)128 * S, 9, 128));
-  for (int n = 0; n < N; ++n)
+  for (int n = 0; n < N && !pool0; ++n)
     NC_TRY(nc_maxpool2_fwd(V + p.cat1 + (size_t)n * 128 * S, V + p.p1 + (size_t)n * 64 * Sh, 64, d0[0], d0[1], d0[2], stream));
   NC_TRY(block(2, V + p.p1, V + p.a2, (size_t)128 * Sh, 3, 128));
   NC_TRY(block(3, V + p.a2, V + p.cat2, (size_t)256 * Sh, 7, 256));
-  for (int n = 0; n < N; ++n)
+  for (int n = 0; n < N && !pool1; ++n)
     NC_TRY(nc_maxpool2_fwd(V + p.cat2 + (size_t)n * 256 * Sh, V + p.p2 + (size_t)n * 128 * Sq, 128, d1[0], d1[1], d1[2], stream));
   NC_TRY(block(4, V + p.p2, V + p.b1, (size_t)256 * Sq, 5, 256));
   NC_TRY(block(5, V + p.b1, V + p.b2, (size_t)256 * Sq, 6, 256));
@@ -299,7 +330,7 @@
   }
   for (int n = 0; n < N; ++n) {
     if (ct2h)
-      NC_TRY(convT_fwd_split_h2(V + p.b3 + (size_t)n * 256 * Sq, P + o.w[10], P + o.b[10], V + p.cat2 + ((size_t)n * 256 + 128) * Sh,
+      NC_TRY(convT_fwd_split_h2(V + p.b3 + (size_t)n * 256 * Sq, P + o.w[10], P + o.b[10], nocat2 ? nullptr : V + p.cat2 + ((size_t)n * 256 + 128) * Sh,
                                 (char*)(V + p.xs3[7]) + (size_t)n * 256 * Sh * 4, 256, 128, 1, 256, d2[0], d2[1], d2[2], 128, cell7, cws, p.conv_ws, hs));
     else if (ct2)
       NC_TRY(nc_convT_k2s2_fwd_split(V + p.b3 + (size_t)n * 256 * Sq, nullptr, P + o.w[10], P + o.b[10], V + p.cat2 + ((size_t)n * 256 + 128) * Sh,
@@ -322,7 +353,7 @@
   }
   for (int n = 0; n < N; ++n) {
     if (ct1h)
-      NC_TRY(convT_fwd_split_h2(V + p.e2b + (size_t)n * 128 * Sh, P + o.w[11], P + o.b[11], V + p.cat1 + ((size_t)n * 128 + 64) * S,
+      NC_TRY(convT_fwd_split_h2(V + p.e2b + (size_t)n * 128 * Sh, P + o.w[11], P + o.b[11], nocat1 ? nullptr : V + p.cat1 + ((size_t)n * 128 + 64) * S,
                                 (char*)(V + p.xs3[9]) + (size_t)n * 128 * S * 4, 128, 64, 1, 128, d1[0], d1[1], d1[2], 64, cell9, cws, p.conv_ws, hs));
     else if (ct1)
       NC_TRY(nc_convT_k2s2_fwd_split(V + p.e2b + (size_t)n * 128 * Sh, nullptr, P + o.w[11], P + o.b[11], V + p.cat1 + ((size_t)n * 128 + 64) * S,
@@ -379,13 +410,25 @@
       off += s3x_packed_bytes(sg[k].Cin, sg[k].Kout, 3, 2);
     }
   }
-  auto block_bwd = [&](int i, const float* g, const float* in, float* draw, float* gin, bool r1 = false) -> int {
+  auto blk_now_h2 = [&](int i) {
+    ConvDims c;
+    return make_dims(c, N, kUB[i].C, p.d[kUB[i].lvl][0], p.d[kUB[i].lvl][1], p.d[kUB[i].lvl][2], kUB[i].K, 3, 3, 3, 1, 1) && conv_layer_h2(c);
+  };
+  auto blk_has_xs = [&](int i) {
+    return ((kept_mask >> i) & 1) && (((kept_mask >> (16 + i)) & 1) != 0) == blk_now_h2(i);
+  };
+  auto blk_fused = [&](int i, bool with_gin) {
+    const UBlock& b = kUB[i];
+    const int* d = p.d[b.lvl];
+    return fuse_bwd && i >= 1 && conv_bwd_pre_supported(N, b.C, d[0], d[1], d[2], b.K, 3, with_gin, p.conv_ws) && instnorm_bwd_s3_supported(N, b.K, p.S[b.lvl]);
+  };
+  struct PoolIn { const float* skip; long stride; const float* dyp; const unsigned char* idx; };
+  auto block_bwd = [&](int i, const float* g, const float* in, float* draw, float* gin, bool r1 = false, const PoolIn* pin = nullptr) -> int {
     const UBlock& b = kUB[i];
     const int* d = p.d[b.lvl];
     const long Sl = p.S[b.lvl];
-    ConvDims cdk;
-    const bool now_h2 = make_dims(cdk, N, b.C, d[0], d[1], d[2], b.K, 3, 3, 3, 1, 1) && conv_layer_h2(cdk);
-    const void* xs = ((kept_mask >> i) & 1) && (((kept_mask >> (16 + i)) & 1) != 0) == now_h2 ? (const void*)(V + p.xs3[i]) : nullptr;
+    const bool now_h2 = blk_now_h2(i);
+    const void* xs = blk_has_xs(i) ? (const void*)(V + p.xs3[i]) : nullptr;
     const S3xPrepared* pd = i >= 1 && gin && now_h2 && (kept_mask & kKeptWPrep) && ((kept_mask >> (16 + i)) & 1) && wprep_now ? &prepd[i] : nullptr;
     const int lj = lean_index(i);
     if (lj >= 0 && ((kept_mask >> (kLeanBit0 + lj)) & 1) &&
@@ -398,15 +441,19 @@
                                              stream, conv_bwd_guard_words(cws, N, b.K, Sl)));
       return conv_bwd_pre(in, xs, P + o.w[i], gin, DP + o.w[i], N, b.C, d[0], d[1], d[2], b.K, 3, cws, p.conv_ws, stream, h2_guard_can_flip(), pd);
     }
-    if (fuse_bwd && i >= 1 && conv_bwd_pre_supported(N, b.C, d[0], d[1], d[2], b.K, 3, gin != nullptr, p.conv_ws) &&
-        instnorm_bwd_s3_supported(N, b.K, Sl)) {
-      if (now_h2)
+    if (blk_fused(i, gin != nullptr)) {
+      if (now_h2 && pin)
+        NC_TRY(instnorm_act_bwd_dbias_h2_pool(pin->skip, pin->stride, pin->dyp, pin->idx, d[0], d[1], d[2], V + p.raw[i], V + p.mean[i], V + p.rstd[i], 0.f, cws,
+                                              DP + o.b[i], N, b.K, iws, p.in_ws, stream, conv_bwd_guard_words(cws, N, b.K, Sl)));
+      else if (pin) { set_error("unet_deconv_bwd: the pooled gradient form needs the two-term norm backward"); return NC_ERR_ARG; }
+      else if (now_h2)
         NC_TRY(instnorm_act_bwd_dbias_h2(g, V + p.raw[i], V + p.mean[i], V + p.rstd[i], 0.f, cws, DP + o.b[i], N, b.K, Sl, iws, p.in_ws, stream,
                                          conv_bwd_guard_words(cws, N, b.K, Sl)));
       else
         NC_TRY(instnorm_act_bwd_dbias_s3(g, V + p.raw[i], V + p.mean[i], V + p.rstd[i], 0.f, cws, DP + o.b[i], N, b.K, Sl, iws, p.in_ws, stream));
       return conv_bwd_pre(in, xs, P + o.w[i], gin, DP + o.w[i], N, b.C, d[0], d[1], d[2], b.K, 3, cws, p.conv_ws, stream, now_h2 && h2_guard_can_flip(), pd);
     }
+    if (pin) { set_error("unet_deconv_bwd: the pooled gradient form needs the two-term norm backward"); return NC_ERR_ARG; }
     NC_TRY(nc_instnorm_act_bwd_dbias(g, V + p.raw[i], V + p.mean[i], V + p.rstd[i], 0.f, draw, DP + o.b[i], N, b.K, Sl, iws,
                                      p.in_ws, stream));
     return conv_bwd_keep(in, xs, draw, P + o.w[i], gin, DP + o.w[i], N, b.C, d[0], d[1], d[2], b.K, 3, cws, p.conv_ws, stream);
@@ -418,6 +465,31 @@
     *out = G + p.T;
     return NC_OK;
   };
+  auto no_fp32 = [&](int i) { return blk_has_xs(i) && blk_now_h2(i) && !h2_guard_can_flip() && blk_fused(i, true); };
+  auto h2_norm_bwd = [&](int i) { return blk_now_h2(i) && blk_fused(i, true); };
+  float* VW = const_cast<float*>(saved);
+  const bool in9 = !no_fp32(9), in7 = !no_fp32(7);
+  const bool full0 = (kept_mask & kKeptPool0) && (in9 || !h2_norm_bwd(1));
+  const bool full1 = (kept_mask & kKeptPool1) && (in7 || !h2_norm_bwd(3));
+  const bool pform0 = (kept_mask & kKeptPool0) && !full0, pform1 = (kept_mask & kKeptPool1) && !full1;
+  if (full0)
+    for (int n = 0; n < N; ++n) {
+      NC_TRY(nc_instnorm_act_fwd(V + p.raw[1] + (size_t)n * 64 * S, V + p.mean[1] + n * 64, V + p.rstd[1] + n * 64, 0.f, VW + p.cat1 + (size_t)n * 128 * S, 64, S, stream));
+    }
+  if (full1)
+    for (int n = 0; n < N; ++n) {
+      NC_TRY(nc_instnorm_act_fwd(V + p.raw[3] + (size_t)n * 128 * Sh, V + p.mean[3] + n * 128, V + p.rstd[3] + n * 128, 0.f, VW + p.cat2 + (size_t)n * 256 * Sh, 128, Sh, stream));
+    }
+  if ((kept_mask & kKeptNoCat1) && in9)
+    for (int n = 0; n < N; ++n)
+      NC_TRY(convT_fwd_split_h2(V + p.e2b + (size_t)n * 128 * Sh, P + o.w[11], P + o.b[11], VW + p.cat1 + ((size_t)n * 128 + 64) * S,
+                                (char*)(VW + p.xs3[9]) + (size_t)n * 128 * S * 4, 128, 64, 1, 128, d1[0], d1[1], d1[2], 64,
+                                h2_cells_of(V + p.xs3[9], (size_t)N * 128 * S) + 1, cws, p.conv_ws, hs));
+  if ((kept_mask & kKeptNoCat2) && in7)
+    for (int n = 0; n < N; ++n)
+      NC_TRY(convT_fwd_split_h2(V + p.b3 + (size_t)n * 256 * Sq, P + o.w[10], P + o.b[10], VW + p.cat2 + ((size_t)n * 256 + 128) * Sh,
+                                (char*)(VW + p.xs3[7]) + (size_t)n * 256 * Sh * 4, 256, 128, 1, 256, d2[0], d2[1], d2[2], 128,
+                                h2_cells_of(V + p.xs3[7], (size_t)N * 256 * Sh) + 1, cws, p.conv_ws, hs));
   NC_TRY(nc_sigmoid_bwd(dy, y, G + p.s1, (long)N * S, stream));
   NC_TRY(nc_conv_wgrad(V + p.t1, G + p.s1, DP + o.w[13], DP + o.b[13], N, 1, d0[0], d0[1], d0[2], 1, 1, 1, 1, 1, 0, cws, p.conv_ws, stream));
   NC_TRY(nc_conv_dgrad(G + p.s1, P + o.w[13], G + p.s2, N, 1, d0[0], d0[1], d0[2], 1, 1, 1, 1, 1, 0, cws, p.conv_ws, stream));
@@ -442,15 +514,17 @@
   NC_TRY(block_bwd(6, G + p.Q1, V + p.b2, G + p.Q2, G + p.Q1));
   NC_TRY(block_bwd(5, G + p.Q1, V + p.b1, G + p.Q2, G + p.Q1));
   NC_TRY(block_bwd(4, G + p.Q1, V + p.p2, G + p.Q2, G + p.Q1));
-  for (int n = 0; n < N; ++n)
+  for (int n = 0; n < N && !pform1; ++n)
     NC_TRY(nc_maxpool2_bwd_add(G + p.Q1 + (size_t)n * 128 * Sq, V + p.cat2 + (size_t)n * 256 * Sh, G + p.H3 + (size_t)n * 256 * Sh,
                                G + p.H1 + (size_t)n * 128 * Sh, 128, d1[0], d1[1], d1[2], stream));
-  NC_TRY(block_bwd(3, G + p.H1, V + p.a2, G + p.H2, G + p.H1));
+  const PoolIn pin1{G + p.H3, (long)256 * Sh, G + p.Q1, (const unsigned char*)(V + p.cat2)};
+  NC_TRY(block_bwd(3, G + p.H1, V + p.a2, G + p.H2, G + p.H1, false, pform1 ? &pin1 : nullptr));
   NC_TRY(block_bwd(2, G + p.H1, V + p.p1, G + p.H2, G + p.H1));
-  for (int n = 0; n < N; ++n)
+  for (int n = 0; n < N && !pform0; ++n)
     NC_TRY(nc_maxpool2_bwd_add(G + p.H1 + (size_t)n * 64 * Sh, V + p.cat1 + (size_t)n * 128 * S, G + p.G3 + (size_t)n * 128 * S,
                                G + p.G1 + (size_t)n * 64 * S, 64, d0[0], d0[1], d0[2], stream));
-  NC_TRY(block_bwd(1, G + p.G1, V + p.a1, G + p.G2, G + p.G1));
+  const PoolIn pin0{G + p.G3, (long)128 * S, G + p.H1, (const unsigned char*)(V + p.cat1)};
+  NC_TRY(block_bwd(1, G + p.G1, V + p.a1, G + p.G2, G + p.G1, false, pform0 ? &pin0 : nullptr));
   return block_bwd(0, G + p.G1, x, G + p.G2, dx);
 }
 
diff --git a/neuroclear_amd/csrc/h2.hip b/neuroclear_amd/csrc/h2.hip
--- a/neuroclear_amd/csrc/h2.hip
+++ b/neuroclear_amd/csrc/h2.hip
@@ -178,9 +178,11 @@
   for (int t = 0; t < 2; ++t) out[(ob * 2 + t) * S + v] = s3_unit(e, t);
 }
 
+template <bool TR>
 __global__ void __launch_bounds__(256) k_act_split2h_pool(const float* __restrict__ x, const float* __restrict__ mean, const float* __restrict__ rstd,
                                                           float slope, uint4* __restrict__ out, uint4* __restrict__ pooled, int D, int H, int W,
-                                                          int cblocks, int oblocks, int ob0, unsigned bound_bits, unsigned* __restrict__ cell) {
+                                                          int cblocks, int oblocks, int ob0, unsigned bound_bits, unsigned* __restrict__ cell,
+                                                          unsigned char* __restrict__ widx, float* __restrict__ pf) {
   if (blockIdx.x == 0 && blockIdx.y == 0 && threadIdx.x == 0 && cell) *cell = bound_bits;
   const int Do = D / 2, Ho = H / 2, Wo = W / 2;
   const long So = (long)Do * Ho * Wo, S = (long)D * H * W;
@@ -196,6 +198,7 @@
   for (int j = 0; j < 8; ++j) { m[j] = mean[c0 + j]; r[j] = rstd[c0 + j]; }
   float best[8];
   unsigned short w0[8], w1[8];
+  unsigned char wk[8];
 #pragma unroll
   for (int kp = 0; kp < 4; ++kp) {
     const long u = ((long)(2 * zo + (kp >> 1)) * H + (2 * yo + (kp & 1))) * W + 2 * xo;
@@ -209,11 +212,18 @@
       asm("" : "+v"(t0), "+v"(t1));
       h2_split(t0 * sc, e[0][j]);
       h2_split(t1 * sc, e[1][j]);
+      if (TR) {
+        const int k0 = (kp >> 1) * 4 + (kp & 1) * 2;
+        if (kp == 0) { best[j] = -INFINITY; wk[j] = 0; }
+        if (t0 > best[j] || t0 != t0) { best[j] = t0; wk[j] = (unsigned char)k0; }
+        if (t1 > best[j] || t1 != t1) { best[j] = t1; wk[j] = (unsigned char)(k0 + 1); }
+      }
     }
 #pragma unroll
     for (int h = 0; h < 2; ++h) {
 #pragma unroll
       for (int t = 0; t < 2; ++t) out[(ob * 2 + t) * S + u + h] = s3_unit(e[h], t);
+      if (TR) continue;
       const int k = (kp >> 1) * 4 + (kp & 1) * 2 + h;
 #pragma unroll
       for (int j = 0; j < 8; ++j) {
@@ -221,6 +231,12 @@
         if (val > best[j] || k == 0) { best[j] = val; w0[j] = e[h][j][0]; w1[j] = e[h][j][1]; }
       }
     }
+  }
+  if (TR) {
+    const long o = ((long)n * cblocks + cb) * 8 * So + v;
+#pragma unroll
+    for (int j = 0; j < 8; ++j) { pf[o + j * So] = best[j]; widx[o + j * So] = wk[j]; }
+    return;
   }
   uint4 o0, o1;
   o0.x = w0[0] | ((unsigned)w0[1] << 16); o0.y = w0[2] | ((unsigned)w0[3] << 16); o0.z = w0[4] | ((unsigned)w0[5] << 16); o0.w = w0[6] | ((unsigned)w0[7] << 16);
@@ -358,14 +374,19 @@
 }
 
 int act_split2h_pool(const float* x, const float* mean, const float* rstd, float slope, void* ys, void* pooled, int N, int C, int D, int H, int W,
-                     int ctot, int c0, float bound, unsigned* cell, hipStream_t s) {
+                     int ctot, int c0, float bound, unsigned* cell, hipStream_t s, unsigned char* widx, float* pooled_f32) {
   if (C % 8 || ctot % 8 || c0 % 8 || ((D | H | W) & 1)) { set_error("act_split2h_pool: channels % 8, even extents"); return NC_ERR_SHAPE; }
   if ((((uintptr_t)x) & 7) != 0) { set_error("act_split2h_pool: input not 8-byte aligned"); return NC_ERR_ARG; }
   unsigned bits;
   __builtin_memcpy(&bits, &bound, 4);
   const long So = (long)(D / 2) * (H / 2) * (W / 2);
-  hipLaunchKernelGGL(k_act_split2h_pool, dim3((unsigned)cdiv(So, 256), (unsigned)(N * C / 8)), dim3(256), 0, s, x, mean, rstd, slope, (uint4*)ys,
-                     (uint4*)pooled, D, H, W, C / 8, ctot / 8, c0 / 8, bits, cell);
+  if ((widx != nullptr) != (pooled_f32 != nullptr)) { set_error("act_split2h_pool: winner bytes and fp32 pooled tensor come together"); return NC_ERR_ARG; }
+  if (widx)
+    hipLaunchKernelGGL(k_act_split2h_pool<true>, dim3((unsigned)cdiv(So, 256), (unsigned)(N * C / 8)), dim3(256), 0, s, x, mean, rstd, slope, (uint4*)ys,
+                       (uint4*)nullptr, D, H, W, C / 8, ctot / 8, c0 / 8, bits, cell, widx, pooled_f32);
+  else
+    hipLaunchKernelGGL(k_act_split2h_pool<false>, dim3((unsigned)cdiv(So, 256), (unsigned)(N * C / 8)), dim3(256), 0, s, x, mean, rstd, slope, (uint4*)ys,
+                       (uint4*)pooled, D, H, W, C / 8, ctot / 8, c0 / 8, bits, cell, widx, pooled_f32);
   return check_launch("act_split2h_pool");
 }
 
diff --git a/neuroclear_amd/csrc/h2_debug.hip b/neuroclear_amd/csrc/h2_debug.hip
--- a/neuroclear_amd/csrc/h2_debug.hip
+++ b/neuroclear_amd/csrc/h2_debug.hip
@@ -47,6 +47,20 @@
   return act_split2h_pool(x, mean, rstd, slope, ys, pooled, N, C, D, H, W, ctot, c0, bound, cell, (hipStream_t)stream);
 }
 
+int nc_act_split2h_pool_arg_debug(const float* x, const float* mean, const float* rstd, float slope, void* ys, void* pooled, int N, int C, int D,
+                                  int H, int W, int ctot, int c0, float bound, unsigned* cell, unsigned char* widx, float* pooled_f32, void* stream) {
+  if (!x || !mean || !rstd || !ys || (!pooled && !widx)) { set_error("act_split2h_pool_arg_debug: null pointer"); return NC_ERR_ARG; }
+  if (D < 2 || H < 2 || W < 2 || !h2_part_ok(N, C, (long)D * H * W, ctot, c0) || !(bound > 0.f)) { set_error("act_split2h_pool_arg_debug: bad shape"); return NC_ERR_SHAPE; }
+  return act_split2h_pool(x, mean, rstd, slope, ys, pooled, N, C, D, H, W, ctot, c0, bound, cell, (hipStream_t)stream, widx, pooled_f32);
+}
+
+int nc_instnorm_act_bwd_dbias_h2_pool_debug(const float* skip, long skip_stride, const float* dyp, const unsigned char* widx, int D, int H, int W,
+                                            const float* x, const float* mean, const float* rstd, float slope, void* dxs, float* dbias, int N, int C,
+                                            void* ws, size_t ws_bytes, unsigned* guard, void* stream) {
+  if (D < 1 || H < 1 || W < 1 || skip_stride < (long)C * D * H * W) { set_error("instnorm_act_bwd_dbias_h2_pool_debug: bad shape"); return NC_ERR_SHAPE; }
+  return instnorm_act_bwd_dbias_h2_pool(skip, skip_stride, dyp, widx, D, H, W, x, mean, rstd, slope, dxs, dbias, N, C, ws, ws_bytes, stream, guard);
+}
+
 int nc_maxpool2_h2_debug(const void* in, void* out, int N, int C, int ctot, int D, int H, int W, void* stream) {
   if (!in || !out) { set_error("maxpool2_h2_debug: null pointer"); return NC_ERR_ARG; }
   if (D < 2 || H < 2 || W < 2 || !h2_part_ok(N, C, (long)D * H * W, ctot, 0)) { set_error("maxpool2_h2_debug: bad shape"); return NC_ERR_SHAPE; }
diff --git a/neuroclear_amd/csrc/norm_act.hip b/neuroclear_amd/csrc/norm_act.hip
--- a/neuroclear_amd/csrc/norm_act.hip
+++ b/neuroclear_amd/csrc/norm_act.hip
@@ -392,12 +392,41 @@
   return g;
 }
 
-template <bool R1 = false>
+struct PoolG {
+  const float* dyp;
+  const unsigned char* idx;
+  long skip_stride, So;
+  int C, H, W, Ho, Wo;
+};
+struct PoolWalk {
+  int x, y, z, sx, sy, sz, H, W;
+  __device__ __forceinline__ PoolWalk() : x(0), y(0), z(0), sx(0), sy(0), sz(0), H(1), W(1) {}
+  __device__ __forceinline__ PoolWalk(long i0, long step, int H_, int W_) : H(H_), W(W_) {
+    x = (int)(i0 % W); long t = i0 / W; y = (int)(t % H); z = (int)(t / H);
+    sx = (int)(step % W); t = step / W; sy = (int)(t % H); sz = (int)(t / H);
+  }
+  __device__ __forceinline__ void next() {
+    x += sx; if (x >= W) { x -= W; ++y; }
+    y += sy; if (y >= H) { y -= H; ++z; }
+    z += sz;
+  }
+  __device__ __forceinline__ long cell(int Ho, int Wo) const { return ((long)(z >> 1) * Ho + (y >> 1)) * Wo + (x >> 1); }
+  __device__ __forceinline__ int k() const { return ((z & 1) << 2) | ((y & 1) << 1) | (x & 1); }
+};
+__device__ __forceinline__ float pool_grad(float skip, unsigned char win, float dyp, int k) {
+  float g = skip + ((int)win == k ? dyp : 0.f);
+  asm("" : "+v"(g));
+  return g;
+}
+
+template <int GF = 0>
 __global__ __launch_bounds__(256) void k_in_bwd_apply_s3(const float* __restrict__ dy, const float* __restrict__ x,
                                                          const float* __restrict__ mean, const float* __restrict__ rstd,
                                                          float slope, long S, int splits, const double* __restrict__ part,
                                                          uint4* __restrict__ dxs, int cblocks, double* __restrict__ rowpart,
-                                                         const unsigned* __restrict__ guard = nullptr, const float* __restrict__ w1 = nullptr) {
+                                                         const unsigned* __restrict__ guard = nullptr, const float* __restrict__ w1 = nullptr,
+                                                         PoolG pl = PoolG{}) {
+  constexpr bool R1 = GF == 1;
   __shared__ float sm[2][8];
   __shared__ double red[8][4];
   if (guard_skip(guard, 1)) return;
@@ -417,7 +446,11 @@
 #pragma unroll
   for (int j = 0; j < 8; ++j) { m[j] = mean[ncb * 8 + j]; r[j] = rstd[ncb * 8 + j]; m1[j] = sm[0][j]; m2[j] = sm[1][j]; }
   const float* px = x + ncb * 8 * S;
-  const float* pg = R1 ? dy : dy + ncb * 8 * S;
+  const float* pg = R1 ? dy : GF == 2 ? dy + (ncb / cblocks) * pl.skip_stride + (ncb % cblocks) * 8 * S : dy + ncb * 8 * S;
+  const float* pd = GF == 2 ? pl.dyp + ncb * 8 * pl.So : nullptr;
+  const unsigned char* pi = GF == 2 ? pl.idx + ncb * 8 * pl.So : nullptr;
+  PoolWalk wk;
+  if constexpr (GF == 2) wk = PoolWalk((long)blockIdx.x * 256 + threadIdx.x, (long)gridDim.x * 256, pl.H, pl.W);
   float wj[8];
 #pragma unroll
   for (int j = 0; j < 8; ++j) wj[j] = R1 ? w1[ncb * 8 + j] : 0.f;
@@ -427,9 +460,16 @@
   for (long v = (long)blockIdx.x * 256 + threadIdx.x; v < S; v += (long)gridDim.x * 256) {
     unsigned short e[8][3];
     const float sv = R1 ? pg[v] : 0.f;
+    long pc = 0;
+    int pk = 0;
+    if constexpr (GF == 2) { pc = wk.cell(pl.Ho, pl.Wo); pk = wk.k(); wk.next(); }
 #pragma unroll
     for (int j = 0; j < 8; ++j) {
-      const float t = in_bwd_value(px[j * S + v], R1 ? r1_product(wj[j], sv) : pg[j * S + v], m[j], r[j], m1[j], m2[j], slope);
+      float gy;
+      if constexpr (GF == 1) gy = r1_product(wj[j], sv);
+      else if constexpr (GF == 2) gy = pool_grad(pg[j * S + v], pi[j * pl.So + pc], pd[j * pl.So + pc], pk);
+      else gy = pg[j * S + v];
+      const float t = in_bwd_value(px[j * S + v], gy, m[j], r[j], m1[j], m2[j], slope);
       rs[j] += (double)t;
       s3_split(t, e[j]);
     }
@@ -451,30 +491,52 @@
   }
 }
 
-template <bool R1 = false>
+template <int GF = 0>
 __global__ __launch_bounds__(256) void k_in_bwd_sums_h2(const float* __restrict__ dy, const float* __restrict__ x, const float* __restrict__ mean,
                                                         const float* __restrict__ rstd, float slope, long S, int splits,
                                                         double* __restrict__ part, unsigned* __restrict__ gmax, unsigned* __restrict__ xmax,
-                                                        const float* __restrict__ w1 = nullptr) {
+                                                        const float* __restrict__ w1 = nullptr, PoolG pl = PoolG{}) {
+  constexpr bool R1 = GF == 1;
   const int inst = blockIdx.y, sp = blockIdx.x;
   long b, e;
   chunk_range(S, splits, sp, b, e);
   const float m = mean[inst], r = rstd[inst];
   const float* px = x + (long)inst * S;
-  const float* pg = R1 ? dy : dy + (long)inst * S;
+  const float* pg = R1 ? dy : GF == 2 ? dy + (long)(inst / pl.C) * pl.skip_stride + (long)(inst % pl.C) * S : dy + (long)inst * S;
+  const float* pd = GF == 2 ? pl.dyp + (long)inst * pl.So : nullptr;
+  const unsigned char* pi = GF == 2 ? pl.idx + (long)inst * pl.So : nullptr;
+  PoolWalk wk;
+  if constexpr (GF == 2) wk = PoolWalk(b + threadIdx.x, 256, pl.H, pl.W);
   const float w = R1 ? w1[inst] : 0.f;
   double s1 = 0.0, s2 = 0.0;
   unsigned gm = 0, xm = 0;
-  for (long i = b + threadIdx.x; i < e; i += 256) {
-    const float xh = (px[i] - m) * r;
-    const float gy = R1 ? r1_product(w, pg[i]) : pg[i];
+  auto grad = [&](long i) __attribute__((always_inline)) -> float {
+    if constexpr (GF == 1) return r1_product(w, pg[i]);
+    else if constexpr (GF == 2) {
+      const long pc = wk.cell(pl.Ho, pl.Wo);
+      const float g = pool_grad(pg[i], pi[pc], pd[pc], wk.k());
+      wk.next();
+      return g;
+    } else return pg[i];
+  };
+  auto acc = [&](float xv, float gy) __attribute__((always_inline)) {
+    const float xh = (xv - m) * r;
     const float g = xh > 0.f ? gy : gy * slope;
     s1 += (double)g;
     s2 = fma((double)g, (double)xh, s2);
     const unsigned gb = __float_as_uint(g) & 0x7fffffffu, xb = __float_as_uint(xh) & 0x7fffffffu;
     if (gb < 0x7f800000u && gb > gm) gm = gb;
     if (xb < 0x7f800000u && xb > xm) xm = xb;
-  }
+  };
+  long i = b + threadIdx.x;
+  for (; i + 768 < e; i += 1024) {
+    float xv[4], gv[4];
+#pragma unroll
+    for (int u = 0; u < 4; ++u) { xv[u] = px[i + 256 * u]; gv[u] = grad(i + 256 * u); }
+#pragma unroll
+    for (int u = 0; u < 4; ++u) acc(xv[u], gv[u]);
+  }
+  for (; i < e; i += 256) acc(px[i], grad(i));
 #pragma unroll
   for (int o = 32; o > 0; o >>= 1) {
     const unsigned q1 = (unsigned)__shfl_xor((int)gm, o), q2 = (unsigned)__shfl_xor((int)xm, o);
@@ -512,13 +574,14 @@
   for (int i = blockIdx.x * blockDim.x + threadIdx.x; i < n; i += gridDim.x * blockDim.x) p[i] = 0u;
 }
 
-template <bool R1 = false>
+template <int GF = 0>
 __global__ __launch_bounds__(256) void k_in_bwd_apply_h2(const float* __restrict__ dy, const float* __restrict__ x,
                                                          const float* __restrict__ mean, const float* __restrict__ rstd,
                                                          float slope, long S, int splits, const double* __restrict__ part,
                                                          uint4* __restrict__ dxs, int cblocks, double* __restrict__ rowpart,
                                                          const unsigned* __restrict__ cell, unsigned* __restrict__ guard,
-                                                         const float* __restrict__ w1 = nullptr) {
+                                                         const float* __restrict__ w1 = nullptr, PoolG pl = PoolG{}) {
+  constexpr bool R1 = GF == 1;
   __shared__ float sm[2][8];
   __shared__ double red[8][4];
   const long ncb = blockIdx.y;
@@ -540,7 +603,11 @@
 #pragma unroll
   for (int j = 0; j < 8; ++j) { m[j] = mean[ncb * 8 + j]; r[j] = rstd[ncb * 8 + j]; m1[j] = sm[0][j]; m2[j] = sm[1][j]; }
   const float* px = x + ncb * 8 * S;
-  const float* pg = R1 ? dy : dy + ncb * 8 * S;
+  const float* pg = R1 ? dy : GF == 2 ? dy + (ncb / cblocks) * pl.skip_stride + (ncb % cblocks) * 8 * S : dy + ncb * 8 * S;
+  const float* pd = GF == 2 ? pl.dyp + ncb * 8 * pl.So : nullptr;
+  const unsigned char* pi = GF == 2 ? pl.idx + ncb * 8 * pl.So : nullptr;
+  PoolWalk wk;
+  if constexpr (GF == 2) wk = PoolWalk((long)blockIdx.x * 256 + threadIdx.x, (long)gridDim.x * 256, pl.H, pl.W);
   float wj[8];
 #pragma unroll
   for (int j = 0; j < 8; ++j) wj[j] = R1 ? w1[ncb * 8 + j] : 0.f;
@@ -551,9 +618,16 @@
     unsigned short e[8][3];
     unsigned mx = 0;
     const float sv = R1 ? pg[v] : 0.f;
+    long pc = 0;
+    int pk = 0;
+    if constexpr (GF == 2) { pc = wk.cell(pl.Ho, pl.Wo); pk = wk.k(); wk.next(); }
 #pragma unroll
     for (int j = 0; j < 8; ++j) {
-      float t = in_bwd_value(px[j * S + v], R1 ? r1_product(wj[j], sv) : pg[j * S + v], m[j], r[j], m1[j], m2[j], slope);
+      float gy;
+      if constexpr (GF == 1) gy = r1_product(wj[j], sv);
+      else if constexpr (GF == 2) gy = pool_grad(pg[j * S + v], pi[j * pl.So + pc], pd[j * pl.So + pc], pk);
+      else gy = pg[j * S + v];
+      float t = in_bwd_value(px[j * S + v], gy, m[j], r[j], m1[j], m2[j], slope);
       rs[j] += (double)t;
       asm("" : "+v"(t));
       const unsigned b = __float_as_uint(t) & 0x7fffffffu;
@@ -973,13 +1047,13 @@
   long bx = cdiv(S, 1024);
   if (bx > 1024) bx = 1024;
   double* rowpart = (double*)((char*)ws + nc_instnorm_ws_bytes(NC, S));
-  hipLaunchKernelGGL(k_in_bwd_apply_s3<false>, dim3((unsigned)bx, (unsigned)(NC / 8)), dim3(256), 0, s, dy, x, mean, rstd, slope, S, splits,
-                     (const double*)ws, (uint4*)dxs, C / 8, rowpart, (const unsigned*)nullptr, (const float*)nullptr);
+  hipLaunchKernelGGL(k_in_bwd_apply_s3<0>, dim3((unsigned)bx, (unsigned)(NC / 8)), dim3(256), 0, s, dy, x, mean, rstd, slope, S, splits,
+                     (const double*)ws, (uint4*)dxs, C / 8, rowpart, (const unsigned*)nullptr, (const float*)nullptr, PoolG{});
   hipLaunchKernelGGL(k_in_dbias_final, dim3(C), dim3(256), 0, s, (const double*)rowpart, N, C, (int)bx, dbias);
   return check_launch("instnorm_act_bwd_dbias_s3");
 }
 static int in_bwd_dbias_h2(const float* dy, const float* w1, const float* x, const float* mean, const float* rstd, float slope, void* dxs,
-                           float* dbias, int N, int C, long S, void* ws, size_t ws_bytes, void* stream, unsigned* guard) {
+                           float* dbias, int N, int C, long S, void* ws, size_t ws_bytes, void* stream, unsigned* guard, const PoolG* pool = nullptr) {
   if (!dy || !x || !mean || !rstd || !dxs || !dbias) { set_error("instnorm_act_bwd_dbias_h2: null pointer"); return NC_ERR_ARG; }
   if (!instnorm_bwd_s3_supported(N, C, S)) { set_error("instnorm_act_bwd_dbias_h2: bad shape"); return NC_ERR_SHAPE; }
   const int NC = N * C;
@@ -992,22 +1066,29 @@
   unsigned* xmax = gmax + NC;
   hipLaunchKernelGGL(k_zero_u32, dim3((unsigned)cdiv(64 + 2 * NC, 256)), dim3(256), 0, s, cells, 64 + 2 * NC);
   const int splits = pick_splits(NC, S);
+  const PoolG pl = pool ? *pool : PoolG{};
   if (w1)
-    hipLaunchKernelGGL(k_in_bwd_sums_h2<true>, dim3(splits, NC), dim3(256), 0, s, dy, x, mean, rstd, slope, S, splits, (double*)ws, gmax, xmax, w1);
+    hipLaunchKernelGGL(k_in_bwd_sums_h2<1>, dim3(splits, NC), dim3(256), 0, s, dy, x, mean, rstd, slope, S, splits, (double*)ws, gmax, xmax, w1, pl);
+  else if (pool)
+    hipLaunchKernelGGL(k_in_bwd_sums_h2<2>, dim3(splits, NC), dim3(256), 0, s, dy, x, mean, rstd, slope, S, splits, (double*)ws, gmax, xmax,
+                       (const float*)nullptr, pl);
   else
-    hipLaunchKernelGGL(k_in_bwd_sums_h2<false>, dim3(splits, NC), dim3(256), 0, s, dy, x, mean, rstd, slope, S, splits, (double*)ws, gmax, xmax,
-                       (const float*)nullptr);
+    hipLaunchKernelGGL(k_in_bwd_sums_h2<0>, dim3(splits, NC), dim3(256), 0, s, dy, x, mean, rstd, slope, S, splits, (double*)ws, gmax, xmax,
+                       (const float*)nullptr, pl);
   hipLaunchKernelGGL(k_in_bwd_bound, dim3(1), dim3(256), 0, s, rstd, gmax, xmax, NC, cells, cells + 1, guard);
   long bx = cdiv(S, 1024);
   if (bx > 1024) bx = 1024;
   double* rowpart = (double*)((char*)ws + nc_instnorm_ws_bytes(NC, S));
   unsigned* g = guard && h2_guard_on() ? guard : nullptr;
   if (w1)
-    hipLaunchKernelGGL(k_in_bwd_apply_h2<true>, dim3((unsigned)bx, (unsigned)(NC / 8)), dim3(256), 0, s, dy, x, mean, rstd, slope, S, splits,
-                       (const double*)ws, (uint4*)dxs, C / 8, rowpart, (const unsigned*)cells, g, w1);
+    hipLaunchKernelGGL(k_in_bwd_apply_h2<1>, dim3((unsigned)bx, (unsigned)(NC / 8)), dim3(256), 0, s, dy, x, mean, rstd, slope, S, splits,
+                       (const double*)ws, (uint4*)dxs, C / 8, rowpart, (const unsigned*)cells, g, w1, pl);
+  else if (pool)
+    hipLaunchKernelGGL(k_in_bwd_apply_h2<2>, dim3((unsigned)bx, (unsigned)(NC / 8)), dim3(256), 0, s, dy, x, mean, rstd, slope, S, splits,
+                       (const double*)ws, (uint4*)dxs, C / 8, rowpart, (const unsigned*)cells, g, (const float*)nullptr, pl);
   else
-    hipLaunchKernelGGL(k_in_bwd_apply_h2<false>, dim3((unsigned)bx, (unsigned)(NC / 8)), dim3(256), 0, s, dy, x, mean, rstd, slope, S, splits,
-                       (const double*)ws, (uint4*)dxs, C / 8, rowpart, (const unsigned*)cells, g, (const float*)nullptr);
+    hipLaunchKernelGGL(k_in_bwd_apply_h2<0>, dim3((unsigned)bx, (unsigned)(NC / 8)), dim3(256), 0, s, dy, x, mean, rstd, slope, S, splits,
+                       (const double*)ws, (uint4*)dxs, C / 8, rowpart, (const unsigned*)cells, g, (const float*)nullptr, pl);
   hipLaunchKernelGGL(k_in_dbias_final, dim3(C), dim3(256), 0, s, (const double*)rowpart, N, C, (int)bx, dbias);
   if (g) {
     const unsigned long long total = (unsigned long long)(NC / 8) * (unsigned long long)cdiv(S, 64);
@@ -1016,11 +1097,14 @@
     if (!flip) return check_launch("instnorm_act_bwd_dbias_h2");
     long bx3 = bx < 128 ? bx : 128;
     if (w1)
-      hipLaunchKernelGGL(k_in_bwd_apply_s3<true>, dim3((unsigned)bx3, (unsigned)(NC / 8)), dim3(256), 0, s, dy, x, mean, rstd, slope, S, splits,
-                         (const double*)ws, (uint4*)dxs, C / 8, (double*)nullptr, (const unsigned*)g, w1);
+      hipLaunchKernelGGL(k_in_bwd_apply_s3<1>, dim3((unsigned)bx3, (unsigned)(NC / 8)), dim3(256), 0, s, dy, x, mean, rstd, slope, S, splits,
+                         (const double*)ws, (uint4*)dxs, C / 8, (double*)nullptr, (const unsigned*)g, w1, pl);
+    else if (pool)
+      hipLaunchKernelGGL(k_in_bwd_apply_s3<2>, dim3((unsigned)bx3, (unsigned)(NC / 8)), dim3(256), 0, s, dy, x, mean, rstd, slope, S, splits,
+                         (const double*)ws, (uint4*)dxs, C / 8, (double*)nullptr, (const unsigned*)g, (const float*)nullptr, pl);
     else
-      hipLaunchKernelGGL(k_in_bwd_apply_s3<false>, dim3((unsigned)bx3, (unsigned)(NC / 8)), dim3(256), 0, s, dy, x, mean, rstd, slope, S, splits,
-                         (const double*)ws, (uint4*)dxs, C / 8, (double*)nullptr, (const unsigned*)g, (const float*)nullptr);
+      hipLaunchKernelGGL(k_in_bwd_apply_s3<0>, dim3((unsigned)bx3, (unsigned)(NC / 8)), dim3(256), 0, s, dy, x, mean, rstd, slope, S, splits,
+                         (const double*)ws, (uint4*)dxs, C / 8, (double*)nullptr, (const unsigned*)g, (const float*)nullptr, pl);
   }
   return check_launch("instnorm_act_bwd_dbias_h2");
 }
@@ -1032,6 +1116,14 @@
                                     float* dbias, int C, long S, void* ws, size_t ws_bytes, void* stream, unsigned* guard) {
   if (!w1) { set_error("instnorm_act_bwd_dbias_h2_rank1: null pointer"); return NC_ERR_ARG; }
   return in_bwd_dbias_h2(dy1, w1, x, mean, rstd, slope, dxs, dbias, 1, C, S, ws, ws_bytes, stream, guard);
+}
+int instnorm_act_bwd_dbias_h2_pool(const float* skip, long skip_stride, const float* dyp, const unsigned char* idx, int D, int H, int W, const float* x,
+                                   const float* mean, const float* rstd, float slope, void* dxs, float* dbias, int N, int C, void* ws, size_t ws_bytes,
+                                   void* stream, unsigned* guard) {
+  if (!dyp || !idx) { set_error("instnorm_act_bwd_dbias_h2_pool: null pointer"); return NC_ERR_ARG; }
+  if (D < 2 || H < 2 || W < 2 || ((D | H | W) & 1)) { set_error("instnorm_act_bwd_dbias_h2_pool: even extents"); return NC_ERR_SHAPE; }
+  const PoolG pl{dyp, idx, skip_stride, (long)(D / 2) * (H / 2) * (W / 2), C, H, W, H / 2, W / 2};
+  return in_bwd_dbias_h2(skip, nullptr, x, mean, rstd, slope, dxs, dbias, N, C, (long)D * H * W, ws, ws_bytes, stream, guard, &pl);
 }
 int instnorm_relu_tail_sigmoid(const float* x, const float* mean, const float* rstd, const float* w1, const float* b1, const float* w2,
                                const float* b2, float* y, int C, long S, hipStream_t s) {
```

Measured after the change: 56.97 million (median of 6 runs). +2.5%, better.
